# RKWin93/E2E-MAPPO-for-MT-FJSP

Measured on AMD Instinct MI355X. Metric: env-steps/sec (batched J6M6E2), higher is better.
Workload: dtype f64 (environment) / f32 (encoder: f32 storage and accumulation; 128x128 products on the 16-bit matrix cores from split f32 operands, f32-accurate: DESIGN.md §4)

## Files before the change

### __graft_entry__.py

```python
#!/usr/bin/env python3
import os
import sys

ROOT = os.path.dirname(os.path.abspath(__file__))
if ROOT not in sys.path:
    sys.path.insert(0, ROOT)


def build() -> None:
    from importlib import import_module
    import mtfjsp_amd
    _build = import_module("e2e-mappo-for-mt-fjsp_amd._build")
    lib = _build.build(force=True, verbose=True)
    capi = import_module("e2e-mappo-for-mt-fjsp_amd.capi")
    capi.lib()
    print("variant:", _build.build_variant("funcs", ["-DMTFJSP_BODY_FUNCS=3"]))
    from oracle import env_oracle
    print("oracle:", env_oracle.build(force=True))
    print("built", lib)


def smoke() -> None:
    import numpy as np
    import torch
    from importlib import import_module
    import mtfjsp_amd
    assert torch.cuda.is_available(), "smoke() needs cuda:0"
    batch_env = import_module("e2e-mappo-for-mt-fjsp_amd.batch_env")
    inst = import_module("e2e-mappo-for-mt-fjsp_amd.instances")
    from oracle.env_oracle import OracleBatch
    J, M, E, B = 6, 6, 2, 8
    T = J * M
    t, p, tt, edge = inst.generate_instances(B, J, M, E, seed=0)
    import random
    random.seed(0)
    w3 = inst.random_weights(B)
    env = batch_env.DeviceBatchEnv(J, M, E, B, obs_dtype="f64")
    env.load_instances(t, p, tt, edge=edge)
    env.scaler_init()
    env.reset(w3)
    orc = OracleBatch(t, p, tt, edge)
    orc.scaler_init()
    orc.reset(w3)
    a = torch.zeros(B, dtype=torch.int32, device=env.device); m = torch.zeros_like(a); j = torch.zeros_like(a)
    for s in range(T):
        env.random_actions(7, s, a, m, j)
        env.step(a, m)
        info, raw, _ = orc.step(a.cpu().numpy(), m.cpu().numpy())
        cand, mask = orc.job_mask_update(j.cpu().numpy())
        o = orc.observe()
        assert np.array_equal(env.info.cpu().numpy(), info), f"step {s}: rewards differ"
        assert np.array_equal(env.tasks_fea.cpu().numpy(), o["tfea"]), f"step {s}: tasks_fea differ"
        assert np.array_equal(env.dense_adj().cpu().numpy(), o["adj"]), f"step {s}: adj differ"
        assert np.array_equal(env.m_fea2.cpu().numpy(), o["mfea2"])
        assert np.array_equal(env.candidate.cpu().numpy(), cand) and np.array_equal(env.job_mask.cpu().numpy(), mask)
    assert bool(env.info[:, 1].all())
    _smoke_encoder()
    print("smoke OK: HIP env == oracle on", B, "instances x", T, "steps")


def _smoke_encoder() -> None:
    try:
        from importlib import import_module
        enc = import_module("e2e-mappo-for-mt-fjsp_amd.encoder")
    except ImportError:
        return
    if hasattr(enc, "smoke"):
        enc.smoke()


if __name__ == "__main__":
    cmd = sys.argv[1] if len(sys.argv) > 1 else "build"
    {"build": build, "smoke": smoke}[cmd]()
```

### e2e-mappo-for-mt-fjsp_amd/capi.py

```python
import ctypes as C
import os

from . import _build

_LIB = None

OBS_F64, OBS_F32 = 0, 1
OK, ERR_ARG, ERR_STATE, ERR_HIP, ERR_ACTION, ERR_RETRY = 0, -1, -2, -3, -4, -5
PATH_MASK, ST_INVALID, ST_INFEASIBLE = 0x7, 0x100, 0x200
FORK_INSTANCE, FORK_STATE, FORK_OBS = 1, 2, 4
STATE_MACHINE, STATE_START, STATE_FINISH, STATE_ROUTES, STATE_PREV_COSTS, STATE_SCALER, STATE_W3 = range(7)


class Config(C.Structure):
    _fields_ = [("n_job", C.c_int32), ("n_machine", C.c_int32), ("n_edge", C.c_int32), ("batch", C.c_int32),
                ("left_shift", C.c_int32), ("obs_dtype", C.c_int32), ("device_id", C.c_int32), ("reserved", C.c_int32),
                ("gamma", C.c_double), ("w_mk", C.c_double), ("w_ec", C.c_double), ("w_tt", C.c_double),
                ("scaling_divisor", C.c_double)]


class Obs(C.Structure):
    _fields_ = [("tasks_fea", C.c_void_p), ("ell_col", C.c_void_p), ("ell_val", C.c_void_p), ("m_fea2", C.c_void_p),
                ("info", C.c_void_p), ("raw", C.c_void_p), ("candidate", C.c_void_p), ("job_mask", C.c_void_p),
                ("status", C.c_void_p)]


class Mfea1Ctx(C.Structure):
    _fields_ = [("t", C.c_void_p), ("p", C.c_void_p), ("tt", C.c_void_p), ("mean3", C.c_void_p), ("shop", C.c_void_p),
                ("link", C.c_void_p), ("m_fea1_out", C.c_void_p), ("mmask_out", C.c_void_p),
                ("T", C.c_int32), ("M", C.c_int32), ("obs_f32", C.c_int32), ("m_fea2", C.c_void_p)]


class EncoderConfig(C.Structure):
    _fields_ = [("n_job", C.c_int32), ("n_machine", C.c_int32), ("batch", C.c_int32), ("hidden", C.c_int32),
                ("obs_dtype", C.c_int32), ("device_id", C.c_int32)]


_VP, _I, _U64, _SZ = C.c_void_p, C.c_int, C.c_uint64, C.c_size_t
PROTOTYPES = {
    "mtfjsp_create": (_I, [C.POINTER(Config), C.POINTER(_VP)]),
    "mtfjsp_destroy": (_I, [_VP]),
    "mtfjsp_last_error": (C.c_char_p, [_VP]),
    "mtfjsp_set_stream": (_I, [_VP, _VP]),
    "mtfjsp_synchronize": (_I, [_VP]),
    "mtfjsp_alloc_obs": (_I, [_VP, C.POINTER(Obs)]),
    "mtfjsp_bind_obs": (_I, [_VP, C.POINTER(Obs)]),
    "mtfjsp_snapshot_obs": (_I, [_VP, C.POINTER(Obs)]),
    "mtfjsp_snapshot_obs2": (_I, [_VP, C.POINTER(Obs), C.POINTER(Obs), _VP]),
    "mtfjsp_generate_instances": (_I, [_VP, _U64, _U64, _VP]),
    "mtfjsp_read_instances_host": (_I, [_VP, _VP, _VP, _VP, _VP]),
    "mtfjsp_load_instances": (_I, [_VP, _VP, _VP, _VP, _VP]),
    "mtfjsp_load_instances_host": (_I, [_VP, _VP, _VP, _VP, _VP]),
    "mtfjsp_scaler_init": (_I, [_VP]),
    "mtfjsp_scaler_reset_returns": (_I, [_VP]),
    "mtfjsp_scaler_reset_returns_masked_host": (_I, [_VP, _VP]),
    "mtfjsp_reset": (_I, [_VP, _VP]),
    "mtfjsp_draw_reward_weights": (_I, [_VP, _U64, _U64, _VP]),
    "mtfjsp_reset_episode": (_I, [_VP, _U64, _U64, _VP, C.c_int32]),
    "mtfjsp_reset_host": (_I, [_VP, _VP]),
    "mtfjsp_step": (_I, [_VP, _VP, _VP]),
    "mtfjsp_step_host": (_I, [_VP, _VP, _VP]),
    "mtfjsp_step_record": (_I, [_VP, _VP, _VP, _VP, _VP]),
    "mtfjsp_step_params_bytes": (C.c_int32, []),
    "mtfjsp_step_params": (_I, [_VP, _VP, _VP, _VP, _VP, _VP, C.c_int32]),
    "mtfjsp_step_kernel_name": (C.c_char_p, [_VP]),
    "mtfjsp_step_kernel_name_for": (C.c_char_p, [C.c_int32, C.c_int32, C.c_int32, C.c_int32, C.c_int64, C.POINTER(C.c_int32), C.POINTER(C.c_int64), C.POINTER(C.c_int32)]),
    "mtfjsp_gae": (_I, [_VP, C.c_int32, _VP, C.c_int64, C.c_int64, _VP, C.c_int64, C.c_int64, _VP, C.c_int64, C.c_int64, _VP, C.c_float, C.c_float, _VP]),
    "mtfjsp_normalize_advantages": (_I, [_VP, C.c_int32, C.c_int32, C.c_int32, C.c_int32, C.c_int32, _VP, C.c_float, _VP, _VP, _VP, _VP, _VP, _VP]),
    "mtfjsp_pack_views": (_I, [_VP, C.c_int32, C.c_int32, _VP, _VP, _VP, _VP]),
    "mtfjsp_observe_mfea1": (_I, [_VP, _VP, _VP, _VP, _VP]),
    "mtfjsp_random_actions": (_I, [_VP, _U64, _U64, _VP, _VP, _VP]),
    "mtfjsp_pdr_plan": (_I, [_VP, _VP, _VP, _VP, _U64, _VP, _VP]),
    "mtfjsp_fork": (_I, [_VP, _VP, _VP, C.c_int32]),
    "mtfjsp_lookahead_expand": (_I, [_VP, _VP, _VP, _VP]),
    "mtfjsp_lookahead_select": (_I, [_VP, _VP, C.c_int32, _VP, _VP, _VP, _VP]),
    "mtfjsp_export_dense_adj": (_I, [_VP, _VP]),
    "mtfjsp_export_dense_adj_host": (_I, [_VP, _VP]),
    "mtfjsp_valid_action_mask": (_I, [_VP, _VP]),
    "mtfjsp_read_state_host": (_I, [_VP, _I, _VP]),
    "mtfjsp_set_scaler_state_host": (_I, [_VP, _I, _I, _VP]),
    "mtfjsp_copy_to_host": (_I, [_VP, _VP, _VP, _SZ]),
    "mtfjsp_footprint_copy": (_I, [_VP, _SZ, _SZ, C.c_int32, C.c_int32, C.c_int32, C.POINTER(C.c_double), C.POINTER(C.c_double)]),
    "mtfjsp_timing_begin": (_I, [_VP]),
    "mtfjsp_timing_end": (_I, [_VP, C.POINTER(C.c_double), C.POINTER(C.c_int64)]),
    "mtfjsp_encoder_create": (_I, [C.POINTER(EncoderConfig), C.POINTER(_VP)]),
    "mtfjsp_encoder_destroy": (_I, [_VP]),
    "mtfjsp_encoder_last_error": (C.c_char_p, [_VP]),
    "mtfjsp_encoder_set_stream": (_I, [_VP, _VP]),
    "mtfjsp_encoder_load_weight_host": (_I, [_VP, C.c_char_p, _VP, C.c_int64]),
    "mtfjsp_encoder_weights_ready": (_I, [_VP]),
    "mtfjsp_job_actor_forward": (_I, [_VP] * 11),
    "mtfjsp_machine_actor_forward": (_I, [_VP] * 8),
    "mtfjsp_global_critic_forward": (_I, [_VP] * 7),
    "mtfjsp_sample_categorical": (_I, [_VP, _VP, C.c_int32, C.c_int32, _U64, _U64, _VP, _VP, _VP, _VP]),
    "mtfjsp_encoder_set_bn_mode": (_I, [_VP, C.c_int32]),
    "mtfjsp_encoder_set_product_mode": (_I, [_VP, C.c_int32]),
    "mtfjsp_encoder_set_stats_reduce": (_I, [_VP, C.c_void_p, _VP, C.c_int64]),
    "mtfjsp_encoder_set_deferred_poll": (_I, [_VP, C.c_int32]),
    "mtfjsp_get_mfea1_context": (_I, [_VP, _VP, _VP, C.POINTER(Mfea1Ctx)]),
    "mtfjsp_encoder_arm_mfea1": (_I, [_VP, C.POINTER(Mfea1Ctx)]),
    "mtfjsp_encoder_arm_machine_heads": (_I, [_VP, _VP, _VP, _VP]),
    "mtfjsp_encoder_fused_launches": (_I, [_VP, C.POINTER(C.c_int64)]),
    "mtfjsp_encoder_arm_env_step": (_I, [_VP, _VP, C.c_int32]),
    "mtfjsp_encoder_arm_values_only": (_I, [_VP]),
    "mtfjsp_encoder_env_step_fused": (_I, [_VP]),
    "mtfjsp_encoder_arm_selection": (_I, [_VP, C.c_int32, C.c_int32, _U64, _U64, _VP, _VP, _VP, _VP]),
    "mtfjsp_hostgen_infeasible": (_I, [_VP, C.POINTER(C.c_int32), C.c_int64, _I, _I, C.c_int64, C.c_int64, _VP]),
    "mtfjsp_hostgen_transport": (_I, [_VP, C.POINTER(C.c_int32), C.c_int64, _I, _VP, C.c_double, C.c_double, C.c_double, C.c_int64, C.c_int64, _VP]),
    "mtfjsp_encoder_check": (_I, [_VP, C.POINTER(C.c_int32)]),
    "mtfjsp_encoder_resident_failures": (_I, [_VP, C.POINTER(C.c_int64)]),
    "mtfjsp_encoder_range_fallbacks": (_I, [_VP, C.POINTER(C.c_int64), C.POINTER(C.c_int32)]),
    "mtfjsp_encoder_peek_nodes_host": (_I, [_VP, _VP, C.c_int64]),
    "mtfjsp_encoder_timing_begin": (_I, [_VP]),
    "mtfjsp_encoder_timing_end": (_I, [_VP, C.POINTER(C.c_double), C.POINTER(C.c_int64)]),
    "mtfjsp_encoder_timing_query": (_I, [_VP, C.c_char_p, C.POINTER(C.c_double), C.POINTER(C.c_int64)]),
}


def lib_path():
    return os.environ.get("MTFJSP_LIB") or _build.LIB


def lib():
    global _LIB
    if _LIB is None:
        path = lib_path()
        if not os.path.exists(path):
            raise RuntimeError(
                f"{path} is missing: build the HIP extension first (python __graft_entry__.py build, "
                "or python e2e-mappo-for-mt-fjsp_amd/_build.py). There is no CPU fallback.")
        L = C.CDLL(path)
        for name, (res, args) in PROTOTYPES.items():
            fn = getattr(L, name)
            fn.restype, fn.argtypes = res, args
        _LIB = L
    return _LIB


class MtfjspError(RuntimeError):
    def __init__(self, code, msg):
        super().__init__(f"libmtfjsp error {code}: {msg}")
        self.code = code


def check(rc, handle=None, enc=False):
    if rc != 0:
        L = lib()
        msg = (L.mtfjsp_encoder_last_error(handle) if enc else L.mtfjsp_last_error(handle)) or b""
        raise MtfjspError(rc, msg.decode())
```

### e2e-mappo-for-mt-fjsp_amd/csrc/mtfjsp_encoder.hip

```cpp
#include <hip/hip_runtime.h>
#include <math.h>
#include <stdint.h>
#include <stdio.h>
#include <stdlib.h>
#include <string.h>
#include <algorithm>
#include <map>
#include <stdexcept>
#include <string>
#include <vector>

#include "../../include/mtfjsp.h"


#include "mtfjsp_enc_shared.h"

enum { PRO_PLAIN = 0, PRO_BNRELU = 1, PRO_AGG = 2, PRO_GIN0 = 3, PRO_GIN0BN = 4 };
enum { EPI_PLAIN = 0, EPI_STATS = 1, EPI_TANH = 2 };

struct GemmArgs {
    const float *in;
    int N;
    const float *Wt;
    const void *Wx6;
// ... 2379 lines not shown
    float *my_a = s_a + wave * 16 * LDA16;
    float *my_f = s_feat + wave * 128;
    const float *ap = my_a + m * LDA16 + q;
    const float *bp = s_w + q * HD + m;
    int bo[8];
    for (int c = 0; c < 8; c++) bo[c] = (c ^ qo) * 16;
    float asrc[8], adst[8];
    for (int c = 0; c < 8; c++) { asrc[c] = A.gat_a[c * 16 + m]; adst[c] = A.gat_a[HD + c * 16 + m]; }
    const int t = wave;
    const bool active = t * 16 < N;
    float mv[8][2];
    for (int c = 0; c < 8; c++) { mv[c][0] = 0.f; mv[c][1] = 0.f; }
    if (active) {
        {
            const int r = t * 16 + (lane >> 1), k0 = (lane & 1) * 4;
            float x[4] = {0.f, 0.f, 0.f, 0.f};
            if (lane < 32 && r < N) {
                const int u = r >> 1, node = r & 1, width = node ? 8 : 6;
                for (int k = 0; k < 4; k++)
                    if (k0 + k < width) {
                        const size_t idx = ((size_t)b * M + u) * width + k0 + k;
                        x[k] = A.feat_f64 ? (float)reinterpret_cast<const double *>(node ? A.f2 : A.f1)[idx]
                                          : reinterpret_cast<const float *>(node ? A.f2 : A.f1)[idx];
                    }
            }
            if (lane < 32) *reinterpret_cast<float4 *>(my_f + lane * 4) = make_float4(x[0], x[1], x[2], x[3]);
            asm volatile("s_waitcnt lgkmcnt(0)" ::: "memory");
        }
#pragma unroll
        for (int p = 0; p < 8; p++) {
            const int r = 2 * p + h;
            const float4 fa = *reinterpret_cast<const float4 *>(my_f + r * 8), fb = *reinterpret_cast<const float4 *>(my_f + r * 8 + 4);
            const float ff[8] = {fa.x, fa.y, fa.z, fa.w, fb.x, fb.y, fb.z, fb.w};
            float o[4];
            for (int x = 0; x < 4; x++) {
                float a = 0.f;
                for (int k = 0; k < 8; k++) {
                    const float w = h == 0 ? (k < 6 ? A.W1[(c4 + x) * 6 + k] : 0.f) : A.W2[(c4 + x) * 8 + k];
                    a = fmaf(ff[k], w, a);
                }
                o[x] = a;
            }
            float *d = my_a + r * LDA16 + c4;
            *reinterpret_cast<float2 *>(d) = make_float2(o[0], o[1]);
            *reinterpret_cast<float2 *>(d + 2) = make_float2(o[2], o[3]);
        }
        asm volatile("s_waitcnt lgkmcnt(0)" ::: "memory");
#pragma unroll 1
        for (int pass = 0; pass < 3; pass++) {
            f32x4 acc[8];
            for (int c = 0; c < 8; c++) for (int i = 0; i < 4; i++) acc[c][i] = 0.f;
            mfma_tile16(ap, bp, bo, acc);
            asm volatile("" ::: "memory");
#pragma unroll
            for (int u = 0; u < 2; u++) {
                const int i = 2 * u;
                float s0 = 0.f, d0 = 0.f, d1 = 0.f;
                for (int c = 0; c < 8; c++) { const float z0 = acc[c][i], z1 = acc[c][i + 1]; s0 += asrc[c] * z0; d0 += adst[c] * z0; d1 += adst[c] * z1; }
                s0 = row_sum16(s0); d0 = row_sum16(d0); d1 = row_sum16(d1);
                float e00 = s0 + d0, e01 = s0 + d1;
                e00 = e00 > 0.f ? e00 : 0.2f * e00;
                e01 = e01 > 0.f ? e01 : 0.2f * e01;
                const float mx = fmaxf(e00, e01);
                const float x0 = __expf(e00 - mx), x1 = __expf(e01 - mx);
                const float inv = 1.0f / (x0 + x1);
                const float al0 = x0 * inv, al1 = x1 * inv;
                const int r = 4 * q + i;
                for (int c = 0; c < 8; c++) {
                    const float z0 = acc[c][i], z1 = acc[c][i + 1];
                    float n0 = al0 * z0 + al1 * z1, n1 = z1;
                    if (pass < 2) {
                        n0 = n0 > 0.f ? n0 : __expf(n0) - 1.0f;
                        n1 = n1 > 0.f ? n1 : __expf(n1) - 1.0f;
                        my_a[r * LDA16 + c * 16 + m] = n0;
                        my_a[(r + 1) * LDA16 + c * 16 + m] = n1;
                    } else mv[c][u] = (n0 + n1) * 0.5f;
                }
            }
            asm volatile("s_waitcnt lgkmcnt(0)" ::: "memory");
        }
        for (int c = 0; c < 8; c++) {
            double a = 0, bq = 0;
            for (int u = 0; u < 2; u++)
                if (t * 16 + 4 * q + 2 * u < N) { a += (double)mv[c][u]; bq += (double)mv[c][u] * (double)mv[c][u]; }
            a += __shfl_xor(a, 16); a += __shfl_xor(a, 32);
            bq += __shfl_xor(bq, 16); bq += __shfl_xor(bq, 32);
            if (q == 0) { atomicAdd(&s_st[c * 16 + m], a); atomicAdd(&s_st[HD + c * 16 + m], bq); }
        }
    }
    __syncthreads();
    stage_bn_local(s_bn, s_st, 1.0 / (double)M, A.gamma, A.beta, tid);
    __syncthreads();
    if (active) {
        for (int c = 0; c < 8; c++) {
            const int col = c * 16 + m;
            float pl = 0.f;
            for (int u = 0; u < 2; u++) {
                const int r = t * 16 + 4 * q + 2 * u;
                if (r < N) {
                    const float y = fmaf(mv[c][u], s_bn[col], s_bn[HD + col]);
                    A.node[((size_t)b * M + (r >> 1)) * HD + col] = y;
                    pl += y;
                }
            }
            pl += __shfl_xor(pl, 16); pl += __shfl_xor(pl, 32);
            if (q == 0) atomicAdd(&s_pool[col], pl);
        }
    }
    __syncthreads();
    if (tid < HD) A.h_pooled[(size_t)b * HD + tid] = s_pool[tid] / (float)M;
}
static size_t inst_lds_bytes() { return (size_t)(HD * HD + 8 * 16 * LDA16 + 2 * HD) * 4 + 512 * 8 + (HD + 8 * 128) * 4 + 64; }

struct mtfjsp_encoder {
    mtfjsp_encoder_config_t cfg;
    int T = 0;
    hipStream_t stream = nullptr;
    std::string err;
    std::map<std::string, float *> w;
    std::map<std::string, float *> wt;
    std::map<std::string, std::vector<float>> hostw;
    std::map<std::string, float *> wfused;
    std::map<std::string, size_t> wx6_bytes;
    std::map<std::string, size_t> wx32_bytes;
    std::map<std::string, void *> wx6;
    std::map<std::string, void *> wx32;
    std::map<std::string, float> wx32_sinv;
    std::map<std::string, float> wx6_sinv;
    std::map<std::string, float *> wimg;
    std::vector<void *> owned;
    int num_cu = 256;
    float *zA = nullptr, *zB = nullptr;
    float *cand_feat = nullptr;
    float *u = nullptr, *c1 = nullptr, *c2 = nullptr, *hm_b = nullptr, *pooled_int = nullptr;
    bool hm_b_valid = false;
    float *node = nullptr;
    double *stats = nullptr;
    bool gin_slot5_dirty = false;
    bool gin_stats_clean = false;
    bool gat_stats_clean[2] = {false, false};
    int bn_mode = 0;
    bool defer_poll = false;
    mtfjsp_stats_reduce_fn reduce_fn = nullptr; void *reduce_user = nullptr;
    double reduce_scale = 1.0;
    int f32_products = (getenv("MTFJSP_GEMM_F32MFMA") ? 1 : 0) | (getenv("MTFJSP_GAT_F32MFMA") ? 2 : 0) |
                       (getenv("MTFJSP_HEADS_F32MFMA") ? 4 : 0) | (getenv("MTFJSP_GIN0_VALU") ? 8 : 0);
    bool res_ok = false; int res_ipc = 0, res_grid = 0;
    double *res_stats = nullptr;
    unsigned long long *res_bar = nullptr;
    unsigned *res_fail = nullptr;
    volatile unsigned *res_fail_host = nullptr;
    unsigned *range_flag = nullptr;
    long long range_fallbacks = 0;
    bool res_eligible = false;
    long long res_failures = 0, res_launches = 0;
    long long res_fail_at = getenv("MTFJSP_GIN_RES_FAIL_AT") ? atoll(getenv("MTFJSP_GIN_RES_FAIL_AT")) : 0;
    long long range_fail_at = getenv("MTFJSP_RANGE_FAIL_AT") ? atoll(getenv("MTFJSP_RANGE_FAIL_AT")) : 0, job_forwards = 0;
    float *res_zspill = nullptr;
    unsigned long long res_epoch = 0;
    int gat_slot = 0;
    struct { bool valid = false; const void *f1 = nullptr, *f2 = nullptr; int slot = 0;
             bool heads = false; const float *h_pooled_o = nullptr; const uint8_t *mmask = nullptr; float *prob = nullptr, *h_pooled = nullptr, *machine_v = nullptr;
           } prefused;
    bool fuse_gat = !getenv("MTFJSP_NO_FUSED_GAT");
    bool fuse_mheads = !getenv("MTFJSP_NO_FUSED_MHEADS");
    struct { bool armed = false; float *prob = nullptr, *h_pooled = nullptr, *machine_v = nullptr; } mh;
    unsigned long long *xw = nullptr;
    unsigned long long xw_epoch = 0;
    long long fused3_launches = 0;
    double xchg_fine_limit = getenv("MTFJSP_XCHG_FINE_LIMIT") ? atof(getenv("MTFJSP_XCHG_FINE_LIMIT")) : 2147483648.0;
    long long fused3_fail_at = getenv("MTFJSP_FUSED3_FAIL_AT") ? atoll(getenv("MTFJSP_FUSED3_FAIL_AT")) : 0;
    bool heads_hg8 = !getenv("MTFJSP_NO_HEADS_HG8");
    bool heads10 = !getenv("MTFJSP_NO_HEADS10");
    bool fuse_env = getenv("MTFJSP_FUSED_ENV") != nullptr;
    bool fuse_env3 = getenv("MTFJSP_FUSED_ENV3") != nullptr;
    bool nodes_lds = !getenv("MTFJSP_FUSED3_NODES_HBM");
    bool warm_heads = !getenv("MTFJSP_NO_WARM_HEADS");
    struct { bool armed = false, done = false; EnvParams P; } env_step;
    int fuse_pair = getenv("MTFJSP_FUSE_PAIR") ? atoi(getenv("MTFJSP_FUSE_PAIR")) : 0;
    int stream_order = getenv("MTFJSP_NO_STREAM_ORDER") ? 0 : 1;
    int fuse_pool = getenv("MTFJSP_FUSE_POOL") ? atoi(getenv("MTFJSP_FUSE_POOL")) : 1;
    int fuse_gin0 = getenv("MTFJSP_FUSE_GIN0") ? atoi(getenv("MTFJSP_FUSE_GIN0")) : 1;
    int pool_s = getenv("MTFJSP_POOL_S") ? atoi(getenv("MTFJSP_POOL_S")) : 4;
    int stream_nt = getenv("MTFJSP_STREAM_NT") ? atoi(getenv("MTFJSP_STREAM_NT")) : 5;
    mtfjsp_mfea1_ctx_t mf_ctx{}; bool mf_armed = false;
    struct FusedSample { bool armed = false; int greedy = 0; uint64_t seed = 0, counter = 0; int32_t *idx = nullptr; float *logp = nullptr;
                         const int32_t *gather_from = nullptr; int32_t *gathered = nullptr; } fs[2];
    int values_only = 0;
    bool vo_now = false;
    FusedSample fs1_consumed;
    bool timing = false;
    std::map<std::string, std::vector<std::pair<hipEvent_t, hipEvent_t>>> ev;
    std::vector<std::pair<hipEvent_t, hipEvent_t>> ev_free;
};
static thread_local std::string g_enc_err;

#define HIPCHK(e, call)                                                                         \
    do {                                                                                        \
        hipError_t e_ = (call);                                                                 \
        if (e_ != hipSuccess) {                                                                 \
            (e)->err = std::string(#call) + ": " + hipGetErrorString(e_);                       \
            return MTFJSP_ERR_HIP;                                                              \
        }                                                                                       \
    } while (0)

template <typename Tp>
static int dalloc(mtfjsp_encoder *e, Tp **ptr, size_t n)
{
    HIPCHK(e, hipMalloc((void **)ptr, n * sizeof(Tp)));
    e->owned.push_back(*ptr);
    return 0;
}

static const char *REQUIRED[] = {
    "job_actor._input",
    "job_actor.encoder.feature_extract.mlps.0.linears.0.weight", "job_actor.encoder.feature_extract.mlps.0.linears.0.bias",
    "job_actor.encoder.feature_extract.mlps.0.linears.1.weight", "job_actor.encoder.feature_extract.mlps.0.linears.1.bias",
    "job_actor.encoder.feature_extract.mlps.0.linears.2.weight", "job_actor.encoder.feature_extract.mlps.0.linears.2.bias",
    "job_actor.encoder.feature_extract.mlps.0.batch_norms.0.weight", "job_actor.encoder.feature_extract.mlps.0.batch_norms.0.bias",
    "job_actor.encoder.feature_extract.mlps.0.batch_norms.1.weight", "job_actor.encoder.feature_extract.mlps.0.batch_norms.1.bias",
    "job_actor.encoder.feature_extract.mlps.1.linears.0.weight", "job_actor.encoder.feature_extract.mlps.1.linears.0.bias",
    "job_actor.encoder.feature_extract.mlps.1.linears.1.weight", "job_actor.encoder.feature_extract.mlps.1.linears.1.bias",
    "job_actor.encoder.feature_extract.mlps.1.linears.2.weight", "job_actor.encoder.feature_extract.mlps.1.linears.2.bias",
    "job_actor.encoder.feature_extract.mlps.1.batch_norms.0.weight", "job_actor.encoder.feature_extract.mlps.1.batch_norms.0.bias",
    "job_actor.encoder.feature_extract.mlps.1.batch_norms.1.weight", "job_actor.encoder.feature_extract.mlps.1.batch_norms.1.bias",
    "job_actor.encoder.feature_extract.batch_norms.0.weight", "job_actor.encoder.feature_extract.batch_norms.0.bias",
    "job_actor.encoder.feature_extract.batch_norms.1.weight", "job_actor.encoder.feature_extract.batch_norms.1.bias",
    "job_actor.o_policy.linears.0.weight", "job_actor.o_policy.linears.0.bias",
    "job_actor.o_policy.linears.1.weight", "job_actor.o_policy.linears.1.bias",
    "job_actor.o_policy.linears.2.weight", "job_actor.o_policy.linears.2.bias",
    "job_actor.job_critic.linears.0.weight", "job_actor.job_critic.linears.0.bias",
    "job_actor.job_critic.linears.1.weight", "job_actor.job_critic.linears.1.bias",
    "job_actor.job_critic.linears.2.weight", "job_actor.job_critic.linears.2.bias",
    "machine_actor.bn.weight", "machine_actor.bn.bias", "machine_actor.m_fea_1_fcl.weight", "machine_actor.m_fea_2_fcl.weight",
    "machine_actor.gat_layer.W", "machine_actor.gat_layer.a",
    "machine_actor.m_policy.linears.0.weight", "machine_actor.m_policy.linears.0.bias",
    "machine_actor.m_policy.linears.1.weight", "machine_actor.m_policy.linears.1.bias",
    "machine_actor.m_policy.linears.2.weight", "machine_actor.m_policy.linears.2.bias",
    "machine_actor.machine_critic.linears.0.weight", "machine_actor.machine_critic.linears.0.bias",
    "machine_actor.machine_critic.linears.1.weight", "machine_actor.machine_critic.linears.1.bias",
    "machine_actor.machine_critic.linears.2.weight", "machine_actor.machine_critic.linears.2.bias",
};

static int res_alloc_fail_word(mtfjsp_encoder *e)
{
    void *h = nullptr, *d = nullptr;
    if (hipHostMalloc(&h, 64, hipHostMallocMapped) != hipSuccess) return 1;
    if (hipHostGetDevicePointer(&d, h, 0) != hipSuccess) { (void)hipHostFree(h); return 1; }
    e->res_fail_host = (volatile unsigned *)h; e->res_fail = (unsigned *)d; e->range_flag = (unsigned *)d + 1;
    e->res_fail_host[0] = 0u; e->res_fail_host[1] = 0u;
    return 0;
}
static bool res_census(mtfjsp_encoder *e)
{
    if (hipDeviceSynchronize() != hipSuccess) return false;
    if (hipMemset(e->res_bar, 0, (size_t)17 * 16 * 8) != hipSuccess) return false;
    e->res_epoch = 0;
    *e->res_fail_host = 0u;
    GinResArgs a{};
    a.bar = e->res_bar; a.epoch = e->res_epoch++; a.fail = e->res_fail; a.barrier_only = 1;
    hipLaunchKernelGGL(k_gin_res, dim3(e->res_grid), dim3(256), gin_res_lds_bytes(), nullptr, a);
    if (hipDeviceSynchronize() != hipSuccess || *e->res_fail_host) {
        (void)hipMemset(e->res_bar, 0, (size_t)17 * 16 * 8); e->res_epoch = 0; *e->res_fail_host = 0u;
        return false;
    }
    return true;
}
static bool split_products_in_use(const mtfjsp_encoder *e) { return (e->f32_products & 15) != 15; }
static int res_poll_failure(mtfjsp_encoder *e)
{
    if (!e->res_fail_host) return MTFJSP_OK;
    if (e->res_fail_host[0]) {
        (void)hipStreamSynchronize(e->stream);
        e->res_ok = false; e->res_failures++;
        e->res_fail_host[0] = 0u; e->res_fail_host[1] = 0u;
        (void)hipMemset(e->res_bar, 0, (size_t)17 * 16 * 8); e->res_epoch = 0;
        if (e->res_stats) (void)hipMemset(e->res_stats, 0, (size_t)2 * GR_STATS_SET * 8);
        if (e->xw) (void)hipMemset(e->xw, 0, (size_t)2 * XW_SET * 8);
        e->xw_epoch = 0; e->prefused.valid = false; e->prefused.heads = false;
        e->gin_stats_clean = false; e->gat_stats_clean[0] = e->gat_stats_clean[1] = false;
        e->err = "single-launch GIN kernel / fused heads launch: a grid-wide statistics exchange timed out (the workgroups were not co-resident); every output "
                 "enqueued since that launch is invalid and must be recomputed; the handle now uses the streaming launches";
        return MTFJSP_ERR_RETRY;
    }
    if (e->res_fail_host[1]) {
        (void)hipStreamSynchronize(e->stream);
        e->res_fail_host[1] = 0u;
        if (split_products_in_use(e)) {
            e->f32_products |= 15; e->range_fallbacks++;
            e->gin_stats_clean = false; e->gat_stats_clean[0] = e->gat_stats_clean[1] = false;
            e->err = "an activation left the f16 range of the split products (outputs were not numbers): the handle now uses the "
                     "f32-instruction kernels; repeat the forward(s) enqueued since";
            return MTFJSP_ERR_RETRY;
        }
    }
    return MTFJSP_OK;
}

extern "C" const char *mtfjsp_encoder_last_error(mtfjsp_encoder_t e) { return e ? e->err.c_str() : g_enc_err.c_str(); }

extern "C" int mtfjsp_encoder_create(const mtfjsp_encoder_config_t *cfg, mtfjsp_encoder_t *out)
{
    if (!cfg || !out) { g_enc_err = "null argument"; return MTFJSP_ERR_ARG; }
    if (cfg->hidden != HD || cfg->n_job < 1 || cfg->n_job > 64 || cfg->n_machine < 2 || cfg->n_machine > 64 || cfg->batch < 1) {
        g_enc_err = "bad encoder configuration (hidden must be 128, n_job<=64, 2<=n_machine<=64)"; return MTFJSP_ERR_ARG;
    }
    int ndev = 0;
    if (hipGetDeviceCount(&ndev) != hipSuccess || ndev == 0) { g_enc_err = "no HIP device available"; return MTFJSP_ERR_HIP; }
    if (cfg->device_id < 0 || cfg->device_id >= ndev) { g_enc_err = "device_id out of range"; return MTFJSP_ERR_ARG; }
    if (hipSetDevice(cfg->device_id) != hipSuccess) { g_enc_err = "hipSetDevice failed"; return MTFJSP_ERR_HIP; }
    mtfjsp_encoder *e = new mtfjsp_encoder();
    e->cfg = *cfg;
    e->T = cfg->n_job * cfg->n_machine;
    hipDeviceProp_t prop;
    if (hipGetDeviceProperties(&prop, cfg->device_id) == hipSuccess) e->num_cu = prop.multiProcessorCount;
    const size_t B = cfg->batch, T = e->T, M = cfg->n_machine, J = cfg->n_job, R = J > M ? J : M;
    int rc = 0;
    auto rows_padded = [](size_t rows) { return ((rows + 31) / 32 + 1) * 32; };
    auto dalloc_rows = [&](float **ptr, size_t rows) {
        const size_t n = rows_padded(rows) * HD;
        if (dalloc(e, ptr, n)) return 1;
        return hipMemset(*ptr, 0, n * sizeof(float)) == hipSuccess ? 0 : 1;
    };
    rc |= dalloc_rows(&e->zA, B * T); rc |= dalloc_rows(&e->zB, B * T);
    rc |= dalloc_rows(&e->cand_feat, B * R);
    rc |= dalloc_rows(&e->u, B); rc |= dalloc_rows(&e->c1, B); rc |= dalloc_rows(&e->c2, B); rc |= dalloc_rows(&e->hm_b, B);
    rc |= dalloc_rows(&e->pooled_int, B);
    rc |= dalloc_rows(&e->node, B * M);
    rc |= dalloc(e, &e->stats, 8 * STAT_REP * 256);
    rc |= res_alloc_fail_word(e);
    rc |= dalloc(e, &e->xw, (size_t)2 * XW_SET);
    if (!rc && hipMemset(e->xw, 0, (size_t)2 * XW_SET * 8) != hipSuccess) rc = 1;
    if (!rc && hipMemset(e->stats, 0, 8 * STAT_REP * 256 * sizeof(double)) == hipSuccess) { e->gin_stats_clean = true; e->gat_stats_clean[0] = e->gat_stats_clean[1] = true; }
    if (rc) { g_enc_err = e->err; mtfjsp_encoder_destroy(e); return MTFJSP_ERR_HIP; }
    const int lds16 = (int)gemm16_lds_bytes();
    (void)hipFuncSetAttribute((const void *)k_gemm16<EPI_PLAIN, false>, hipFuncAttributeMaxDynamicSharedMemorySize, lds16);
    (void)hipFuncSetAttribute((const void *)k_gemm16<EPI_TANH, false>, hipFuncAttributeMaxDynamicSharedMemorySize, lds16);
    (void)hipFuncSetAttribute((const void *)k_gemm16<EPI_TANH, true>, hipFuncAttributeMaxDynamicSharedMemorySize, lds16);
    (void)hipFuncSetAttribute((const void *)k_gemm16p<PRO_BNRELU>, hipFuncAttributeMaxDynamicSharedMemorySize, lds16);
    (void)hipFuncSetAttribute((const void *)k_gemm16p<PRO_AGG>, hipFuncAttributeMaxDynamicSharedMemorySize, lds16);
    (void)hipFuncSetAttribute((const void *)k_gat3, hipFuncAttributeMaxDynamicSharedMemorySize, lds16);
    (void)hipFuncSetAttribute((const void *)k_gat3x, hipFuncAttributeMaxDynamicSharedMemorySize, (int)gat3x_lds_bytes());
    (void)hipFuncSetAttribute((const void *)k_gemm_x6<PRO_BNRELU>, hipFuncAttributeMaxDynamicSharedMemorySize, (int)gemm_x6_lds_bytes());
    (void)hipFuncSetAttribute((const void *)k_gemm_x6<PRO_AGG>, hipFuncAttributeMaxDynamicSharedMemorySize, (int)gemm_x6_lds_bytes());
    (void)hipFuncSetAttribute((const void *)k_gemm_x6<PRO_GIN0>, hipFuncAttributeMaxDynamicSharedMemorySize, (int)gemm_x6_lds_bytes());
    (void)hipFuncSetAttribute((const void *)k_gemm_x6<PRO_GIN0BN>, hipFuncAttributeMaxDynamicSharedMemorySize, (int)gemm_x6_lds_bytes());
    if (hipFuncSetAttribute((const void *)k_gemm_x6f, hipFuncAttributeMaxDynamicSharedMemorySize, (int)gemm_x6f_lds_bytes()) != hipSuccess) e->fuse_pair = 0;
    (void)hipFuncSetAttribute((const void *)k_gin_inst<float>, hipFuncAttributeMaxDynamicSharedMemorySize, (int)inst_lds_bytes());
    (void)hipFuncSetAttribute((const void *)k_gin_inst<double>, hipFuncAttributeMaxDynamicSharedMemorySize, (int)inst_lds_bytes());
    (void)hipFuncSetAttribute((const void *)k_gat_inst, hipFuncAttributeMaxDynamicSharedMemorySize, (int)inst_lds_bytes());
    (void)hipFuncSetAttribute((const void *)k_heads, hipFuncAttributeMaxDynamicSharedMemorySize, (int)heads_lds_bytes());
    (void)hipFuncSetAttribute((const void *)k_headsx, hipFuncAttributeMaxDynamicSharedMemorySize, (int)headsx_lds_bytes());
    if (hipFuncSetAttribute((const void *)k_headsx10, hipFuncAttributeMaxDynamicSharedMemorySize, (int)headsx10_lds_bytes()) != hipSuccess) e->heads10 = false;
    (void)hipFuncSetAttribute((const void *)k_headsx_envstep<float>, hipFuncAttributeMaxDynamicSharedMemorySize, (int)(headsx_lds_bytes() > EnvGrpDynLds<1>::bytes ? headsx_lds_bytes() : EnvGrpDynLds<1>::bytes));
    (void)hipFuncSetAttribute((const void *)k_headsx_envstep<double>, hipFuncAttributeMaxDynamicSharedMemorySize, (int)(headsx_lds_bytes() > EnvGrpDynLds<1>::bytes ? headsx_lds_bytes() : EnvGrpDynLds<1>::bytes));
    (void)hipFuncSetAttribute((const void *)k_headsx_gat3x, hipFuncAttributeMaxDynamicSharedMemorySize,
                              (int)(headsx_lds_bytes() > gat3x_lds_bytes() ? headsx_lds_bytes() : gat3x_lds_bytes()));
#if !MTFJSP_BODY_FUNCS
    (void)hipFuncSetAttribute((const void *)k_headsx_values, hipFuncAttributeMaxDynamicSharedMemorySize, (int)headsx_lds_bytes());
    (void)hipFuncSetAttribute((const void *)k_headsx_gat3x_headsx<1, false>, hipFuncAttributeMaxDynamicSharedMemorySize, (int)fused3_lds_bytes());
    (void)hipFuncSetAttribute((const void *)k_headsx_gat3x_headsx<2, false>, hipFuncAttributeMaxDynamicSharedMemorySize, (int)fused3_lds_bytes());
    (void)hipFuncSetAttribute((const void *)k_headsx_gat3x_headsx<0, true>, hipFuncAttributeMaxDynamicSharedMemorySize, (int)fused3_lds_bytes());
    (void)hipFuncSetAttribute((const void *)k_headsx_gat3x_headsx<1, true>, hipFuncAttributeMaxDynamicSharedMemorySize, (int)fused3_lds_bytes());
    (void)hipFuncSetAttribute((const void *)k_headsx_gat3x_headsx<2, true>, hipFuncAttributeMaxDynamicSharedMemorySize, (int)fused3_lds_bytes());
    if (hipFuncSetAttribute((const void *)k_headsx_gat3x_headsx<0, false>, hipFuncAttributeMaxDynamicSharedMemorySize,
                            (int)fused3_lds_bytes()) != hipSuccess) e->fuse_mheads = false;
#else
    e->fuse_mheads = false;
#endif
    {
        const int T = e->T, B = cfg->batch;
        if (!getenv("MTFJSP_NO_RESIDENT_GIN") && T >= GR_MINT && T <= GR_MAXT) {
            const int ipc = (B + e->num_cu - 1) / e->num_cu;
            const int grid = (B + ipc - 1) / ipc;
            if (ipc * T <= GR_ROWS && ipc <= GR_MAXIPC && grid <= e->num_cu && (grid + 7) / 8 <= 63 && ipc * cfg->n_job <= GR_MAXCAND &&
                hipFuncSetAttribute((const void *)k_gin_res, hipFuncAttributeMaxDynamicSharedMemorySize, (int)gin_res_lds_bytes()) == hipSuccess) {
                int rc = dalloc(e, &e->res_stats, (size_t)2 * GR_STATS_SET) | dalloc(e, &e->res_bar, (size_t)17 * 16) |
                         dalloc(e, &e->res_zspill, (size_t)grid * 4 * (GR_NT - GR_NRES) * 1024);
                if (!rc && hipMemset(e->res_stats, 0, (size_t)2 * GR_STATS_SET * 8) == hipSuccess &&
                    hipMemset(e->res_bar, 0, (size_t)17 * 16 * 8) == hipSuccess) {
                    e->res_ipc = ipc; e->res_grid = grid; e->res_eligible = true;
                    e->res_ok = res_census(e);
                }
            }
        }
    }
    *out = e;
    return MTFJSP_OK;
}

extern "C" int mtfjsp_encoder_destroy(mtfjsp_encoder_t e)
{
    if (!e) return MTFJSP_OK;
    (void)hipSetDevice(e->cfg.device_id);
    (void)hipDeviceSynchronize();
    for (void *p : e->owned) (void)hipFree(p);
    if (e->res_fail_host) (void)hipHostFree((void *)e->res_fail_host);
    for (auto &kv : e->ev) for (auto &p : kv.second) { (void)hipEventDestroy(p.first); (void)hipEventDestroy(p.second); }
    for (auto &p : e->ev_free) { (void)hipEventDestroy(p.first); (void)hipEventDestroy(p.second); }
    delete e;
    return MTFJSP_OK;
}
extern "C" int mtfjsp_encoder_set_stream(mtfjsp_encoder_t e, void *s) { if (!e) return MTFJSP_ERR_ARG; e->stream = (hipStream_t)s; return MTFJSP_OK; }

static uint16_t f32_to_f16_bits(float x)
{
    uint32_t u; memcpy(&u, &x, 4);
    const uint32_t sign = (u >> 16) & 0x8000u; u &= 0x7fffffffu;
    uint32_t o;
    if (u >= ((127u + 16u) << 23)) o = u > (255u << 23) ? 0x7e00u : 0x7c00u;
    else if (u < (113u << 23)) { float f, magic; const uint32_t mb = ((127u - 15u) + (23u - 10u) + 1u) << 23; memcpy(&f, &u, 4); memcpy(&magic, &mb, 4);
                                 f += magic; uint32_t fu; memcpy(&fu, &f, 4); o = fu - mb; }
    else { const uint32_t odd = (u >> 13) & 1u; u += ((15u - 127u) << 23) + 0xfffu; u += odd; o = u >> 13; }
    return (uint16_t)(o | sign);
}
static float f16_bits_to_f32(uint16_t hbits)
{
    const uint32_t sgn = (uint32_t)(hbits & 0x8000u) << 16, ex = (hbits >> 10) & 31u, m = hbits & 0x3ffu;
    float x;
    if (ex == 0) { x = ldexpf((float)m, -24); return sgn ? -x : x; }
    const uint32_t u = sgn | ((ex == 31 ? 255u : ex + 112u) << 23) | (m << 13);
    memcpy(&x, &u, 4); return x;
}
static float f16_image_scale(const float *data, int64_t numel, bool *finite)
{
    float mx = 0.f;
    for (int64_t i = 0; i < numel; i++) mx = fmaxf(mx, fabsf(data[i]));
    *finite = mx < INFINITY;
    int ex = 0;
    if (mx > 0.f && *finite) (void)frexpf(mx, &ex);
    int k = 14 - ex; k = k > 60 ? 60 : k < -60 ? -60 : k;
    return ldexpf(1.0f, k);
}

static int64_t expected_numel(const std::string &key)
{
    const size_t dot = key.find('.');
    if (dot == std::string::npos) return -1;
    const std::string pre = key.substr(0, dot), k = key.substr(dot + 1);
    if (pre != "job_actor" && pre != "machine_actor" && pre != "global_critic") return -1;
    auto ends = [&](const char *suf) { const size_t n = strlen(suf); return k.size() >= n && k.compare(k.size() - n, n, suf) == 0; };
    auto has = [&](const char *sub) { return k.find(sub) != std::string::npos; };
    if (k == "_input") return HD;
    if (has("batch_norms") || k == "bn.weight" || k == "bn.bias" || k == "encoder.feature_extract.bn.weight" || k == "encoder.feature_extract.bn.bias")
        return has("feature_extract.bn.") ? 12 : HD;
    if (has("feature_extract.mlps.")) {
        if (ends(".bias")) return HD;
        return has("mlps.0.linears.0.weight") ? (int64_t)HD * 12 : (int64_t)HD * HD;
    }
    if (has("feature_extract.eps")) return 2;
    if (k == "m_fea_1_fcl.weight") return (int64_t)HD * 6;
    if (k == "m_fea_2_fcl.weight") return (int64_t)HD * 8;
    if (k == "gat_layer.W") return (int64_t)HD * HD;
    if (k == "gat_layer.a") return 2 * HD;
    if (has("fcl_pooling")) return ends(".bias") ? HD : (int64_t)HD * HD;
    for (const char *head : {"o_policy", "m_policy", "job_critic", "machine_critic", "critic"}) {
        const std::string h = std::string(head) + ".linears.";
        if (k.compare(0, h.size(), h) != 0) continue;
        const int layer = k[h.size()] - '0';
        const bool policy = strstr(head, "policy") != nullptr;
        const int first_in = policy ? 3 * HD : (strcmp(head, "critic") == 0 ? 2 * HD : HD);
        const int out_last = policy ? 1 : (strcmp(head, "critic") == 0 ? 4 : 2);
        const int in = layer == 0 ? first_in : HD, out = layer == 2 ? out_last : HD;
        if (layer < 0 || layer > 2) return -1;
        return ends(".bias") ? out : (int64_t)out * in;
    }
    return -1;
}

extern "C" int mtfjsp_encoder_load_weight_host(mtfjsp_encoder_t e, const char *name, const float *data, int64_t numel)
{
    if (!e || !name || !data || numel <= 0) return MTFJSP_ERR_ARG;
    std::string key(name);
    {
        const int64_t want = expected_numel(key);
        if (want < 0) { e->err = "unknown weight name: " + key; return MTFJSP_ERR_ARG; }
        if (want != numel) {
            e->err = "weight " + key + ": expected " + std::to_string(want) + " elements, got " + std::to_string(numel);
            return MTFJSP_ERR_ARG;
        }
    }
    HIPCHK(e, hipSetDevice(e->cfg.device_id));
    float *d = nullptr;
    auto it = e->w.find(key);
    if (it != e->w.end()) d = it->second;
    else { if (dalloc(e, &d, (size_t)numel)) return MTFJSP_ERR_HIP; e->w[key] = d; }
    HIPCHK(e, hipMemcpy(d, data, (size_t)numel * 4, hipMemcpyHostToDevice));
    if (key == "job_actor._input") e->hm_b_valid = false;
    if ((key.size() >= 11 && key.compare(key.size() - 11, 11, "gat_layer.W") == 0) || key.find("m_fea_1_fcl.weight") != std::string::npos ||
        key.find("m_fea_2_fcl.weight") != std::string::npos) {
        e->hostw[key].assign(data, data + numel);
        const std::string prefix = key.substr(0, key.find('.') + 1);
        e->wfused.erase(prefix + "1"); e->wfused.erase(prefix + "2"); e->wfused.erase(prefix + "q");
    }
    if (numel == (int64_t)HD * 12 && key.find("mlps.0.linears.0.weight") != std::string::npos) {
        auto to_bf16 = [](float x) { uint32_t u; memcpy(&u, &x, 4); u += 0x7fffu + ((u >> 16) & 1u); return (uint16_t)(u >> 16); };
        auto from_bf16 = [](uint16_t b) { uint32_t u = (uint32_t)b << 16; float x; memcpy(&x, &u, 4); return x; };
        std::vector<uint16_t> im((size_t)4 * 2 * 3 * 64 * 8, 0);
        for (int cgi = 0; cgi < 4; cgi++)
            for (int c = 0; c < 2; c++)
                for (int lane = 0; lane < 64; lane++)
                    for (int i = 0; i < 8; i++) {
                        const int n = 32 * cgi + 16 * c + (lane & 15), k = 8 * (lane >> 4) + i;
                        if (k >= 12) continue;
                        const float w = data[(size_t)n * 12 + k];
                        const uint16_t p0 = to_bf16(w); const float r1 = w - from_bf16(p0);
                        const uint16_t p1 = to_bf16(r1); const float r2 = r1 - from_bf16(p1);
                        const uint16_t pl[3] = {p0, p1, to_bf16(r2)};
                        for (int p = 0; p < 3; p++) im[(((((size_t)cgi * 2 + c) * 3 + p) * 64 + lane) * 8) + i] = pl[p];
                    }
        void *dx = nullptr;
        auto kt = e->wx6.find(key);
        if (kt != e->wx6.end()) dx = kt->second;
        else { float *tmp = nullptr; if (dalloc(e, &tmp, im.size() / 2)) return MTFJSP_ERR_HIP; dx = tmp; e->wx6[key] = dx; }
        HIPCHK(e, hipMemcpy(dx, im.data(), im.size() * 2, hipMemcpyHostToDevice));
            e->wx6_bytes[key] = im.size() * 2;
    }
    if (key.find("feature_extract.mlps.") != std::string::npos && key.size() > 7 && key.compare(key.size() - 7, 7, ".weight") == 0 &&
        key.find("linears") != std::string::npos) {
        const int in = (int)(numel / HD), KS = in == 12 ? 1 : in / 16, P = in == 12 ? 3 : 2;
        auto to_bf16 = [](float x) { uint32_t u; memcpy(&u, &x, 4); u += 0x7fffu + ((u >> 16) & 1u); return (uint16_t)(u >> 16); };
        auto from_bf16 = [](uint16_t b) { uint32_t u = (uint32_t)b << 16; float x; memcpy(&x, &u, 4); return x; };
        float scale = 1.0f;
        if (P == 2) {
            bool finite = true;
            scale = f16_image_scale(data, numel, &finite);
            if (!finite) { e->err = "load_weight: non-finite value in " + key; return MTFJSP_ERR_ARG; }
        }
        std::vector<uint16_t> im((size_t)4 * P * KS * 64 * 8, 0);
        for (int w = 0; w < 4; w++)
            for (int ks = 0; ks < KS; ks++)
                for (int lane = 0; lane < 64; lane++)
                    for (int j = 0; j < 8; j++) {
                        const int n = 32 * w + (lane & 31), k = 16 * ks + 8 * (lane >> 5) + j;
// ... 211 lines not shown
            hipLaunchKernelGGL((k_gin0<float>), dim3(pgrid), dim3(256), 0, e->stream, N, T, (const float *)tasks_fea, ell_col, ell_val,
                               W(P + "mlps.0.linears.0.weight"), W(P + "mlps.0.linears.0.bias"), e->zA, st + 0 * STAT_REP * 256);
        else
            hipLaunchKernelGGL((k_gin0<double>), dim3(pgrid), dim3(256), 0, e->stream, N, T, (const double *)tasks_fea, ell_col, ell_val,
                               W(P + "mlps.0.linears.0.weight"), W(P + "mlps.0.linears.0.bias"), e->zA, st + 0 * STAT_REP * 256);
        if ((rrc = reduce_stats(e, st + 0 * STAT_REP * 256))) return rrc;
    }
    const int so = e->stream_order;
    auto bn_gemm = [&](const float *in, float *out, int sin, const std::string &bn, const std::string &lin, int sout, int rev) {
        GemmArgs a = gemm_args(in, N, WT(P + lin + ".weight"), W(P + lin + ".bias"), out);
        a.rev = so ? rev : 0; a.nt = so && (e->stream_nt & 1);
        a.pro_stats = st + sin * STAT_REP * 256; a.pro_gamma = W(P + bn + ".weight"); a.pro_beta = W(P + bn + ".bias"); a.pro_inv_rows = invN;
        a.epi_stats = st + sout * STAT_REP * 256;
        a.Wx6 = e->wx6.at(P + lin + ".weight"); a.w_sinv = e->wx6_sinv.at(P + lin + ".weight");
        launch_gemm<PRO_BNRELU, EPI_STATS>(e, a, "gin_gemm_bn_relu");
        if (!rrc) rrc = reduce_stats(e, st + sout * STAT_REP * 256);
    };
    auto bn_gemm_pair = [&](const float *in, float *out, int sin, const std::string &bn1, const std::string &lin1, int smid,
                            const std::string &bn2, const std::string &lin2, int sout, int rev) {
        {
            GemmArgs a = gemm_args(in, N, WT(P + lin1 + ".weight"), W(P + lin1 + ".bias"), nullptr);
            a.rev = so ? rev : 0; a.nt = so && (e->stream_nt & 1);
            a.pro_stats = st + sin * STAT_REP * 256; a.pro_gamma = W(P + bn1 + ".weight"); a.pro_beta = W(P + bn1 + ".bias"); a.pro_inv_rows = invN;
            a.epi_stats = st + smid * STAT_REP * 256;
            a.Wx6 = e->wx6.at(P + lin1 + ".weight"); a.w_sinv = e->wx6_sinv.at(P + lin1 + ".weight");
            launch_gemm<PRO_BNRELU, EPI_STATS>(e, a, "gin_gemm_stats_only");
            if (!rrc) rrc = reduce_stats(e, st + smid * STAT_REP * 256);
        }
        {
            Timed t(e, "gin_gemm_pair");
            Gemm2Args g{};
            g.a = gemm_args(in, N, WT(P + lin1 + ".weight"), W(P + lin1 + ".bias"), out);
            g.a.rev = so ? rev ^ 1 : 0; g.a.nt = so && (e->stream_nt & 1);
            g.a.pro_stats = st + sin * STAT_REP * 256; g.a.pro_gamma = W(P + bn1 + ".weight"); g.a.pro_beta = W(P + bn1 + ".bias"); g.a.pro_inv_rows = invN;
            g.a.epi_stats = st + sout * STAT_REP * 256;
            g.a.Wx6 = e->wx6.at(P + lin1 + ".weight"); g.a.w_sinv = e->wx6_sinv.at(P + lin1 + ".weight");
            g.a.range_flag = e->range_flag;
            g.Wx6b = e->wx6.at(P + lin2 + ".weight"); g.w_sinvb = e->wx6_sinv.at(P + lin2 + ".weight"); g.biasb = W(P + lin2 + ".bias");
            g.mid_stats = st + smid * STAT_REP * 256; g.mid_gamma = W(P + bn2 + ".weight"); g.mid_beta = W(P + bn2 + ".bias"); g.mid_inv_rows = invN;
            const int ntiles = (N + 15) / 16;
            int grid = (ntiles + 7) / 8;
            if (grid > e->num_cu) grid = e->num_cu;
            hipLaunchKernelGGL(k_gemm_x6f, dim3(grid), dim3(512), gemm_x6f_lds_bytes(), e->stream, g);
        }
        if (!rrc) rrc = reduce_stats(e, st + sout * STAT_REP * 256);
    };
    if (pair) bn_gemm_pair(e->zA, e->zB, 0, "mlps.0.batch_norms.0", "mlps.0.linears.1", 1, "mlps.0.batch_norms.1", "mlps.0.linears.2", 2, 0);
    else {
    if (fuse0) {
        const std::string lin = "mlps.0.linears.1", bn = "mlps.0.batch_norms.0";
        GemmArgs a = gemm_args(nullptr, N, WT(P + lin + ".weight"), W(P + lin + ".bias"), e->zB);
        a.rev = 0; a.nt = 0;
        a.tfea = tasks_fea; a.feat_f64 = 0; a.ell_col = ell_col; a.ell_val = ell_val; a.T = T;
        a.Wx6_0 = e->wx6.at(P + "mlps.0.linears.0.weight"); a.bias0 = W(P + "mlps.0.linears.0.bias");
        a.W0 = mom0 ? W(P + "mlps.0.linears.0.weight") : nullptr;
        a.pro_stats = st + 0 * STAT_REP * 256; a.pro_gamma = W(P + bn + ".weight"); a.pro_beta = W(P + bn + ".bias"); a.pro_inv_rows = invN;
        a.epi_stats = st + 1 * STAT_REP * 256;
        a.Wx6 = e->wx6.at(P + lin + ".weight"); a.w_sinv = e->wx6_sinv.at(P + lin + ".weight");
        launch_gemm<PRO_GIN0BN, EPI_STATS>(e, a, "gin0_bn_gemm");
        if (!rrc) rrc = reduce_stats(e, st + 1 * STAT_REP * 256);
    } else
    bn_gemm(e->zA, e->zB, 0, "mlps.0.batch_norms.0", "mlps.0.linears.1", 1, 0);
    bn_gemm(e->zB, e->zA, 1, "mlps.0.batch_norms.1", "mlps.0.linears.2", 2, 1);
    }
    const float *z2 = pair ? e->zB : e->zA;
    float *z3 = pair ? e->zA : e->zB;
    {
        GemmArgs a = gemm_args(z2, N, WT(P + "mlps.1.linears.0.weight"), W(P + "mlps.1.linears.0.bias"), z3);
        a.pro_stats = st + 2 * STAT_REP * 256; a.pro_gamma = W(P + "batch_norms.0.weight"); a.pro_beta = W(P + "batch_norms.0.bias"); a.pro_inv_rows = invN;
        a.ell_col = ell_col; a.ell_val = ell_val; a.T = T;
        a.rev = 0; a.nt = so && (e->stream_nt & 2);
        a.epi_stats = st + 3 * STAT_REP * 256;
        a.Wx6 = e->wx6.at(P + "mlps.1.linears.0.weight"); a.w_sinv = e->wx6_sinv.at(P + "mlps.1.linears.0.weight");
        launch_gemm<PRO_AGG, EPI_STATS>(e, a, "gin_gemm_agg");
        if (!rrc) rrc = reduce_stats(e, st + 3 * STAT_REP * 256);
    }
    if (pair) bn_gemm_pair(z3, e->zB, 3, "mlps.1.batch_norms.0", "mlps.1.linears.1", 4, "mlps.1.batch_norms.1", "mlps.1.linears.2", 5, 1);
    else {
    bn_gemm(e->zB, e->zA, 3, "mlps.1.batch_norms.0", "mlps.1.linears.1", 4, 1);
    const bool fuse_pool = e->fuse_pool && h_pooled && !h_nodes && T >= 16 && T < 65536 && (!candidate || (J > 0 && T % J == 0)) && (size_t)N < ((size_t)1 << 24) &&
                           e->wx6.count(P + "mlps.1.linears.2.weight") && !(e->f32_products & 1);
    if (fuse_pool) {
        const std::string lin = "mlps.1.linears.2", bn = "mlps.1.batch_norms.1";
        GemmArgs a = gemm_args(e->zA, N, WT(P + lin + ".weight"), W(P + lin + ".bias"), nullptr);
        a.rev = 0; a.nt = 0;
        a.pro_stats = st + 4 * STAT_REP * 256; a.pro_gamma = W(P + bn + ".weight"); a.pro_beta = W(P + bn + ".bias"); a.pro_inv_rows = invN;
        a.epi_stats = st + 5 * STAT_REP * 256;
        a.Wx6 = e->wx6.at(P + lin + ".weight"); a.w_sinv = e->wx6_sinv.at(P + lin + ".weight");
        a.zero_f32 = h_pooled; a.zero_count = B * HD;
        launch_gemm<PRO_BNRELU, EPI_STATS>(e, a, "gin_gemm_stats_only");
        a.zero_f32 = nullptr; a.zero_count = 0;
        if (!rrc) rrc = reduce_stats(e, st + 5 * STAT_REP * 256);
        if (rrc) return rrc;
        a.rev = so ? 1 : 0; a.nt = so && (e->stream_nt & 1);
        a.epi_stats = nullptr;
        a.T = T; a.pooled = h_pooled; a.cand_feat = candidate ? cand_feat : nullptr; a.cand = candidate; a.pool_J = candidate ? J : 0;
        a.pool_stats = st + 5 * STAT_REP * 256; a.pool_gamma = W(P + "batch_norms.1.weight"); a.pool_beta = W(P + "batch_norms.1.bias"); a.pool_inv_rows = invN;
        launch_gemm<PRO_BNRELU, EPI_STATS>(e, a, "gin_gemm_pool");
        if (candidate) {
            Timed t(e, "cand_fixup");
            hipLaunchKernelGGL(k_cand_fixup, dim3((B * J + 127) / 128), dim3(128), 0, e->stream, B, T, J, candidate, e->zA, st + 4 * STAT_REP * 256, W(P + bn + ".weight"), W(P + bn + ".bias"),
                               WT(P + lin + ".weight"), W(P + lin + ".bias"), st + 5 * STAT_REP * 256, W(P + "batch_norms.1.weight"), W(P + "batch_norms.1.bias"), invN, cand_feat);
        }
        HIPCHK(e, hipGetLastError());
        return MTFJSP_OK;
    }
    bn_gemm(e->zA, e->zB, 4, "mlps.1.batch_norms.1", "mlps.1.linears.2", 5, 0);
    }
    if (rrc) return rrc;
    if (h_pooled) {
        Timed t(e, "job_pool_gather");
        const int ntiles = (N + 15) / 16, ggrid = std::min((ntiles + 7) / 8, e->num_cu), rpr = so && e->pool_s > 0 ? ((ntiles + ggrid - 1) / ggrid) * 16 : 0;
        const int pool_grid = rpr ? ggrid * e->pool_s : (B < e->num_cu * 8 ? B : e->num_cu * 8);
        if (so && (e->stream_nt & 4))
            hipLaunchKernelGGL(k_job_pool_gather<1>, dim3(pool_grid), dim3(256), 0, e->stream, split_products_in_use(e) ? e->range_flag : nullptr, rpr, e->pool_s, B, T, candidate ? J : 0, e->zB, st + 5 * STAT_REP * 256, invN,
                               W(P + "batch_norms.1.weight"), W(P + "batch_norms.1.bias"), candidate, h_pooled, cand_feat, h_nodes);
        else
            hipLaunchKernelGGL(k_job_pool_gather<0>, dim3(pool_grid), dim3(256), 0, e->stream, split_products_in_use(e) ? e->range_flag : nullptr, rpr, e->pool_s, B, T, candidate ? J : 0, e->zB, st + 5 * STAT_REP * 256, invN,
                               W(P + "batch_norms.1.weight"), W(P + "batch_norms.1.bias"), candidate, h_pooled, cand_feat, h_nodes);
    }
    HIPCHK(e, hipGetLastError());
    return MTFJSP_OK;
}

static int run_gin_resident(mtfjsp_encoder *e, const std::string &pre, const void *tasks_fea, const int32_t *ell_col, const float *ell_val,
                            const int32_t *candidate, int J, float *h_pooled, float *cand_feat, float *h_nodes)
{
    const int B = e->cfg.batch, T = e->T;
    const std::string P = pre + "encoder.feature_extract.";
    auto W = [&](const std::string &k) { return e->w.at(k); };
    GinResArgs a{};
    a.B = B; a.T = T; a.J = candidate ? J : 0; a.ipc = e->res_ipc;
    a.tfea = tasks_fea; a.feat_f64 = e->cfg.obs_dtype == MTFJSP_OBS_F64; a.ell_col = ell_col; a.ell_val = ell_val;
    const char *lin[6] = {"mlps.0.linears.0", "mlps.0.linears.1", "mlps.0.linears.2", "mlps.1.linears.0", "mlps.1.linears.1", "mlps.1.linears.2"};
    const char *bn[6] = {"mlps.0.batch_norms.0", "mlps.0.batch_norms.1", "batch_norms.0", "mlps.1.batch_norms.0", "mlps.1.batch_norms.1", "batch_norms.1"};
    for (int i = 0; i < 6; i++) {
        a.Wx32[i] = e->wx32.at(P + lin[i] + ".weight");
        a.wsinv[i] = e->wx32_sinv.at(P + lin[i] + ".weight");
        a.gamma[i] = W(P + bn[i] + ".weight"); a.beta[i] = W(P + bn[i] + ".bias");
    }
    for (int i = 0; i < 6; i++) {
        int ex = 0;
        const float mant = frexpf(a.wsinv[i], &ex);
        if (mant != 0.5f) { e->err = "resident GIN: a weight image scale is not a power of two"; return MTFJSP_ERR_STATE; }
        a.wexp[i] = 1 - ex;
        a.ffrac[i] = i == 0 ? GR_FIX_FRAC_FIRST : GR_FIX_FRAC_DEFAULT;
    }
    const int set = (int)(e->res_epoch & 1);
    a.stats = reinterpret_cast<unsigned long long *>(e->res_stats) + (size_t)set * GR_STATS_SET;
    a.stats_next = reinterpret_cast<unsigned long long *>(e->res_stats) + (size_t)(set ^ 1) * GR_STATS_SET;
    a.bar = e->res_bar; a.epoch = e->res_epoch++; a.fail = e->res_fail; a.range_flag = e->range_flag;
    a.candidate = candidate; a.pooled = h_pooled; a.cand_feat = cand_feat; a.h_nodes = h_nodes; a.zspill = e->res_zspill;
    a.inv_rows = 1.0 / ((double)B * (double)T);
    if (pre == "job_actor." && e->warm_heads) {
        const char *keys[9] = {"job_actor.o_policy.linears.0.weight", "job_actor.job_critic.linears.0.weight", "job_actor.o_policy.linears.1.weight",
                               "job_actor.job_critic.linears.1.weight", "machine_actor.gat_layer.W", "machine_actor.m_policy.linears.0.weight",
                               "machine_actor.machine_critic.linears.0.weight", "machine_actor.m_policy.linears.1.weight", "machine_actor.machine_critic.linears.1.weight"};
        for (const char *k : keys) {
            auto it = e->wx6.find(k);
            auto bt = e->wx6_bytes.find(k);
            if (it == e->wx6.end() || bt == e->wx6_bytes.end() || a.nwarm >= GR_MAXWARM) continue;
            a.warm[a.nwarm] = it->second; a.warm_lines[a.nwarm] = (unsigned)(bt->second / 128); a.nwarm++;
        }
        auto q = e->wfused.find("machine_actor.q");
        if (q != e->wfused.end() && a.nwarm < GR_MAXWARM) { a.warm[a.nwarm] = q->second; a.warm_lines[a.nwarm] = 64; a.nwarm++; }
    }
    if (++e->res_launches == e->res_fail_at) a.expect_extra = 1u;
#ifdef GR_STAMP
    static unsigned long long *d_st = nullptr;
    if (!d_st) (void)hipMalloc((void **)&d_st, 256 * 64 * 8);
    a.stamps = d_st;
#endif
    {
        Timed t(e, "gin_resident");
        hipLaunchKernelGGL(k_gin_res, dim3(e->res_grid), dim3(256), gin_res_lds_bytes(), e->stream, a);
    }
#ifdef GR_STAMP
    static int printed = 0;
    if (printed++ % 50 == 20 && getenv("MTFJSP_STAMP_PRINT")) {
        (void)hipStreamSynchronize(e->stream);
        std::vector<unsigned long long> h((size_t)e->res_grid * 64);
        (void)hipMemcpy(h.data(), d_st, h.size() * 8, hipMemcpyDeviceToHost);
        unsigned long long t0 = ~0ull;
        for (int b = 0; b < e->res_grid; b++) t0 = h[(size_t)b * 64 + 32] < t0 ? h[(size_t)b * 64 + 32] : t0;
        printf("GR_STAMP (us since first block start; mean / max over %d blocks):", e->res_grid);
        for (int i = 0; i < 33; i++) {
            double m = 0, mx = 0;
            for (int b = 0; b < e->res_grid; b++) { const double v = (double)(h[(size_t)b * 64 + i] - t0) / 100.0; m += v; mx = v > mx ? v : mx; }
            printf(" [%d] %.1f/%.1f", i, m / e->res_grid, mx);
        }
        printf("\n");
        {
            auto clk = [&](int a, int b) {
                std::vector<double> v;
                for (int blk = 0; blk < e->res_grid; blk++) {
                    const double dr = (double)(h[(size_t)blk * 64 + b] - h[(size_t)blk * 64 + a]), dc = (double)(h[(size_t)blk * 64 + 33 + b] - h[(size_t)blk * 64 + 33 + a]);
                    if (dr > 0) v.push_back(dc / dr * 0.1);
                }
                std::sort(v.begin(), v.end());
                return v.empty() ? 0.0 : v[v.size() / 2];
            };
            printf("GR_CLOCK launch %d (GHz, median over %d workgroups): five layers [7 -> 24] %.3f | layer 1 [7 -> 8] %.3f  layer 2 [11 -> 12] %.3f  layer 3 [15 -> 16] %.3f  "
                   "layer 4 [19 -> 20] %.3f  layer 5 [23 -> 24] %.3f | whole kernel [0 -> 30] %.3f\n", printed, e->res_grid, clk(7, 24), clk(7, 8), clk(11, 12), clk(15, 16), clk(19, 20), clk(23, 24), clk(0, 30));
        }
    }
#endif
    HIPCHK(e, hipGetLastError());
    return MTFJSP_OK;
}

static std::vector<float> fused_projection_host(mtfjsp_encoder *e, const std::string &pre, int which)
{
    const int K = which == 1 ? 6 : 8;
    const std::vector<float> &P = e->hostw.at(pre + (which == 1 ? "m_fea_1_fcl.weight" : "m_fea_2_fcl.weight"));
    const std::vector<float> &W = e->hostw.at(pre + "gat_layer.W");
    std::vector<float> f((size_t)HD * K);
    for (int n = 0; n < HD; n++)
        for (int k = 0; k < K; k++) {
            double a = 0.0;
            for (int i = 0; i < HD; i++) a += (double)P[(size_t)i * K + k] * (double)W[(size_t)i * HD + n];
            f[(size_t)n * K + k] = (float)a;
        }
    return f;
}
static int fused_projection(mtfjsp_encoder *e, const std::string &pre, int which, const float **out)
{
    const std::string key = pre + (which == 1 ? "1" : "2");
    auto it = e->wfused.find(key);
    if (it != e->wfused.end()) { *out = it->second; return MTFJSP_OK; }
    const std::vector<float> f = fused_projection_host(e, pre, which);
    float *d = nullptr;
    if (dalloc(e, &d, f.size())) return MTFJSP_ERR_HIP;
    HIPCHK(e, hipMemcpy(d, f.data(), f.size() * 4, hipMemcpyHostToDevice));
    e->wfused[key] = d;
    *out = d;
    return MTFJSP_OK;
}
static int fused_projection_image(mtfjsp_encoder *e, const std::string &pre, const float **out)
{
    const std::string key = pre + "q";
    auto it = e->wfused.find(key);
    if (it != e->wfused.end()) { *out = it->second; return MTFJSP_OK; }
    const std::vector<float> f1 = fused_projection_host(e, pre, 1), f2 = fused_projection_host(e, pre, 2);
    std::vector<float> img((size_t)8 * 64 * 4);
    for (int c = 0; c < 8; c++)
        for (int lane = 0; lane < 64; lane++)
            for (int ks = 0; ks < 4; ks++) {
                const int kk = 4 * ks + (lane >> 4), col = 16 * c + (lane & 15);
                img[((size_t)c * 64 + lane) * 4 + ks] = kk < 6 ? f1[(size_t)col * 6 + kk] : kk < 8 ? 0.f : f2[(size_t)col * 8 + (kk - 8)];
            }
    float *d = nullptr;
    if (dalloc(e, &d, img.size())) return MTFJSP_ERR_HIP;
    HIPCHK(e, hipMemcpy(d, img.data(), img.size() * 4, hipMemcpyHostToDevice));
    e->wfused[key] = d;
    *out = d;
    return MTFJSP_OK;
}
static int gat3x_args(mtfjsp_encoder *e, const std::string &pre, const void *m_fea1, const void *m_fea2, int slot, GatArgs *out)
{
    const int R = e->cfg.batch * e->cfg.n_machine;
    double *st = nullptr;
    if (slot >= 0) {
        st = e->stats + (6 + slot) * STAT_REP * 256;
        if (!e->gat_stats_clean[slot]) HIPCHK(e, hipMemsetAsync(st, 0, STAT_REP * 256 * sizeof(double), e->stream));
        e->gat_stats_clean[slot] = false;
    }
    GatArgs a{};
    a.R = R; a.f1 = m_fea1; a.f2 = m_fea2; a.feat_f64 = e->cfg.obs_dtype == MTFJSP_OBS_F64;
    int frc = fused_projection(e, pre, 1, &a.W1);
    if (!frc) frc = fused_projection(e, pre, 2, &a.W2);
    if (!frc) frc = fused_projection_image(e, pre, &a.Wq);
    if (frc) return frc;
    a.Wt = e->wt.at(pre + "gat_layer.W"); a.gat_a = e->w.at(pre + "gat_layer.a"); a.node = e->node; a.epi_stats = st;
    a.Wx6 = e->wx6.at(pre + "gat_layer.W"); a.w_sinv = e->wx6_sinv.at(pre + "gat_layer.W");
    *out = a;
    return MTFJSP_OK;
}
static bool gat_fusable(const mtfjsp_encoder *e)
{
    const int hgrid = e->cfg.batch / HG, gtiles = (2 * e->cfg.batch * e->cfg.n_machine + 15) / 16, ggrid = (gtiles + 7) / 8 < e->num_cu ? (gtiles + 7) / 8 : e->num_cu;
    return e->fuse_gat && !e->bn_mode && !e->reduce_fn && !(e->f32_products & (2 | 4)) && e->cfg.batch % HG == 0 && hgrid <= e->num_cu && hgrid >= ggrid &&
           e->w.count("machine_actor.gat_layer.W") && e->wx6.count("machine_actor.gat_layer.W");
}
static bool mheads_fusable(const mtfjsp_encoder *e)
{
    const int hgrid = e->cfg.batch / HG;
    return e->fuse_mheads && e->res_ok && gat_fusable(e) && hgrid <= e->num_cu && (hgrid + 7) / 8 <= 63 && e->xw && e->cfg.n_machine <= 8 &&
           e->wx6.count("machine_actor.m_policy.linears.0.weight") && e->wx6.count("machine_actor.machine_critic.linears.0.weight");
}
static int run_gat(mtfjsp_encoder *e, const std::string &pre, const void *m_fea1, const void *m_fea2, float *h_pooled, int *slot_out = nullptr)
{
    const int B = e->cfg.batch, M = e->cfg.n_machine, R = B * M;
    auto W = [&](const std::string &k) { return e->w.at(k); };
    auto WT = [&](const std::string &k) { return e->wt.at(k); };
    const int slot = e->gat_slot;
    e->gat_slot ^= 1;
    if (slot_out) *slot_out = slot;
    double *st = e->stats + (6 + slot) * STAT_REP * 256;
    if (!e->gat_stats_clean[slot]) HIPCHK(e, hipMemsetAsync(st, 0, STAT_REP * 256 * sizeof(double), e->stream));
    e->gat_stats_clean[slot] = false;
    {
        Timed t(e, "gat3");
        GatArgs a{};
        a.R = R; a.f1 = m_fea1; a.f2 = m_fea2; a.feat_f64 = e->cfg.obs_dtype == MTFJSP_OBS_F64;
        int frc = fused_projection(e, pre, 1, &a.W1);
        if (!frc) frc = fused_projection(e, pre, 2, &a.W2);
// ... 455 lines not shown
    int slot = 0;
    if (e->prefused.heads && !e->bn_mode && m_fea1 == e->prefused.f1 && m_fea2 == e->prefused.f2 && h_pooled_o == e->prefused.h_pooled_o &&
        mmask == e->prefused.mmask && prob == e->prefused.prob && h_pooled == e->prefused.h_pooled && machine_v == e->prefused.machine_v) {
        if (!e->defer_poll && (rc = res_poll_failure(e))) { e->prefused.heads = false; e->prefused.valid = false; return rc; }
        e->prefused.heads = false; e->prefused.valid = false;
        e->fs1_consumed = mtfjsp_encoder::FusedSample{};
        e->env_step.armed = false;
        e->fs[1].armed = false;
        return MTFJSP_OK;
    }
    if (e->prefused.heads && e->fs1_consumed.idx && !e->fs[1].armed) e->fs[1] = e->fs1_consumed;
    e->fs1_consumed = mtfjsp_encoder::FusedSample{};
    e->prefused.heads = false;
    if (e->prefused.valid && !e->bn_mode && m_fea1 == e->prefused.f1 && m_fea2 == e->prefused.f2) slot = e->prefused.slot;
    else rc = e->bn_mode ? run_gat_inst(e, "machine_actor.", m_fea1, m_fea2, h_pooled) : run_gat(e, "machine_actor.", m_fea1, m_fea2, nullptr, &slot);
    e->prefused.valid = false;
    if (rc) return rc;
    {
        Timed t(e, "heads");
        HeadArgs ha = machine_head_args(e, h_pooled_o, mmask, prob, machine_v);
        if (e->bn_mode) ha.pooled = h_pooled;
        else {
            ha.pooled = nullptr;
            ha.xbn_stats = e->stats + (6 + slot) * STAT_REP * 256; ha.xbn_gamma = W("machine_actor.bn.weight"); ha.xbn_beta = W("machine_actor.bn.bias");
            ha.xbn_inv_rows = 1.0 / ((double)R * e->reduce_scale); ha.pooled_out = h_pooled;
            ha.zero_stats = e->stats + (6 + (slot ^ 1)) * STAT_REP * 256; ha.zero_count = STAT_REP * 256;
            e->gat_stats_clean[slot ^ 1] = true;
            if (e->gin_slot5_dirty) {
                ha.zero_stats2 = e->stats + 5 * STAT_REP * 256; ha.zero_count2 = STAT_REP * 256;
                e->gin_slot5_dirty = false; e->gin_stats_clean = true;
            }
        }
        arm_sampling(e, 1, ha);
        e->vo_now = e->values_only > 0 && !ha.sample_mode && !(e->f32_products & 4) && !e->bn_mode;
        if (e->values_only > 0) e->values_only--;
        const EnvParams &EP = e->env_step.P;
        const bool env_tail = e->env_step.armed && e->fuse_env && !e->timing && !e->bn_mode && !(e->f32_products & 4) && ha.sample_mode &&
                              (const void *)ha.idx_out == (const void *)EP.mach_idx && EP.B == B && EP.M == M && env_one_slot(EP.J, EP.M, EP.T);
        e->env_step.armed = false; e->env_step.done = env_tail;
        launch_heads(e, ha, "machine_actor.m_policy", "machine_actor.machine_critic", nullptr, (env_tail && !e->vo_now) ? &EP : nullptr);
        e->vo_now = false;
    }
    HIPCHK(e, hipGetLastError());
    return MTFJSP_OK;
}

__global__ void k_linear_small(int B, int O, const float *x, const float *W, const float *bias, float *out, unsigned *range_flag)
{
    const int i = blockIdx.x * blockDim.x + threadIdx.x;
    if (i >= B * O) return;
    const int b = i / O, o = i % O;
    float p = 0.f;
    for (int k = 0; k < HD; k++) p = fmaf(x[(size_t)b * HD + k], W[o * HD + k], p);
    p += bias[o];
    out[i] = p;
    if (range_flag && p != p) __hip_atomic_store(range_flag, 1u, __ATOMIC_RELAXED, __HIP_MEMORY_SCOPE_SYSTEM);
}

static int global_critic_forward_impl(mtfjsp_encoder_t e, const void *tasks_fea, const int32_t *ell_col, const float *ell_val,
                                      const void *m_fea1, const void *m_fea2, float *value4)
{
    if (!e || !tasks_fea || !ell_col || !ell_val || !m_fea1 || !m_fea2 || !value4) return MTFJSP_ERR_ARG;
    static const char *need[] = {"global_critic.critic.linears.0.weight", "global_critic.critic.linears.2.bias", "global_critic.gat_layer.W",
                                 "global_critic.encoder.feature_extract.mlps.1.linears.2.weight", "global_critic.bn.weight"};
    for (const char *k : need)
        if (!e->w.count(k)) { e->err = std::string("missing weight: ") + k; return MTFJSP_ERR_STATE; }
    HIPCHK(e, hipSetDevice(e->cfg.device_id));
    e->prefused.valid = false; e->prefused.heads = false;
    if (!e->defer_poll) { const int prc = res_poll_failure(e); if (prc) return prc; }
    const int B = e->cfg.batch;
    auto W = [&](const std::string &k) { return e->w.at(k); };
    auto WT = [&](const std::string &k) { return e->wt.at(k); };
    const bool resident = e->res_ok && !e->reduce_fn && !(e->f32_products & (1 | 8 | 16));
    int rc = resident ? run_gin_resident(e, "global_critic.", tasks_fea, ell_col, ell_val, nullptr, 0, e->pooled_int, e->cand_feat, nullptr)
                      : run_gin(e, "global_critic.", tasks_fea, ell_col, ell_val, nullptr, 0, e->pooled_int, e->cand_feat, nullptr);
    if (rc) return rc;
    rc = run_gat(e, "global_critic.", m_fea1, m_fea2, e->u);
    if (rc) return rc;
    const float *W0t = WT("global_critic.critic.linears.0.weight");
    GemmArgs a = gemm_args(e->u, B, W0t, W("global_critic.critic.linears.0.bias"), e->c1);
    launch_gemm<PRO_PLAIN, EPI_PLAIN>(e, a, "head_gemm");
    GemmArgs b = gemm_args(e->pooled_int, B, W0t + HD * HD, nullptr, e->c1);
    launch_gemm<PRO_PLAIN, EPI_TANH, true>(e, b, "head_gemm");
    GemmArgs c = gemm_args(e->c1, B, WT("global_critic.critic.linears.1.weight"), W("global_critic.critic.linears.1.bias"), e->c2);
    launch_gemm<PRO_PLAIN, EPI_TANH>(e, c, "head_gemm");
    {
        Timed t(e, "small");
        hipLaunchKernelGGL(k_linear_small, dim3((B * 4 + 255) / 256), dim3(256), 0, e->stream, B, 4, e->c2, W("global_critic.critic.linears.2.weight"),
                           W("global_critic.critic.linears.2.bias"), value4, split_products_in_use(e) ? e->range_flag : nullptr);
    }
    HIPCHK(e, hipGetLastError());
    return MTFJSP_OK;
}

#define GUARDED(e, call)                                                                               \
    try { return call; }                                                                               \
    catch (const std::exception &ex) { if (e) (e)->err = std::string("missing weight or internal error: ") + ex.what(); return MTFJSP_ERR_STATE; }
extern "C" int mtfjsp_job_actor_forward(mtfjsp_encoder_t e, const void *tasks_fea, const int32_t *ell_col, const float *ell_val,
                                        const int32_t *candidate, const uint8_t *job_mask, const float *h_m_prev,
                                        float *prob, float *h_pooled, float *job_v, float *h_nodes)
{
    GUARDED(e, job_actor_forward_impl(e, tasks_fea, ell_col, ell_val, candidate, job_mask, h_m_prev, prob, h_pooled, job_v, h_nodes))
}
extern "C" int mtfjsp_machine_actor_forward(mtfjsp_encoder_t e, const void *m_fea1, const void *m_fea2, const float *h_pooled_o,
                                            const uint8_t *mmask, float *prob, float *h_pooled, float *machine_v)
{
    GUARDED(e, machine_actor_forward_impl(e, m_fea1, m_fea2, h_pooled_o, mmask, prob, h_pooled, machine_v))
}
extern "C" int mtfjsp_global_critic_forward(mtfjsp_encoder_t e, const void *tasks_fea, const int32_t *ell_col, const float *ell_val,
                                            const void *m_fea1, const void *m_fea2, float *value4)
{
    GUARDED(e, global_critic_forward_impl(e, tasks_fea, ell_col, ell_val, m_fea1, m_fea2, value4))
}

extern "C" int mtfjsp_sample_categorical(mtfjsp_encoder_t e, const float *prob, int32_t n, int32_t greedy, uint64_t seed, uint64_t counter,
                                         int32_t *idx_out, float *logp_out, const int32_t *gather_from, int32_t *gathered_out)
{
    if (!e || !prob || !idx_out || n < 1) return MTFJSP_ERR_ARG;
    HIPCHK(e, hipSetDevice(e->cfg.device_id));
    Timed t(e, "sample");
    const int B = e->cfg.batch;
    hipLaunchKernelGGL(k_sample, dim3((B + 127) / 128), dim3(128), 0, e->stream, B, n, prob, greedy, seed, counter, idx_out, logp_out, gather_from, gathered_out);
    HIPCHK(e, hipGetLastError());
    return MTFJSP_OK;
}

extern "C" int mtfjsp_encoder_check(mtfjsp_encoder_t e, int32_t *gin_resident_out)
{
    if (!e) return MTFJSP_ERR_ARG;
    HIPCHK(e, hipSetDevice(e->cfg.device_id));
    HIPCHK(e, hipStreamSynchronize(e->stream));
    int rc = res_poll_failure(e);
    if (!rc && e->res_eligible && !e->res_ok && e->res_failures > 0 && !getenv("MTFJSP_NO_RESIDENT_GIN")) {
        e->res_ok = res_census(e);
    }
    if (gin_resident_out) *gin_resident_out = (e->res_ok && !e->reduce_fn && !(e->f32_products & (1 | 8 | 16))) ? 1 : 0;
    return rc;
}
extern "C" int mtfjsp_encoder_resident_failures(mtfjsp_encoder_t e, int64_t *count_out)
{
    if (!e || !count_out) return MTFJSP_ERR_ARG;
    *count_out = e->res_failures;
    return MTFJSP_OK;
}

extern "C" int mtfjsp_encoder_peek_nodes_host(mtfjsp_encoder_t e, float *out_host, int64_t count)
{
    if (!e || !out_host || count < 0 || count > (int64_t)e->cfg.batch * e->cfg.n_machine * HD) return MTFJSP_ERR_ARG;
    HIPCHK(e, hipSetDevice(e->cfg.device_id));
    HIPCHK(e, hipStreamSynchronize(e->stream));
    HIPCHK(e, hipMemcpy(out_host, e->node, (size_t)count * sizeof(float), hipMemcpyDeviceToHost));
    return MTFJSP_OK;
}
extern "C" int mtfjsp_encoder_range_fallbacks(mtfjsp_encoder_t e, int64_t *count_out, int32_t *product_mode_out)
{
    if (!e || !count_out) return MTFJSP_ERR_ARG;
    *count_out = e->range_fallbacks;
    if (product_mode_out) *product_mode_out = e->f32_products;
    return MTFJSP_OK;
}

extern "C" int mtfjsp_encoder_timing_begin(mtfjsp_encoder_t e)
{
    if (!e) return MTFJSP_ERR_ARG;
    for (auto &kv : e->ev) { for (auto &p : kv.second) e->ev_free.push_back(p); kv.second.clear(); }
    e->timing = true;
    return MTFJSP_OK;
}
extern "C" int mtfjsp_encoder_timing_end(mtfjsp_encoder_t e, double *ms_total, int64_t *launches)
{
    if (!e) return MTFJSP_ERR_ARG;
    HIPCHK(e, hipSetDevice(e->cfg.device_id));
    HIPCHK(e, hipStreamSynchronize(e->stream));
    double tot = 0; int64_t n = 0;
    for (auto &kv : e->ev)
        for (auto &p : kv.second) { float ms = 0; HIPCHK(e, hipEventElapsedTime(&ms, p.first, p.second)); tot += ms; n++; }
    if (ms_total) *ms_total = tot;
    if (launches) *launches = n;
    e->timing = false;
    return MTFJSP_OK;
}
extern "C" int mtfjsp_encoder_timing_query(mtfjsp_encoder_t e, const char *family, double *ms_total, int64_t *launches)
{
    if (!e || !family) return MTFJSP_ERR_ARG;
    HIPCHK(e, hipSetDevice(e->cfg.device_id));
    HIPCHK(e, hipStreamSynchronize(e->stream));
    double tot = 0; int64_t n = 0;
    auto it = e->ev.find(family);
    if (it != e->ev.end())
        for (auto &p : it->second) { float ms = 0; HIPCHK(e, hipEventElapsedTime(&ms, p.first, p.second)); tot += ms; n++; }
    if (ms_total) *ms_total = tot;
    if (launches) *launches = n;
    return MTFJSP_OK;
}
```

### e2e-mappo-for-mt-fjsp_amd/csrc/mtfjsp_gin_resident.h

```cpp
#pragma once
#include <type_traits>
#include <utility>

#ifndef GR_ABL
#define GR_ABL 0
#endif
#define GR_NT 18
#ifndef GR_NRES
#define GR_NRES 16
#endif
#ifndef GR_VRES
#define GR_VRES 1
#endif
#define GR_ROWS (32 * GR_NT)
#define GR_RING 6
#define GR_NBAR 6
#ifndef GR_GRP
#define GR_GRP 2
#endif
#ifndef GR_LOOK
#define GR_LOOK 2
#endif
#define GR_ROWB 272
#define GR_PLANE (32 * GR_ROWB)
#define GR_TILE (2 * GR_PLANE)
#define GR_MAXCAND 384
#define GR_MAXWARM 10
#define GR_MAXT 65
#define GR_MINT 16
#define GR_MAXIPC 64

#ifndef GR_MIX
#define GR_MIX 2
#endif
#ifndef GR_SETTLE
#define GR_SETTLE 1
#endif
#ifndef GR_FOLD_DPP
#define GR_FOLD_DPP 1
#endif
#ifndef GR_STAT_ASM
#define GR_STAT_ASM 0
#endif
#ifndef GR_PK
#define GR_PK 1
#endif
typedef float f32x16 __attribute__((ext_vector_type(16)));
typedef _Float16 gr_h8 __attribute__((ext_vector_type(8)));
typedef _Float16 gr_h2 __attribute__((ext_vector_type(2)));

struct GinResArgs {
    int B, T, J, ipc;
    const void *tfea; int feat_f64;
    const int *ell_col; const float *ell_val;
    const void *Wx32[6];
    float wsinv[6];
    const float *gamma[6], *beta[6];
    unsigned long long *stats;
    unsigned long long *stats_next;
    int wexp[6];
    int ffrac[6];
    unsigned long long *bar;
    unsigned long long epoch;
    unsigned *fail;
    unsigned *range_flag;
    const int *candidate;
    float *pooled;
    float *cand_feat;
    float *h_nodes;
    float *zspill;
    double inv_rows;
    int barrier_only;
    unsigned expect_extra;
    unsigned long long *stamps;
    const void *warm[GR_MAXWARM];
    unsigned warm_lines[GR_MAXWARM];
    int nwarm;
};
#define GR_STATS_PART (6 * 8 * HD * 2)
#define GR_STATS_SET GR_STATS_PART
#ifdef GR_STAMP
#define GR_STAMP_AT(i) do { if (tid == 0 && A.stamps) { A.stamps[(size_t)blockIdx.x * 64 + (i)] = __builtin_amdgcn_s_memrealtime(); \
                                                         if ((i) <= 30) A.stamps[(size_t)blockIdx.x * 64 + 33 + (i)] = __builtin_amdgcn_s_memtime(); } } while (0)
#else
#define GR_STAMP_AT(i) do { } while (0)
#endif

#define GR_OFF_PLANES 0
#define GR_OFF_RING (2 * GR_TILE)
#define GR_RING_BYTES ((2 * GR_LOOK - 2) * GR_TILE > GR_RING * 32 * HD * 4 ? (2 * GR_LOOK - 2) * GR_TILE : GR_RING * 32 * HD * 4)
#define GR_OFF_ELLC (GR_OFF_RING + GR_RING_BYTES)
#define GR_OFF_ELLV0 (GR_OFF_ELLC + GR_ROWS * 4)
#define GR_OFF_ELLV1 (GR_OFF_ELLV0 + GR_ROWS * 4)
#define GR_OFF_BN (GR_OFF_ELLV1 + GR_ROWS * 4)
#define GR_OFF_CAND (GR_OFF_BN + 2 * HD * 4)
#define GR_OFF_ZERO (GR_OFF_CAND + GR_ROWS * 4)
#define GR_OFF_FLAG (GR_OFF_ZERO + 2 * HD * 4)
#define GR_OFF_CNT (GR_OFF_FLAG + 64)
#define GR_LDS_BYTES (GR_OFF_CNT + 5 * (GR_NT / GR_GRP) * 4 + 12)
static size_t gin_res_lds_bytes() { return (size_t)GR_LDS_BYTES; }
static_assert(GR_LDS_BYTES <= 160 * 1024, "resident GIN kernel: LDS budget");

#if GR_PK == 1
__device__ __forceinline__ f32x2 gr_fma2(f32x2 a, f32x2 b, f32x2 c) { return __builtin_elementwise_fma(a, b, c); }
__device__ __forceinline__ f32x2 gr_add2(f32x2 a, f32x2 b) { return a + b; }
__device__ __forceinline__ f32x2 gr_sub2(f32x2 a, f32x2 b) { return a - b; }
__device__ __forceinline__ f32x2 gr_mul2(f32x2 a, f32x2 b) { return a * b; }
#else
#if GR_PK == 2
__device__ __forceinline__ float gr_pin(float x) { return x; }
#else
__device__ __forceinline__ float gr_pin(float x) { asm("" : "+v"(x)); return x; }
#endif
__device__ __forceinline__ f32x2 gr_fma2(f32x2 a, f32x2 b, f32x2 c) { return f32x2{gr_pin(__builtin_fmaf(a[0], b[0], c[0])), gr_pin(__builtin_fmaf(a[1], b[1], c[1]))}; }
__device__ __forceinline__ f32x2 gr_add2(f32x2 a, f32x2 b) { return f32x2{gr_pin(a[0] + b[0]), gr_pin(a[1] + b[1])}; }
__device__ __forceinline__ f32x2 gr_sub2(f32x2 a, f32x2 b) { return f32x2{gr_pin(a[0] - b[0]), gr_pin(a[1] - b[1])}; }
__device__ __forceinline__ f32x2 gr_mul2(f32x2 a, f32x2 b) { return f32x2{gr_pin(a[0] * b[0]), gr_pin(a[1] * b[1])}; }
#endif
__device__ __forceinline__ f32x2 gr_rem2(f32x2 v, gr_h2 p)
{
#if GR_MIX
    float r0, r1;
    const unsigned pp = __builtin_bit_cast(unsigned, p);
    asm("v_fma_mix_f32 %0, %1, -1.0, %2 op_sel_hi:[1,0,0]" : "=v"(r0) : "v"(pp), "v"(v[0]));
    asm("v_fma_mix_f32 %0, %1, -1.0, %2 op_sel:[1,0,0] op_sel_hi:[1,0,0]" : "=v"(r1) : "v"(pp), "v"(v[1]));
    return f32x2{r0, r1};
#else
    return gr_sub2(v, __builtin_convertvector(p, f32x2));
#endif
}
__device__ __forceinline__ gr_h2 gr_rem16(f32x2 v, gr_h2 p)
{
    unsigned r;
    const unsigned pp = __builtin_bit_cast(unsigned, p);
    asm("v_fma_mixlo_f16 %0, %1, -1.0, %2 op_sel_hi:[1,0,0]" : "=v"(r) : "v"(pp), "v"(v[0]));
    asm("v_fma_mixhi_f16 %0, %1, -1.0, %2 op_sel:[1,0,0] op_sel_hi:[1,0,0]" : "+v"(r) : "v"(pp), "v"(v[1]));
    return __builtin_bit_cast(gr_h2, r);
}
template <typename F, int... I>
__device__ __forceinline__ void gr_static_for_impl(F &&f, std::integer_sequence<int, I...>) { (f(std::integral_constant<int, I>{}), ...); }
template <int N, typename F>
__device__ __forceinline__ void gr_static_for(F &&f) { gr_static_for_impl(f, std::make_integer_sequence<int, N>{}); }

__device__ __forceinline__ float gr_sum32(float x)
{
    x = row_sum16(x);
    return x + __shfl_xor(x, 16);
}

#define GR_FIX_FRAC_DEFAULT 20
#define GR_FIX_FRAC_FIRST 12
#define GR_FIX_BIAS (1ull << 51)
#define GR_FIX_ONE (1ull << 58)
#define GR_FIX_PAYLOAD (GR_FIX_ONE - 1ull)
__device__ __forceinline__ unsigned long long gr_fix_encode(float x, int exp2, int frac)
{
    const unsigned u = __builtin_bit_cast(unsigned, x);
    const int e = (int)((u >> 23) & 255u);
    const unsigned long long mant = (unsigned long long)((u & 0x7fffffu) | (e ? 0x800000u : 0u));
    const int sh = (e ? e : 1) - 150 + frac - exp2;
    long long v = sh >= 0 ? (long long)(mant << (sh > 39 ? 39 : sh)) : (sh > -25 ? (long long)((mant + (1ull << (-sh - 1))) >> (-sh)) : 0ll);
    if (u >> 31) v = -v;
    return GR_FIX_ONE | (unsigned long long)(v + (long long)GR_FIX_BIAS);
}
__device__ __forceinline__ double gr_fix_decode(unsigned long long sum, unsigned n, int frac)
{
    const long long v = (long long)sum - (long long)n * (long long)GR_FIX_BIAS;
    return __builtin_ldexp((double)v, -frac);
}

__device__ __forceinline__ void gr_grid_barrier(unsigned long long *bar, unsigned long long gen, unsigned nblk, unsigned *fail, unsigned *s_flag)
{
    const int tid = threadIdx.x;
    const unsigned g = blockIdx.x & 7u;
    const unsigned ngroups = nblk < 8u ? nblk : 8u;
    (void)s_flag;
    __syncthreads();
    if (tid == 0) {
        const unsigned long long gsize = (nblk >> 3) + (g < (nblk & 7u) ? 1u : 0u);
        const unsigned long long old = __hip_atomic_fetch_add(&bar[16 * g], 1ull, __ATOMIC_RELAXED, __HIP_MEMORY_SCOPE_AGENT);
        if (old + 1 == gen * gsize) {
            const unsigned long long old2 = __hip_atomic_fetch_add(&bar[16 * 8], 1ull, __ATOMIC_RELAXED, __HIP_MEMORY_SCOPE_AGENT);
            if (old2 + 1 == gen * ngroups)
                for (unsigned j = 0; j < ngroups; j++) __hip_atomic_store(&bar[16 * (9 + j)], gen, __ATOMIC_RELAXED, __HIP_MEMORY_SCOPE_AGENT);
        }
        const unsigned long long t0 = __builtin_amdgcn_s_memrealtime();
        while (__hip_atomic_load(&bar[16 * (9 + g)], __ATOMIC_RELAXED, __HIP_MEMORY_SCOPE_AGENT) < gen) {
            __builtin_amdgcn_s_sleep(1);
            if (__builtin_amdgcn_s_memrealtime() - t0 > 400000ull) {
                __hip_atomic_store(fail, 1u, __ATOMIC_RELAXED, __HIP_MEMORY_SCOPE_SYSTEM);
                break;
            }
        }
    }
    __syncthreads();
}

#ifdef MTFJSP_GIN_RES_DECL_ONLY
__global__ __launch_bounds__(256) void k_gin_res(GinResArgs A);
#else
__global__ __launch_bounds__(256) void k_gin_res(GinResArgs A)
{
    extern __shared__ __align__(16) unsigned char smem[];
    unsigned char *s_planes = smem + GR_OFF_PLANES;
    float *s_ring = reinterpret_cast<float *>(smem + GR_OFF_RING);
    unsigned *s_ellc = reinterpret_cast<unsigned *>(smem + GR_OFF_ELLC);
    float *s_ellv0 = reinterpret_cast<float *>(smem + GR_OFF_ELLV0);
    float *s_ellv1 = reinterpret_cast<float *>(smem + GR_OFF_ELLV1);
    float *s_bn = reinterpret_cast<float *>(smem + GR_OFF_BN);
    int *s_rowcand = reinterpret_cast<int *>(smem + GR_OFF_CAND);
    float *s_zero = reinterpret_cast<float *>(smem + GR_OFF_ZERO);
    unsigned *s_flag = reinterpret_cast<unsigned *>(smem + GR_OFF_FLAG);
    unsigned *s_cnt = reinterpret_cast<unsigned *>(smem + GR_OFF_CNT);
    const int tid = threadIdx.x, wave = __builtin_amdgcn_readfirstlane(tid >> 6), lane = tid & 63;
    const int n = lane & 31, h = lane >> 5;
    const unsigned nblk = gridDim.x + A.expect_extra;
    const unsigned long long gen0 = A.epoch * GR_NBAR;
    if (A.barrier_only) {
        for (int k = 0; k < GR_NBAR; k++) gr_grid_barrier(A.bar, gen0 + k + 1, nblk, A.fail, s_flag);
        return;
    }
    const int T = A.T;
    const int inst0 = blockIdx.x * A.ipc;
    const int ninst = A.B - inst0 < A.ipc ? A.B - inst0 : A.ipc;
    const int nrows = ninst * T;
    const size_t grow0 = (size_t)inst0 * T;

    GR_STAMP_AT(32);
    f32x4 w0pre[3];
    for (int i = blockIdx.x * 256 + tid; i < GR_STATS_SET; i += (int)gridDim.x * 256) A.stats_next[i] = 0ull;
    {
        int cand_pre[(GR_MAXCAND + 255) / 256];
#pragma unroll
        for (int k = 0; k < (GR_MAXCAND + 255) / 256; k++) {
            const int i = tid + 256 * k;
            cand_pre[k] = (A.candidate && i < ninst * A.J) ? A.candidate[(size_t)inst0 * A.J + i] : -1;
        }
        float *s_feat = s_ring;
        constexpr int NF4 = (GR_ROWS * 3 + 255) / 256, NER = (GR_ROWS + 255) / 256;
        f32x4 fpre[NF4];
        {
            const f32x4 *src = reinterpret_cast<const f32x4 *>(reinterpret_cast<const float *>(A.tfea) + grow0 * 12);
            const int last = nrows * 3 - 1;
#pragma unroll
            for (int k = 0; k < NF4; k++) { const int i = tid + 256 * k; fpre[k] = src[i < last ? i : last]; }
        }
        int2 ecc[NER]; float2 evv[NER];
#pragma unroll
        for (int k = 0; k < NER; k++) {
            const int r = tid + 256 * k, rc = r < nrows ? r : nrows - 1;
            ecc[k] = *reinterpret_cast<const int2 *>(A.ell_col + (grow0 + rc) * 2);
            evv[k] = *reinterpret_cast<const float2 *>(A.ell_val + (grow0 + rc) * 2);
        }
#pragma unroll
        for (int k = 0; k < NF4; k++) reinterpret_cast<f32x4 *>(s_feat)[tid + 256 * k] = fpre[k];
        if (A.feat_f64) {
            const double *src = reinterpret_cast<const double *>(A.tfea) + grow0 * 12;
            const int n12 = nrows * 12;
            __syncthreads();
#pragma unroll 1
            for (int i0 = 0; i0 < n12; i0 += 256 * 9) {
                double d[9];
#pragma unroll
                for (int k = 0; k < 9; k++) { const int i = i0 + tid + 256 * k; d[k] = src[i < n12 ? i : n12 - 1]; }
#pragma unroll
                for (int k = 0; k < 9; k++) { const int i = i0 + tid + 256 * k; if (i < n12) s_feat[i] = (float)d[k]; }
            }
        }
#pragma unroll
        for (int k = 0; k < NER; k++) {
            const int r = tid + 256 * k;
            if (r < GR_ROWS) {
                unsigned cp = 0xffffffffu; float v0 = 0.f, v1 = 0.f;
                if (r < nrows) {
                    const int2 cc = ecc[k];
                    const float2 vv = evv[k];
                    const int base = (r / T) * T;
                    const unsigned r0 = cc.x >= 0 ? (unsigned)(base + cc.x) : 0xffffu, r1 = cc.y >= 0 ? (unsigned)(base + cc.y) : 0xffffu;
                    cp = r0 | (r1 << 16); v0 = cc.x >= 0 ? vv.x : 0.f; v1 = cc.y >= 0 ? vv.y : 0.f;
                }
                s_ellc[r] = cp; s_ellv0[r] = v0; s_ellv1[r] = v1; s_rowcand[r] = -1;
            }
        }
        {
            const f32x4 *wi = reinterpret_cast<const f32x4 *>(A.Wx32[0]) + (size_t)wave * (3 * 64) + lane;
            __builtin_amdgcn_sched_barrier(0);
#pragma unroll
            for (int p = 0; p < 3; p++) w0pre[p] = wi[p * 64];
            __builtin_amdgcn_sched_barrier(0);
        }
        if (tid == 0) s_flag[1] = 0u;
        if (tid < 5 * (GR_NT / GR_GRP)) s_cnt[tid] = 0u;
        for (int i = tid; i < 2 * GR_TILE / 16; i += 256) reinterpret_cast<float4 *>(s_planes)[i] = make_float4(0.f, 0.f, 0.f, 0.f);
        if (A.candidate) {
            LDS_BARRIER();
#pragma unroll
            for (int k = 0; k < (GR_MAXCAND + 255) / 256; k++) {
                const int i = tid + 256 * k, c = cand_pre[k];
                if (i < ninst * A.J && c >= 0 && c < T && atomicExch(&s_rowcand[(i / A.J) * T + c], i) != -1) s_flag[1] = 1u;
            }
        }
        s_zero[tid] = 0.f;
    }
    f32x16 acc[GR_NRES];
    f32x16 zs[2];
    float *zsp = A.zspill + ((size_t)(blockIdx.x * 4 + wave) * (GR_NT - GR_NRES)) * 1024 + lane * 4;
    auto zload = [&](auto Jc) __attribute__((always_inline)) {
        constexpr int j = decltype(Jc)::value;
        if constexpr (GR_VRES) return;
#pragma unroll
        for (int g = 0; g < 4; g++) {
            const float4 v = *reinterpret_cast<const float4 *>(zsp + j * 1024 + g * 256);
            zs[j & 1][4 * g] = v.x; zs[j & 1][4 * g + 1] = v.y; zs[j & 1][4 * g + 2] = v.z; zs[j & 1][4 * g + 3] = v.w;
        }
    };
    auto zstore = [&](auto Jc, const f32x16 &a) __attribute__((always_inline)) {
        constexpr int j = decltype(Jc)::value;
        if constexpr (GR_VRES) return;
#pragma unroll
        for (int g = 0; g < 4; g++) *reinterpret_cast<float4 *>(zsp + j * 1024 + g * 256) = make_float4(a[4 * g], a[4 * g + 1], a[4 * g + 2], a[4 * g + 3]);
    };
#define GR_TILEVAL(rt) ((rt) < GR_NRES ? acc[(rt) < GR_NRES ? (rt) : 0] : zs[(rt) >= GR_NRES ? ((rt) - GR_NRES) & 1 : 0])
    auto mfma_v = [&](f32x16 &c, const gr_h8 &a, const gr_h8 &b, bool zero) __attribute__((always_inline)) {
        if (zero) asm volatile("v_mfma_f32_32x32x16_f16 %0, %1, %2, 0" : "=v"(c) : "v"(a), "v"(b));
        else asm volatile("v_mfma_f32_32x32x16_f16 %0, %1, %2, %0" : "+v"(c) : "v"(a), "v"(b));
    };
    int nrows_l = nrows, n_l = n;
    bool timed_out = false;
    gr_h8 wf[2][8];
    bf16x8 w0f[3];
    f32x2 ts[8], tq[8];
#pragma unroll
    for (int i = 0; i < 8; i++) { ts[i] = f32x2{0.f, 0.f}; tq[i] = f32x2{0.f, 0.f}; }

    auto load_weights = [&](int layer) __attribute__((always_inline)) {
        const float4 *wi = reinterpret_cast<const float4 *>(A.Wx32[layer]) + (size_t)wave * (2 * 8 * 64) + lane;
#pragma unroll
        for (int p = 0; p < 2; p++)
#pragma unroll
            for (int ks = 0; ks < 8; ks++) wf[p][ks] = __builtin_bit_cast(gr_h8, wi[(p * 8 + ks) * 64]);
    };
    auto stat2 = [&](int i, float x, float y) __attribute__((always_inline)) {
        const f32x2 v = {x, y};
#if GR_STAT_ASM == 1
        asm volatile("v_pk_add_f32 %0, %2, %0\n\tv_pk_fma_f32 %1, %2, %2, %1" : "+v"(ts[i]), "+v"(tq[i]) : "v"(v));
#elif GR_STAT_ASM == 2
        float s0 = ts[i][0], s1 = ts[i][1], q0 = tq[i][0], q1 = tq[i][1];
        asm volatile("v_add_f32 %0, %4, %0\n\tv_add_f32 %1, %5, %1\n\tv_fma_f32 %2, %4, %4, %2\n\tv_fma_f32 %3, %5, %5, %3" : "+v"(s0), "+v"(s1), "+v"(q0), "+v"(q1) : "v"(x), "v"(y));
        ts[i] = f32x2{s0, s1}; tq[i] = f32x2{q0, q1};
#else
        ts[i] = gr_add2(ts[i], v); tq[i] = gr_fma2(v, v, tq[i]);
        asm volatile("" : "+v"(ts[i]), "+v"(tq[i]));
#endif
    };
    auto stats_all = [&](const f32x16 &a) __attribute__((always_inline)) {
        if (GR_ABL & 4) return;
#pragma unroll
        for (int i = 0; i < 8; i++) stat2(i, a[2 * i], a[2 * i + 1]);
    };
    auto split2x4 = [&](f32x2 v01, f32x2 v23, uint2 &p0, uint2 &p1) __attribute__((always_inline)) {
        const gr_h2 a = __builtin_convertvector(v01, gr_h2), b = __builtin_convertvector(v23, gr_h2);
#if GR_MIX == 2
        const gr_h2 c = gr_rem16(v01, a), d = gr_rem16(v23, b);
#else
        const f32x2 r01 = gr_rem2(v01, a), r23 = gr_rem2(v23, b);
        const gr_h2 c = __builtin_convertvector(r01, gr_h2), d = __builtin_convertvector(r23, gr_h2);
#endif
        p0 = make_uint2(__builtin_bit_cast(unsigned, a), __builtin_bit_cast(unsigned, b));
        p1 = make_uint2(__builtin_bit_cast(unsigned, c), __builtin_bit_cast(unsigned, d));
    };
    auto stats_tile = [&](auto Tc) __attribute__((always_inline)) {
        constexpr int RT = decltype(Tc)::value;
        stats_all(GR_TILEVAL(RT));
    };
    auto fold_stats = [&]() __attribute__((always_inline)) {
        float *red = s_ring;
        float *mine = red + (wave * 64 + lane) * 36;
#pragma unroll
        for (int j = 0; j < 4; j++) {
            *reinterpret_cast<float4 *>(mine + 4 * j) = make_float4(ts[2 * j][0], ts[2 * j][1], ts[2 * j + 1][0], ts[2 * j + 1][1]);
            *reinterpret_cast<float4 *>(mine + 16 + 4 * j) = make_float4(tq[2 * j][0], tq[2 * j][1], tq[2 * j + 1][0], tq[2 * j + 1][1]);
        }
#pragma unroll
        for (int i = 0; i < 8; i++) { ts[i] = f32x2{0.f, 0.f}; tq[i] = f32x2{0.f, 0.f}; }
        LDS_BARRIER();
        const int col = tid >> 1, kind = tid & 1, cw = col & 31;
        const float *src = red + ((col >> 5) * 64 + 32 * ((cw >> 2) & 1)) * 36 + 4 * (cw >> 3) + (cw & 3) + 16 * kind;
        float s0 = 0.f, s1 = 0.f, s2 = 0.f, s3 = 0.f;
#pragma unroll
        for (int i = 0; i < 32; i += 4) { s0 += src[i * 36]; s1 += src[(i + 1) * 36]; s2 += src[(i + 2) * 36]; s3 += src[(i + 3) * 36]; }
        return (s0 + s1) + (s2 + s3);
    };
    auto fold_stats_dpp = [&]() __attribute__((always_inline)) {
        const bool b4 = (lane & 16) != 0, b3 = (lane & 8) != 0, b2 = (lane & 4) != 0, b1 = (lane & 2) != 0, b0 = (lane & 1) != 0;
        auto dpp = [&](float x, auto Ctrl) __attribute__((always_inline)) {
            return __builtin_bit_cast(float, __builtin_amdgcn_update_dpp(0, __builtin_bit_cast(int, x), decltype(Ctrl)::value, 0xF, 0xF, true));
        };
        float v16[16];
#pragma unroll
        for (int c = 0; c < 16; c++) {
            const float a = ts[c >> 1][c & 1], q_ = tq[c >> 1][c & 1];
            v16[c] = (b4 ? q_ : a) + __shfl_xor(b4 ? a : q_, 16);
        }
#pragma unroll
        for (int i = 0; i < 8; i++) { ts[i] = f32x2{0.f, 0.f}; tq[i] = f32x2{0.f, 0.f}; }
        float v8[8];
#pragma unroll
        for (int c = 0; c < 8; c++) v8[c] = (b3 ? v16[c + 8] : v16[c]) + dpp(b3 ? v16[c] : v16[c + 8], std::integral_constant<int, 0x140>{});
        float v4[4];
#pragma unroll
        for (int c = 0; c < 4; c++) v4[c] = (b2 ? v8[c + 4] : v8[c]) + dpp(b2 ? v8[c] : v8[c + 4], std::integral_constant<int, 0x141>{});
        float v2[2];
#pragma unroll
        for (int c = 0; c < 2; c++) v2[c] = (b1 ? v4[c + 2] : v4[c]) + dpp(b1 ? v4[c] : v4[c + 2], std::integral_constant<int, 0x4E>{});
        return (b0 ? v2[1] : v2[0]) + dpp(b0 ? v2[0] : v2[1], std::integral_constant<int, 0xB1>{});
    };
    unsigned char *const pl0 = s_planes, *const pl1 = s_planes + GR_TILE, *const plr = reinterpret_cast<unsigned char *>(s_ring);
    auto plane_buf = [&](int i) __attribute__((always_inline)) { return i == 0 ? pl0 : i == 1 ? pl1 : plr + (i - 2) * GR_TILE; };
    auto produce_quarter = [&](auto Tc, auto Gc, unsigned char *pbuf) __attribute__((always_inline)) {
        constexpr int rt = decltype(Tc)::value, g = decltype(Gc)::value;
        unsigned char *dst = pbuf + n * GR_ROWB + (32 * wave + 8 * g + 4 * h) * 2;
        const float *bn = rt * 32 + n_l < nrows_l ? s_bn : s_zero;
        const float4 s4 = *reinterpret_cast<const float4 *>(bn + 32 * wave + 8 * g + 4 * h);
        const float4 h4 = *reinterpret_cast<const float4 *>(bn + HD + 32 * wave + 8 * g + 4 * h);
        const f32x16 &a = GR_TILEVAL(rt);
        uint2 p0, p1;
        split2x4(f32x2{bn_relu_ss(a[4 * g], s4.x, h4.x), bn_relu_ss(a[4 * g + 1], s4.y, h4.y)},
                 f32x2{bn_relu_ss(a[4 * g + 2], s4.z, h4.z), bn_relu_ss(a[4 * g + 3], s4.w, h4.w)}, p0, p1);
        *reinterpret_cast<uint2 *>(dst) = p0;
        *reinterpret_cast<uint2 *>(dst + GR_PLANE) = p1;
    };
    auto produce_tile = [&](auto Tc, unsigned char *pbuf) __attribute__((always_inline)) {
        gr_static_for<4>([&](auto Gc) __attribute__((always_inline)) { produce_quarter(Tc, Gc, pbuf); });
        __builtin_amdgcn_sched_barrier(0);
    };
    const unsigned char *xa0 = s_planes + n * GR_ROWB + 16 * h;
#define GR_FENCE() __builtin_amdgcn_sched_barrier(0)
#define GR_PIN_V() do { } while (0)
    auto consume_tile = [&](auto Tc) __attribute__((always_inline)) {
        constexpr int RT = decltype(Tc)::value;
        constexpr int PT = RT + GR_LOOK;
        constexpr bool NEXT = (PT < GR_NT) && !(GR_ABL & 1);
        constexpr bool STATS = RT > 0 && (GR_VRES || RT - 1 < GR_NRES) && !(GR_ABL & 4);
        const unsigned char *xa = plane_buf(RT % (2 * GR_LOOK)) + n * GR_ROWB + 16 * h;
        unsigned char *pnext = plane_buf(PT % (2 * GR_LOOK));
        const float *bn = PT * 32 + n_l < nrows_l ? s_bn : s_zero;
        gr_h8 xf[2][2];
#pragma unroll
        for (int p = 0; p < 2; p++) xf[0][p] = *reinterpret_cast<const gr_h8 *>(xa + p * GR_PLANE);
        float4 s4 = make_float4(0.f, 0.f, 0.f, 0.f), h4 = s4;
        if constexpr (NEXT) {
            s4 = *reinterpret_cast<const float4 *>(bn + 32 * wave + 4 * h);
            h4 = *reinterpret_cast<const float4 *>(bn + HD + 32 * wave + 4 * h);
        }
        constexpr bool VT = GR_VRES && RT >= GR_NRES;
        f32x16 atmp;
        f32x16 &a = RT < GR_NRES ? acc[RT < GR_NRES ? RT : 0] : VT ? zs[RT >= GR_NRES ? (RT - GR_NRES) & 1 : 0] : atmp;
        if constexpr (RT + GR_LOOK + 1 >= GR_NRES && RT + GR_LOOK + 1 < GR_NT) zload(std::integral_constant<int, RT + GR_LOOK + 1 - GR_NRES>{});
        gr_static_for<4>([&](auto Pc) __attribute__((always_inline)) {
            constexpr int g = decltype(Pc)::value;
            const gr_h8 *x0 = xf[0], *x1 = xf[1];
            f32x2 v01 = {0.f, 0.f}, v23 = {0.f, 0.f}, e01 = v01, e23 = v01;
            gr_h2 p01 = {0, 0}, p23 = p01, q01 = p01, q23 = p01;
            unsigned char *dst = pnext + n * GR_ROWB + (32 * wave + 8 * g + 4 * h) * 2;
            const f32x16 &nx = GR_TILEVAL(PT < GR_NT ? PT : RT);
            const f32x16 &pv = GR_TILEVAL(RT > 0 ? RT - 1 : 0);
            auto M = [&](int ks, int wp, int xp) __attribute__((always_inline)) {
                if (GR_ABL & 2) return;
                if constexpr (VT) mfma_v(a, wf[wp][ks], (ks & 1) ? x1[xp] : x0[xp], ks == 0 && wp == 0 && xp == 1);
                else if (ks == 0 && wp == 0 && xp == 1)
                    a = __builtin_amdgcn_mfma_f32_32x32x16_f16(wf[wp][ks], x0[xp], f32x16{0.f, 0.f, 0.f, 0.f, 0.f, 0.f, 0.f, 0.f, 0.f, 0.f, 0.f, 0.f, 0.f, 0.f, 0.f, 0.f}, 0, 0, 0);
                else a = __builtin_amdgcn_mfma_f32_32x32x16_f16(wf[wp][ks], (ks & 1) ? x1[xp] : x0[xp], a, 0, 0, 0);
            };
            M(2 * g, 0, 1);
            xf[1][0] = *reinterpret_cast<const gr_h8 *>(xa + 32 * (2 * g + 1));
            if constexpr (NEXT) { v01 = gr_fma2(f32x2{nx[4 * g], nx[4 * g + 1]}, f32x2{s4.x, s4.y}, f32x2{h4.x, h4.y});
                                  v23 = gr_fma2(f32x2{nx[4 * g + 2], nx[4 * g + 3]}, f32x2{s4.z, s4.w}, f32x2{h4.z, h4.w}); }
            GR_FENCE();
            M(2 * g, 1, 0);
            xf[1][1] = *reinterpret_cast<const gr_h8 *>(xa + GR_PLANE + 32 * (2 * g + 1));
            if constexpr (NEXT) { v01 = __builtin_elementwise_max(v01, f32x2{0.f, 0.f}); v23 = __builtin_elementwise_max(v23, f32x2{0.f, 0.f}); }
            GR_FENCE();
            M(2 * g, 0, 0);
            if constexpr (NEXT) { p01 = __builtin_convertvector(v01, gr_h2); p23 = __builtin_convertvector(v23, gr_h2); }
            if constexpr (NEXT && g < 3) s4 = *reinterpret_cast<const float4 *>(bn + 32 * wave + 8 * (g + 1) + 4 * h);
            GR_FENCE();
            M(2 * g + 1, 0, 1);
            if constexpr (g < 3) xf[0][0] = *reinterpret_cast<const gr_h8 *>(xa + 32 * (2 * g + 2));
            if constexpr (NEXT && !GR_MIX) { e01 = __builtin_convertvector(p01, f32x2); e23 = __builtin_convertvector(p23, f32x2); }
            if constexpr (NEXT && g < 3) h4 = *reinterpret_cast<const float4 *>(bn + HD + 32 * wave + 8 * (g + 1) + 4 * h);
            GR_FENCE();
            M(2 * g + 1, 1, 0);
            if constexpr (g < 3) xf[0][1] = *reinterpret_cast<const gr_h8 *>(xa + GR_PLANE + 32 * (2 * g + 2));
            if constexpr (NEXT) { if constexpr (GR_MIX == 2) { q01 = gr_rem16(v01, p01); q23 = gr_rem16(v23, p23); }
                                  else if constexpr (GR_MIX == 1) { v01 = gr_rem2(v01, p01); v23 = gr_rem2(v23, p23); } else { v01 = gr_sub2(v01, e01); v23 = gr_sub2(v23, e23); }
                                  if (!(GR_ABL & 8)) *reinterpret_cast<uint2 *>(dst) = make_uint2(__builtin_bit_cast(unsigned, p01), __builtin_bit_cast(unsigned, p23));
                                  if constexpr (GR_MIX != 2) { q01 = __builtin_convertvector(v01, gr_h2); q23 = __builtin_convertvector(v23, gr_h2); } }
            GR_FENCE();
            M(2 * g + 1, 0, 0);
            if constexpr (NEXT) { if (!(GR_ABL & 8)) *reinterpret_cast<uint2 *>(dst + GR_PLANE) = make_uint2(__builtin_bit_cast(unsigned, q01), __builtin_bit_cast(unsigned, q23));
                                  else asm volatile("" :: "v"(p01), "v"(p23), "v"(q01), "v"(q23)); }
            if constexpr (STATS) { stat2(2 * g, pv[4 * g], pv[4 * g + 1]); stat2(2 * g + 1, pv[4 * g + 2], pv[4 * g + 3]); }
            GR_FENCE();
        });
        if constexpr (RT >= GR_NRES && !GR_VRES) {
            stats_all(a);
            zstore(std::integral_constant<int, RT - GR_NRES>{}, a);
            GR_FENCE();
        }
        if constexpr (!VT && GR_SETTLE) { asm volatile("s_nop 1"); GR_FENCE(); }
    };
    auto consume_tile0 = [&](auto Tc) __attribute__((always_inline)) {
        constexpr int RT = decltype(Tc)::value;
        const unsigned char *xa = xa0 + 32 * (RT & 7);
        bf16x8 x[3];
#pragma unroll
        for (int p = 0; p < 3; p++) x[p] = *reinterpret_cast<const bf16x8 *>(xa + p * GR_PLANE);
        f32x16 a = {0.f, 0.f, 0.f, 0.f, 0.f, 0.f, 0.f, 0.f, 0.f, 0.f, 0.f, 0.f, 0.f, 0.f, 0.f, 0.f};
        a = __builtin_amdgcn_mfma_f32_32x32x16_bf16(w0f[0], x[2], a, 0, 0, 0);
        a = __builtin_amdgcn_mfma_f32_32x32x16_bf16(w0f[2], x[0], a, 0, 0, 0);
        a = __builtin_amdgcn_mfma_f32_32x32x16_bf16(w0f[1], x[1], a, 0, 0, 0);
        a = __builtin_amdgcn_mfma_f32_32x32x16_bf16(w0f[0], x[1], a, 0, 0, 0);
        a = __builtin_amdgcn_mfma_f32_32x32x16_bf16(w0f[1], x[0], a, 0, 0, 0);
        a = __builtin_amdgcn_mfma_f32_32x32x16_bf16(w0f[0], x[0], a, 0, 0, 0);
        if constexpr (RT < GR_NRES) acc[RT] = a;
        else if constexpr (GR_VRES) zs[(RT - GR_NRES) & 1] = a;
        else {
            stats_all(a);
            zstore(std::integral_constant<int, RT - GR_NRES>{}, a);
        }
        if constexpr (RT > 0 && (GR_VRES || RT - 1 < GR_NRES)) stats_tile(std::integral_constant<int, RT - 1>{});
        __builtin_amdgcn_sched_barrier(0);
    };
    auto layer_boundary = [&](auto Kc) __attribute__((always_inline)) {
        constexpr int k = decltype(Kc)::value;
        GR_STAMP_AT(4 + 4 * k);
        if constexpr (GR_VRES && GR_NT > GR_NRES) {
            asm volatile("s_nop 15\n\ts_nop 15" ::: "memory");
            stats_all(zs[(GR_NT - 1 - GR_NRES) & 1]);
        }
#if GR_FOLD_DPP
        (void)fold_stats;
        const float colsum = fold_stats_dpp();
        const int kind = n >> 4, scol = 32 * wave + 8 * ((n & 15) >> 2) + 4 * h + (n & 3);
        constexpr int PAIR = 16;
#else
        const float colsum = fold_stats();
        const int kind = tid & 1, scol = tid >> 1;
        constexpr int PAIR = 1;
#endif
        const int sidx = 2 * scol + kind;
        if (k == 1) GR_STAMP_AT(2);
        const unsigned grp = blockIdx.x & 7u;
        {
            float x = colsum;
            if (!(__builtin_fabsf(x) * (kind ? A.wsinv[k] * A.wsinv[k] : A.wsinv[k]) < __builtin_ldexpf(1.0f, 51 - A.ffrac[k]))) {
                if (A.range_flag && !timed_out) __hip_atomic_store(A.range_flag, 1u, __ATOMIC_RELAXED, __HIP_MEMORY_SCOPE_SYSTEM);
                x = 0.f;
            }
            (void)__hip_atomic_fetch_add(A.stats + ((size_t)k * 8 + grp) * 256 + sidx, gr_fix_encode(x, kind ? 2 * A.wexp[k] : A.wexp[k], A.ffrac[k]),
                                         __ATOMIC_RELAXED, __HIP_MEMORY_SCOPE_AGENT);
        }
        if (k == 1) GR_STAMP_AT(3);
        const float ga = A.gamma[k][scol], be = A.beta[k][scol];
        if constexpr (k < 5) load_weights(k + 1);
        GR_STAMP_AT(5 + 4 * k);
        const unsigned long long *w0 = A.stats + (size_t)k * 8 * 256 + sidx;
        unsigned long long vw[8], want[8], ssum = 0;
#pragma unroll
        for (int j = 0; j < 8; j++) want[j] = (unsigned long long)((nblk >> 3) + ((unsigned)j < (nblk & 7u) ? 1u : 0u));
        {
            const unsigned long long t0 = __builtin_amdgcn_s_memrealtime();
            for (;;) {
#pragma unroll
                for (int j = 0; j < 8; j++) vw[j] = __hip_atomic_load(w0 + (size_t)j * 256, __ATOMIC_RELAXED, __HIP_MEMORY_SCOPE_AGENT);
                bool done = true;
                ssum = 0;
#pragma unroll
                for (int j = 0; j < 8; j++) { done = done && (vw[j] >> 58) == want[j]; ssum += vw[j] & GR_FIX_PAYLOAD; }
                if (__builtin_amdgcn_ballot_w64(!done) == 0ull) break;
                if (__builtin_amdgcn_s_memrealtime() - t0 > 400000ull) {
                    __hip_atomic_store(A.fail, 1u, __ATOMIC_RELAXED, __HIP_MEMORY_SCOPE_SYSTEM);
                    timed_out = true;
                    break;
                }
                __builtin_amdgcn_s_sleep(2);
            }
            GR_STAMP_AT(6 + 4 * k);
            const double tot = gr_fix_decode(ssum, nblk, A.ffrac[k]);
            const double oth = __shfl_xor(tot, PAIR);
            if (!kind) {
                const double mean = tot * A.inv_rows;
                double var = oth * A.inv_rows - mean * mean;
                if (var < 0) var = 0;
                const float rstd = 1.0f / sqrtf((float)(var + BN_EPS));
                const float s = rstd * ga;
                s_bn[scol] = s * A.wsinv[k];
                s_bn[HD + scol] = be - (float)mean * s;
            }
        }
        LDS_BARRIER();
        GR_STAMP_AT(7 + 4 * k);
    };

    GR_STAMP_AT(0);
#pragma unroll
    for (int p = 0; p < 3; p++) w0f[p] = __builtin_bit_cast(bf16x8, w0pre[p]);
    LDS_BARRIER();
    GR_STAMP_AT(1);
    {
        const float *s_feat = s_ring;
        auto produce0 = [&](int rt) __attribute__((always_inline)) {
            const int r = 8 * wave + (lane >> 3), fk = lane & 7, row = rt * 32 + r;
            const int fo = fk < 6 ? 2 * fk : 0;
            const unsigned cp = s_ellc[row];
            const unsigned r0 = cp & 0xffffu, r1 = cp >> 16;
            const int deg = 1 + (r0 != 0xffffu) + (r1 != 0xffffu);
            const float inv = deg == 1 ? 1.0f : deg == 2 ? 0.5f : (1.0f / 3.0f);
            const float w0 = s_ellv0[row], w1 = s_ellv1[row];
            const int n0 = r0 != 0xffffu ? (int)r0 : row, n1 = r1 != 0xffffu ? (int)r1 : row;
            const float2 o = *reinterpret_cast<const float2 *>(s_feat + row * 12 + fo);
            const float2 x = *reinterpret_cast<const float2 *>(s_feat + n0 * 12 + fo);
            const float2 y = *reinterpret_cast<const float2 *>(s_feat + n1 * 12 + fo);
            float v[4] = {__builtin_fmaf(w1, y.x, __builtin_fmaf(w0, x.x, o.x)) * inv, __builtin_fmaf(w1, y.y, __builtin_fmaf(w0, x.y, o.y)) * inv, 0.f, 0.f};
            if (row >= nrows) { v[0] = 0.f; v[1] = 0.f; }
            uint2 p0, p1, p2;
            split3x4(v, p0, p1, p2);
            unsigned char *d = s_planes + r * GR_ROWB + 32 * (rt & 7) + 4 * fk;
            if (fk < 6) {
                *reinterpret_cast<unsigned *>(d) = p0.x;
                *reinterpret_cast<unsigned *>(d + GR_PLANE) = p1.x;
                *reinterpret_cast<unsigned *>(d + 2 * GR_PLANE) = p2.x;
            }
        };
        gr_static_for<(GR_NT + 7) / 8>([&](auto Cc) __attribute__((always_inline)) {
            constexpr int C = decltype(Cc)::value;
            constexpr int NTC = GR_NT - 8 * C < 8 ? GR_NT - 8 * C : 8;
#pragma unroll
            for (int i = 0; i < NTC; i++) produce0(8 * C + i);
            LDS_BARRIER();
            __builtin_amdgcn_sched_barrier(0);
            gr_static_for<NTC>([&](auto Ic) __attribute__((always_inline)) {
                constexpr int RT = 8 * C + decltype(Ic)::value;
                consume_tile0(std::integral_constant<int, RT>{});
            });
            LDS_BARRIER();
            __builtin_amdgcn_sched_barrier(0);
        });
    }
    layer_boundary(std::integral_constant<int, 0>{});

    gr_static_for<5>([&](auto Lc) __attribute__((always_inline)) {
        constexpr int layer = decltype(Lc)::value + 1;
#ifndef GR_KEEP_MASKS
        asm volatile("" : "+s"(nrows_l), "+v"(n_l));
#endif
        if constexpr (layer != 3) {
            gr_static_for<GR_LOOK>([&](auto Ic) __attribute__((always_inline)) { produce_tile(Ic, plane_buf(decltype(Ic)::value)); });
            LDS_BARRIER();
            unsigned *cnt = s_cnt + (layer - 1) * (GR_NT / GR_GRP);
            gr_static_for<GR_NT>([&](auto Tc) __attribute__((always_inline)) {
                constexpr int RT = decltype(Tc)::value;
                constexpr int step = RT / GR_GRP, back = GR_LOOK / GR_GRP;
                if constexpr (GR_LOOK > GR_GRP && RT % GR_GRP == 0 && step >= back) {
                    while (__builtin_amdgcn_readfirstlane(__hip_atomic_load(&cnt[step - back], __ATOMIC_RELAXED, __HIP_MEMORY_SCOPE_WORKGROUP)) < 4u)
                        __builtin_amdgcn_s_sleep(1);
                    asm volatile("" ::: "memory");
                    __builtin_amdgcn_sched_barrier(0);
                }
                consume_tile(Tc);
                GR_PIN_V();
                if constexpr (RT % GR_GRP == GR_GRP - 1) {
                    if constexpr (GR_LOOK > GR_GRP) {
                        asm volatile("" ::: "memory");
                        if (lane == 0) __hip_atomic_fetch_add(&cnt[step], 1u, __ATOMIC_RELAXED, __HIP_MEMORY_SCOPE_WORKGROUP);
                    } else LDS_BARRIER();
                }
                __builtin_amdgcn_sched_barrier(0);
            });
            if constexpr (GR_LOOK > GR_GRP) LDS_BARRIER();
            static_assert(GR_NT % GR_GRP == 0 && GR_GRP >= 1 && (GR_LOOK == GR_GRP || GR_LOOK == 2 * GR_GRP) && GR_LOOK <= GR_NRES, "tile groups");
        } else {
            auto write_h = [&](auto Tc) __attribute__((always_inline)) {
                constexpr int rt = decltype(Tc)::value;
                float *base = s_ring + ((rt % GR_RING) * 32 + n) * HD;
                gr_static_for<4>([&](auto Gc) __attribute__((always_inline)) {
                    constexpr int g = decltype(Gc)::value;
                    const float *bn = rt * 32 + n_l < nrows_l ? s_bn : s_zero;
                    const float4 s4 = *reinterpret_cast<const float4 *>(bn + 32 * wave + 8 * g + 4 * h);
                    const float4 h4 = *reinterpret_cast<const float4 *>(bn + HD + 32 * wave + 8 * g + 4 * h);
                    const f32x16 &a = GR_TILEVAL(rt);
                    const int ch = (8 * wave + 2 * g + h) ^ (n & 7);
                    *reinterpret_cast<float4 *>(base + 4 * ch) = make_float4(bn_relu_ss(a[4 * g], s4.x, h4.x), bn_relu_ss(a[4 * g + 1], s4.y, h4.y),
                                                                             bn_relu_ss(a[4 * g + 2], s4.z, h4.z), bn_relu_ss(a[4 * g + 3], s4.w, h4.w));
                });
                __builtin_amdgcn_sched_barrier(0);
            };
            auto ring_row = [&](int R) __attribute__((always_inline)) {
                const int t = R >> 5;
                return ((t - GR_RING * ((t * 43) >> 8)) * 32 + (R & 31)) * HD;
            };
            struct AggRow { const float *po, *px, *py; float w0, w1, inv; int s0, s1, s2; };
            auto agg_row = [&](int RT) __attribute__((always_inline)) {
                AggRow r;
                const int row = RT * 32 + n_l;
                const unsigned cp = s_ellc[row];
                const unsigned r0 = cp & 0xffffu, r1 = cp >> 16;
                r.w0 = s_ellv0[row]; r.w1 = s_ellv1[row];
                const int deg = 1 + (r0 != 0xffffu) + (r1 != 0xffffu);
                r.inv = deg == 1 ? 1.0f : deg == 2 ? 0.5f : (1.0f / 3.0f);
                const int n0 = r0 != 0xffffu ? (int)r0 : row, n1 = r1 != 0xffffu ? (int)r1 : row;
                r.po = s_ring + ((RT % GR_RING) * 32 + n) * HD; r.px = s_ring + ring_row(n0); r.py = s_ring + ring_row(n1);
                r.s0 = n & 7; r.s1 = n0 & 7; r.s2 = n1 & 7;
                return r;
            };
            auto agg_quarter_standalone = [&](const AggRow &r, int g, unsigned char *dst) __attribute__((always_inline)) {
                const int chl = 8 * wave + 2 * g + h;
                const float4 o = *reinterpret_cast<const float4 *>(r.po + 4 * (chl ^ r.s0));
                const float4 x = *reinterpret_cast<const float4 *>(r.px + 4 * (chl ^ r.s1));
                const float4 y = *reinterpret_cast<const float4 *>(r.py + 4 * (chl ^ r.s2));
                const f32x2 W0 = {r.w0, r.w0}, W1 = {r.w1, r.w1}, IV = {r.inv, r.inv};
                const f32x2 v01 = gr_mul2(gr_fma2(W1, f32x2{y.x, y.y}, gr_fma2(W0, f32x2{x.x, x.y}, f32x2{o.x, o.y})), IV);
                const f32x2 v23 = gr_mul2(gr_fma2(W1, f32x2{y.z, y.w}, gr_fma2(W0, f32x2{x.z, x.w}, f32x2{o.z, o.w})), IV);
                uint2 p0, p1;
                split2x4(v01, v23, p0, p1);
                *reinterpret_cast<uint2 *>(dst + 16 * g) = p0;
                *reinterpret_cast<uint2 *>(dst + 16 * g + GR_PLANE) = p1;
            };
            auto consume_agg = [&](auto Tc) __attribute__((always_inline)) {
                constexpr int RT = decltype(Tc)::value;
                constexpr bool NEXT = RT + 1 < GR_NT && !(GR_ABL & 1);
                constexpr bool WH = RT + 4 < GR_NT && !(GR_ABL & 1);
                constexpr int WT = WH ? RT + 4 : RT;
                constexpr bool STATS = RT > 0 && (GR_VRES || RT - 1 < GR_NRES) && !(GR_ABL & 4);
                constexpr bool VT = GR_VRES && RT >= GR_NRES;
                const unsigned char *xa = xa0 + (RT & 1) * GR_TILE;
                gr_h8 xf[2][2];
#pragma unroll
                for (int p = 0; p < 2; p++) xf[0][p] = *reinterpret_cast<const gr_h8 *>(xa + p * GR_PLANE);
                AggRow r = agg_row(NEXT ? RT + 1 : RT);
                unsigned char *dst = s_planes + ((RT + 1) & 1) * GR_TILE + n * GR_ROWB + (32 * wave + 4 * h) * 2;
                const float *bnw = WT * 32 + n_l < nrows_l ? s_bn : s_zero;
                float *hbase = s_ring + ((WT % GR_RING) * 32 + n) * HD;
                float4 s4 = make_float4(0.f, 0.f, 0.f, 0.f), h4 = s4;
                if constexpr (WH) {
                    s4 = *reinterpret_cast<const float4 *>(bnw + 32 * wave + 4 * h);
                    h4 = *reinterpret_cast<const float4 *>(bnw + HD + 32 * wave + 4 * h);
                }
                f32x16 atmp;
                f32x16 &a = RT < GR_NRES ? acc[RT < GR_NRES ? RT : 0] : VT ? zs[RT >= GR_NRES ? (RT - GR_NRES) & 1 : 0] : atmp;
                if constexpr (RT + 6 >= GR_NRES && RT + 6 < GR_NT) zload(std::integral_constant<int, RT + 6 - GR_NRES>{});
                gr_static_for<4>([&](auto Pc) __attribute__((always_inline)) {
                    constexpr int g = decltype(Pc)::value;
                    const gr_h8 *x0 = xf[0], *x1 = xf[1];
                    const f32x16 &wv = GR_TILEVAL(WT);
                    const f32x16 &pv = GR_TILEVAL(RT > 0 ? RT - 1 : 0);
                    const int chl = 8 * wave + 2 * g + h;
                    float4 o = make_float4(0.f, 0.f, 0.f, 0.f), x = o, y = o;
                    f32x2 v01 = {0.f, 0.f}, v23 = v01, e01 = v01, e23 = v01, u01 = v01, u23 = v01;
                    gr_h2 p01 = {0, 0}, p23 = p01, q01 = p01, q23 = p01;
                    const f32x2 W0 = {r.w0, r.w0}, W1 = {r.w1, r.w1}, IV = {r.inv, r.inv};
                    auto M = [&](int ks, int wp, int xp) __attribute__((always_inline)) {
                        if (!(GR_ABL & 2)) {
                            if constexpr (VT) mfma_v(a, wf[wp][ks], (ks & 1) ? x1[xp] : x0[xp], g == 0 && ks == 0 && wp == 0 && xp == 1);
                            else if (g == 0 && ks == 0 && wp == 0 && xp == 1)
                                a = __builtin_amdgcn_mfma_f32_32x32x16_f16(wf[wp][ks], x0[xp], f32x16{0.f, 0.f, 0.f, 0.f, 0.f, 0.f, 0.f, 0.f, 0.f, 0.f, 0.f, 0.f, 0.f, 0.f, 0.f, 0.f}, 0, 0, 0);
                            else a = __builtin_amdgcn_mfma_f32_32x32x16_f16(wf[wp][ks], (ks & 1) ? x1[xp] : x0[xp], a, 0, 0, 0);
                        }
                    };
                    M(2 * g, 0, 1);
                    xf[1][0] = *reinterpret_cast<const gr_h8 *>(xa + 32 * (2 * g + 1));
                    if constexpr (NEXT) { o = *reinterpret_cast<const float4 *>(r.po + 4 * (chl ^ r.s0)); x = *reinterpret_cast<const float4 *>(r.px + 4 * (chl ^ r.s1));
                                          y = *reinterpret_cast<const float4 *>(r.py + 4 * (chl ^ r.s2)); }
                    if constexpr (STATS) { stat2(2 * g, pv[4 * g], pv[4 * g + 1]); stat2(2 * g + 1, pv[4 * g + 2], pv[4 * g + 3]); }
                    GR_FENCE();
                    M(2 * g, 1, 0);
                    xf[1][1] = *reinterpret_cast<const gr_h8 *>(xa + GR_PLANE + 32 * (2 * g + 1));
                    if constexpr (WH) { u01 = __builtin_elementwise_max(gr_fma2(f32x2{wv[4 * g], wv[4 * g + 1]}, f32x2{s4.x, s4.y}, f32x2{h4.x, h4.y}), f32x2{0.f, 0.f});
                                        u23 = __builtin_elementwise_max(gr_fma2(f32x2{wv[4 * g + 2], wv[4 * g + 3]}, f32x2{s4.z, s4.w}, f32x2{h4.z, h4.w}), f32x2{0.f, 0.f}); }
                    GR_FENCE();
                    M(2 * g, 0, 0);
                    if constexpr (WH) *reinterpret_cast<float4 *>(hbase + 4 * (chl ^ (n & 7))) = make_float4(u01[0], u01[1], u23[0], u23[1]);
                    if constexpr (NEXT) { v01 = gr_fma2(W0, f32x2{x.x, x.y}, f32x2{o.x, o.y}); v23 = gr_fma2(W0, f32x2{x.z, x.w}, f32x2{o.z, o.w}); }
                    if constexpr (WH && g < 3) s4 = *reinterpret_cast<const float4 *>(bnw + 32 * wave + 8 * (g + 1) + 4 * h);
                    GR_FENCE();
                    M(2 * g + 1, 0, 1);
                    if constexpr (g < 3) xf[0][0] = *reinterpret_cast<const gr_h8 *>(xa + 32 * (2 * g + 2));
                    if constexpr (NEXT) { v01 = gr_fma2(W1, f32x2{y.x, y.y}, v01); v23 = gr_fma2(W1, f32x2{y.z, y.w}, v23); }
                    if constexpr (WH && g < 3) h4 = *reinterpret_cast<const float4 *>(bnw + HD + 32 * wave + 8 * (g + 1) + 4 * h);
                    GR_FENCE();
                    M(2 * g + 1, 1, 0);
                    if constexpr (g < 3) xf[0][1] = *reinterpret_cast<const gr_h8 *>(xa + GR_PLANE + 32 * (2 * g + 2));
                    if constexpr (NEXT) { v01 = gr_mul2(v01, IV); v23 = gr_mul2(v23, IV); p01 = __builtin_convertvector(v01, gr_h2); p23 = __builtin_convertvector(v23, gr_h2);
                                          if constexpr (!GR_MIX) { e01 = __builtin_convertvector(p01, f32x2); e23 = __builtin_convertvector(p23, f32x2); } }
                    GR_FENCE();
                    M(2 * g + 1, 0, 0);
                    if constexpr (NEXT) { if constexpr (GR_MIX == 2) { q01 = gr_rem16(v01, p01); q23 = gr_rem16(v23, p23); }
                                          else { if constexpr (GR_MIX) { v01 = gr_rem2(v01, p01); v23 = gr_rem2(v23, p23); } else { v01 = gr_sub2(v01, e01); v23 = gr_sub2(v23, e23); } q01 = __builtin_convertvector(v01, gr_h2); q23 = __builtin_convertvector(v23, gr_h2); }
                                          *reinterpret_cast<uint2 *>(dst + 16 * g) = make_uint2(__builtin_bit_cast(unsigned, p01), __builtin_bit_cast(unsigned, p23));
                                          *reinterpret_cast<uint2 *>(dst + 16 * g + GR_PLANE) = make_uint2(__builtin_bit_cast(unsigned, q01), __builtin_bit_cast(unsigned, q23)); }
                    GR_FENCE();
                });
                if constexpr (RT >= GR_NRES && !GR_VRES) {
                    stats_all(a);
                    zstore(std::integral_constant<int, RT - GR_NRES>{}, a);
                    GR_FENCE();
                }
                if constexpr (!VT && GR_SETTLE) { asm volatile("s_nop 1"); GR_FENCE(); }
            };
            write_h(std::integral_constant<int, 0>{}); write_h(std::integral_constant<int, 1>{}); write_h(std::integral_constant<int, 2>{});
            write_h(std::integral_constant<int, 3>{});
            LDS_BARRIER();
            {
                const AggRow r = agg_row(0);
                unsigned char *dst = s_planes + n * GR_ROWB + (32 * wave + 4 * h) * 2;
#pragma unroll
                for (int g = 0; g < 4; g++) agg_quarter_standalone(r, g, dst);
            }
            LDS_BARRIER();
            __builtin_amdgcn_sched_barrier(0);
            gr_static_for<GR_NT>([&](auto Tc) __attribute__((always_inline)) {
                consume_agg(Tc);
                LDS_BARRIER();
                __builtin_amdgcn_sched_barrier(0);
            });
        }
        layer_boundary(std::integral_constant<int, layer>{});
    });

    GR_STAMP_AT(30);
    {
        float *s_part = reinterpret_cast<float *>(s_planes);
        static_assert(2 * GR_NT * 2 * HD * 4 <= 2 * GR_TILE + 4096, "partial pool sums: plane buffers + 4 KB");
        float *tb = s_ring + 1024 + wave * (2 * 32 * 36);
        float *s_wtab = s_ring + 1024 + 4 * (2 * 32 * 36);
        for (int i = tid; i < 17 * 16; i += 256) s_wtab[i] = (i & 15) < (i >> 4) ? 1.0f : 0.0f;
        unsigned warm_word = 0;
        if (A.nwarm > 0) {
            unsigned l = (blockIdx.x >> 3) * 256u + (unsigned)tid;
            const unsigned char *wp = reinterpret_cast<const unsigned char *>(A.warm[0]);
            bool found = false;
            for (int w = 0; w < A.nwarm; w++) {
                const unsigned nl = A.warm_lines[w];
                if (!found && l < nl) { wp = reinterpret_cast<const unsigned char *>(A.warm[w]) + (size_t)l * 128; found = true; }
                if (!found) l -= nl;
            }
            warm_word = *reinterpret_cast<const unsigned *>(wp);
        }
        float4 S[4], Hs[4];
#pragma unroll
        for (int g = 0; g < 4; g++) {
            S[g] = *reinterpret_cast<const float4 *>(s_bn + 32 * wave + 8 * g + 4 * h);
            Hs[g] = *reinterpret_cast<const float4 *>(s_bn + HD + 32 * wave + 8 * g + 4 * h);
        }
        if constexpr (GR_NT - GR_NRES >= 1) zload(std::integral_constant<int, 0>{});
        if constexpr (GR_NT - GR_NRES >= 2) zload(std::integral_constant<int, 1>{});
        const int c = lane & 31;
        int left = ((16 * h) / T + 1) * T - 16 * h;
        int slot[GR_NT];
#ifndef GR_KEEP_MASKS
        asm volatile("" : "+v"(n_l));
#endif
#pragma unroll
        for (int rt = 0; rt < GR_NT; rt++) slot[rt] = (GR_ABL & 32) ? -1 : s_rowcand[rt * 32 + n_l];
        LDS_BARRIER();
        GR_STAMP_AT(28);
        float x[16];
        float4 w0, w1, w2, w3;
        auto pool_load = [&](int rt) __attribute__((always_inline)) {
            const float *rb = tb + (rt & 1) * (32 * 36) + (16 * h) * 36 + c;
#pragma unroll
            for (int i = 0; i < 16; i++) x[i] = rb[i * 36];
            const float4 *wt = reinterpret_cast<const float4 *>(s_wtab + (left < 16 ? left : 16) * 16);
            w0 = wt[0]; w1 = wt[1]; w2 = wt[2]; w3 = wt[3];
        };
        auto pool_math = [&](int rt) __attribute__((always_inline)) {
            f32x2 sa2 = gr_fma2(f32x2{x[0], x[1]}, f32x2{w0.x, w0.y}, f32x2{0.f, 0.f});
            sa2 = gr_fma2(f32x2{x[2], x[3]}, f32x2{w0.z, w0.w}, sa2);
            sa2 = gr_fma2(f32x2{x[4], x[5]}, f32x2{w1.x, w1.y}, sa2);
            sa2 = gr_fma2(f32x2{x[6], x[7]}, f32x2{w1.z, w1.w}, sa2);
            sa2 = gr_fma2(f32x2{x[8], x[9]}, f32x2{w2.x, w2.y}, sa2);
            sa2 = gr_fma2(f32x2{x[10], x[11]}, f32x2{w2.z, w2.w}, sa2);
            sa2 = gr_fma2(f32x2{x[12], x[13]}, f32x2{w3.x, w3.y}, sa2);
            sa2 = gr_fma2(f32x2{x[14], x[15]}, f32x2{w3.z, w3.w}, sa2);
            const f32x2 t2 = gr_add2(gr_add2(gr_add2(f32x2{x[0], x[1]}, f32x2{x[2], x[3]}), gr_add2(f32x2{x[4], x[5]}, f32x2{x[6], x[7]})),
                                     gr_add2(gr_add2(f32x2{x[8], x[9]}, f32x2{x[10], x[11]}), gr_add2(f32x2{x[12], x[13]}, f32x2{x[14], x[15]})));
            const float tot = t2[0] + t2[1];
            const float sa = sa2[0] + sa2[1];
            float *pp = s_part + ((2 * rt + h) * 2) * HD + 32 * wave + c;
            pp[0] = left >= 16 ? tot : sa; pp[HD] = left >= 16 ? 0.f : tot - sa;
            left -= 32;
            if (left <= 0) left += T;
            if (left <= 0) left += T;
        };
        gr_static_for<GR_NT>([&](auto Tc) __attribute__((always_inline)) {
            constexpr int rt = decltype(Tc)::value;
            const f32x16 &a = GR_TILEVAL(rt);
            if constexpr (rt > 0) { if (!(GR_ABL & 16)) pool_load(rt - 1); }
            float4 v[4];
#pragma unroll
            for (int g = 0; g < 4; g++) {
                const f32x2 lo = __builtin_elementwise_max(gr_fma2(f32x2{a[4 * g], a[4 * g + 1]}, f32x2{S[g].x, S[g].y}, f32x2{Hs[g].x, Hs[g].y}), f32x2{0.f, 0.f});
                const f32x2 hi = __builtin_elementwise_max(gr_fma2(f32x2{a[4 * g + 2], a[4 * g + 3]}, f32x2{S[g].z, S[g].w}, f32x2{Hs[g].z, Hs[g].w}), f32x2{0.f, 0.f});
                v[g] = make_float4(lo[0], lo[1], hi[0], hi[1]);
            }
            float *wb = tb + (rt & 1) * (32 * 36);
#pragma unroll
            for (int g = 0; g < 4; g++) *reinterpret_cast<float4 *>(wb + n * 36 + 8 * g + 4 * h) = v[g];
            if (slot[rt] >= 0) {
                float *d = A.cand_feat + ((size_t)inst0 * A.J + slot[rt]) * HD + 32 * wave + 4 * h;
#pragma unroll
                for (int g = 0; g < 4; g++) *reinterpret_cast<float4 *>(d + 8 * g) = v[g];
            }
            if (A.h_nodes && rt * 32 + n_l < nrows) {
                float *d = A.h_nodes + (grow0 + rt * 32 + n_l) * HD + 32 * wave + 4 * h;
#pragma unroll
                for (int g = 0; g < 4; g++) *reinterpret_cast<float4 *>(d + 8 * g) = v[g];
            }
            if constexpr (rt > 0) { if (!(GR_ABL & 16)) pool_math(rt - 1); }
            __builtin_amdgcn_sched_barrier(0);
        });
        if (!(GR_ABL & 16)) { pool_load(GR_NT - 1); pool_math(GR_NT - 1); }
        asm volatile("" :: "v"(warm_word));
        GR_STAMP_AT(29);
        LDS_BARRIER();
        const float invT = 1.0f / (float)T;
        static_assert(GR_MAXT <= 65, "an instance spans at most five 16-row chunks");
        for (int item = tid; item < ninst * HD; item += 256) {
            const int inst = item >> 7, col = item & (HD - 1);
            const int r0 = inst * T, k0 = r0 >> 4, k1 = (r0 + T - 1) >> 4;
            float pv[5];
#pragma unroll
            for (int kk = 0; kk < 5; kk++) {
                const int k = k0 + kk < k1 ? k0 + kk : k1;
                pv[kk] = s_part[(2 * k + (16 * k < r0 ? 1 : 0)) * HD + col];
            }
            float sum = 0.f;
#pragma unroll
            for (int kk = 0; kk < 5; kk++) sum = k0 + kk <= k1 ? sum + pv[kk] : sum;
            A.pooled[(size_t)inst0 * HD + item] = sum * invT;
        }
        if (A.candidate && s_flag[1]) {
            __threadfence();
            __syncthreads();
            for (int i = wave; i < ninst * A.J; i += 4) {
                const int cnd = A.candidate[(size_t)inst0 * A.J + i];
                if (cnd < 0 || cnd >= T) continue;
                const int win = s_rowcand[(i / A.J) * T + cnd];
                if (win != i) {
                    const float2 x = *reinterpret_cast<const float2 *>(A.cand_feat + ((size_t)inst0 * A.J + win) * HD + 2 * lane);
                    *reinterpret_cast<float2 *>(A.cand_feat + ((size_t)inst0 * A.J + i) * HD + 2 * lane) = x;
                }
            }
        }
    }
    GR_STAMP_AT(31);
}
#endif
```

### e2e-mappo-for-mt-fjsp_amd/encoder.py

```python
import ctypes as C
import math

import os

import numpy as np
import torch

from . import capi

H = 128
FAMILIES = ["gin0_agg_linear12", "gin0_stats_only", "gin0_moments", "gin0_bn_gemm", "gin_gemm_bn_relu", "gin_gemm_stats_only", "gin_gemm_pool", "cand_fixup", "gin_gemm_pair", "gin_gemm_agg", "job_pool_gather", "heads", "head_gemm", "gat3", "mach_bn_pool",
            "sample", "small", "gin_inst", "gat_inst", "gin_resident", "heads_gat3", "heads_gat3_heads"]


def available():
    try:
        capi.lib()
        return torch.cuda.is_available()
    except Exception:
        return False


def random_init_weights(seed=0, with_critic=False):
    g = torch.Generator().manual_seed(seed)
# ... 3 lines not shown
        w = (torch.rand(out, inp, generator=g) * 2 - 1) * b
        return (w, (torch.rand(out, generator=g) * 2 - 1) * b) if bias else (w, None)

    ja, ma = {}, {}
    pre = "encoder.feature_extract."
    for l, inp in ((0, 12), (1, H)):
        for i, (o, k) in enumerate(((H, inp), (H, H), (H, H))):
            w, b = lin(o, k)
            ja[f"{pre}mlps.{l}.linears.{i}.weight"], ja[f"{pre}mlps.{l}.linears.{i}.bias"] = w, b
        for i in range(2):
            ja[f"{pre}mlps.{l}.batch_norms.{i}.weight"] = torch.ones(H); ja[f"{pre}mlps.{l}.batch_norms.{i}.bias"] = torch.zeros(H)
        ja[f"{pre}batch_norms.{l}.weight"] = torch.ones(H); ja[f"{pre}batch_norms.{l}.bias"] = torch.zeros(H)
    ja["_input"] = torch.rand(H, generator=g) * 2 - 1
    for name, d, out_last in (("o_policy", ja, 1), ("job_critic", ja, 2), ("m_policy", ma, 1), ("machine_critic", ma, 2)):
        first_in = 3 * H if "policy" in name else H
        for i, (o, k) in enumerate(((H, first_in), (H, H), (out_last, H))):
            w, b = lin(o, k)
            d[f"{name}.linears.{i}.weight"], d[f"{name}.linears.{i}.bias"] = w, b
    ma["bn.weight"] = torch.ones(H); ma["bn.bias"] = torch.zeros(H)
    ma["m_fea_1_fcl.weight"] = lin(H, 6, False)[0]; ma["m_fea_2_fcl.weight"] = lin(H, 8, False)[0]
    ma["gat_layer.W"] = torch.randn(H, H, generator=g) * math.sqrt(2.0 / (H + H))
    ma["gat_layer.a"] = torch.randn(1, 2 * H, 1, generator=g) * math.sqrt(2.0 / (2 * H + 1 * 1))
    if not with_critic:
        return {k: v.numpy() for k, v in ja.items()}, {k: v.numpy() for k, v in ma.items()}
    gc = {}
    for l, inp in ((0, 12), (1, H)):
        for i, (o, k) in enumerate(((H, inp), (H, H), (H, H))):
            w, b = lin(o, k)
            gc[f"{pre}mlps.{l}.linears.{i}.weight"], gc[f"{pre}mlps.{l}.linears.{i}.bias"] = w, b
        for i in range(2):
            gc[f"{pre}mlps.{l}.batch_norms.{i}.weight"] = torch.ones(H); gc[f"{pre}mlps.{l}.batch_norms.{i}.bias"] = torch.zeros(H)
        gc[f"{pre}batch_norms.{l}.weight"] = torch.ones(H); gc[f"{pre}batch_norms.{l}.bias"] = torch.zeros(H)
    for i, (o, k) in enumerate(((H, 2 * H), (H, H), (4, H))):
        w, b = lin(o, k)
        gc[f"critic.linears.{i}.weight"], gc[f"critic.linears.{i}.bias"] = w, b
    gc["bn.weight"] = torch.ones(H); gc["bn.bias"] = torch.zeros(H)
    gc["m_fea_1_fcl.weight"] = lin(H, 6, False)[0]; gc["m_fea_2_fcl.weight"] = lin(H, 8, False)[0]
    gc["gat_layer.W"] = torch.randn(H, H, generator=g) * math.sqrt(2.0 / (H + H))
    gc["gat_layer.a"] = torch.randn(1, 2 * H, 1, generator=g) * math.sqrt(2.0 / (2 * H + 1 * 1))
    return tuple({k: v.numpy() for k, v in d.items()} for d in (ja, ma, gc))


class Encoder:
    def __init__(self, n_job, n_machine, batch, device=0, obs_dtype="f32"):
        if not torch.cuda.is_available():
            raise RuntimeError("the encoder needs a GPU (MI355X); there is no CPU fallback")
        self.L = capi.lib()
        self.J, self.M, self.B = n_job, n_machine, batch
        self.T = n_job * n_machine
        self.device = torch.device("cuda", device)
        self.obs_f32 = obs_dtype in ("f32", torch.float32, np.float32)
        cfg = capi.EncoderConfig(n_job, n_machine, batch, H, capi.OBS_F32 if self.obs_f32 else capi.OBS_F64, device)
        h = C.c_void_p()
        capi.check(self.L.mtfjsp_encoder_create(C.byref(cfg), C.byref(h)), None, enc=True)
        self.h = h
        B, J, M = batch, n_job, n_machine
        f32 = dict(dtype=torch.float32, device=self.device)
        self.job_prob = torch.zeros(B, J, **f32); self.h_pooled_o = torch.zeros(B, H, **f32); self.job_v = torch.zeros(B, 2, **f32)
        self.mch_prob = torch.zeros(B, M, **f32); self.h_pooled_m = torch.zeros(B, H, **f32); self.mach_v = torch.zeros(B, 2, **f32)
        self.use_current_stream()

    def use_current_stream(self):
        s = torch.cuda.current_stream(self.device).cuda_stream
        capi.check(self.L.mtfjsp_encoder_set_stream(self.h, C.c_void_p(s)), self.h, enc=True)

    def close(self):
        if getattr(self, "h", None):
            self.L.mtfjsp_encoder_destroy(self.h)
            self.h = None

    def __del__(self):
        try:
            self.close()
        except Exception:
            pass

    def load_weights(self, job_actor, machine_actor, global_critic=None):
        for prefix, d in (("job_actor.", job_actor), ("machine_actor.", machine_actor), ("global_critic.", global_critic or {})):
            for k, v in d.items():
                if "running_" in k or "num_batches_tracked" in k:
                    continue
                a = v.detach().cpu().numpy() if torch.is_tensor(v) else np.asarray(v)
                a = np.ascontiguousarray(a, np.float32)
                capi.check(self.L.mtfjsp_encoder_load_weight_host(self.h, (prefix + k).encode(), a.ctypes.data, a.size), self.h, enc=True)
        capi.check(self.L.mtfjsp_encoder_weights_ready(self.h), self.h, enc=True)

    def job_actor_forward(self, tasks_fea, ell_col, ell_val, candidate, job_mask, h_m_prev=None, h_nodes=None, v_out=None):
        capi.check(self.L.mtfjsp_job_actor_forward(
            self.h, tasks_fea.data_ptr(), ell_col.data_ptr(), ell_val.data_ptr(), candidate.data_ptr(), job_mask.data_ptr(),
            h_m_prev.data_ptr() if h_m_prev is not None else 0, self.job_prob.data_ptr(), self.h_pooled_o.data_ptr(),
            (v_out if v_out is not None else self.job_v).data_ptr(), h_nodes.data_ptr() if h_nodes is not None else 0), self.h, enc=True)
        return self.job_prob, self.h_pooled_o, (v_out if v_out is not None else self.job_v)

    def machine_actor_forward(self, m_fea1, m_fea2, h_pooled_o, mmask, v_out=None):
        capi.check(self.L.mtfjsp_machine_actor_forward(
            self.h, m_fea1.data_ptr(), m_fea2.data_ptr(), h_pooled_o.data_ptr(), mmask.data_ptr(), self.mch_prob.data_ptr(),
            self.h_pooled_m.data_ptr(), (v_out if v_out is not None else self.mach_v).data_ptr()), self.h, enc=True)
        return self.mch_prob, self.h_pooled_m, (v_out if v_out is not None else self.mach_v)

    def global_critic_forward(self, tasks_fea, ell_col, ell_val, m_fea1, m_fea2, out=None):
        if out is None:
            out = torch.empty(self.B, 4, dtype=torch.float32, device=self.device)
        capi.check(self.L.mtfjsp_global_critic_forward(self.h, tasks_fea.data_ptr(), ell_col.data_ptr(), ell_val.data_ptr(),
                                                       m_fea1.data_ptr(), m_fea2.data_ptr(), out.data_ptr()), self.h, enc=True)
        return out

    def sample(self, prob, greedy, seed, counter, idx_out, logp_out=None, gather_from=None, gathered_out=None):
        capi.check(self.L.mtfjsp_sample_categorical(
            self.h, prob.data_ptr(), prob.shape[1], int(greedy), seed, counter, idx_out.data_ptr(),
            logp_out.data_ptr() if logp_out is not None else 0, gather_from.data_ptr() if gather_from is not None else 0,
            gathered_out.data_ptr() if gathered_out is not None else 0), self.h, enc=True)

    def set_bn_mode(self, per_instance):
        capi.check(self.L.mtfjsp_encoder_set_bn_mode(self.h, 1 if per_instance else 0), self.h, enc=True)

    def set_product_mode(self, f32_instruction_mask=0):
        capi.check(self.L.mtfjsp_encoder_set_product_mode(self.h, int(f32_instruction_mask)), self.h, enc=True)

    def set_stats_reduce(self, fn, global_batch=0):
        if fn is None:
            capi.check(self.L.mtfjsp_encoder_set_stats_reduce(self.h, None, None, 0), self.h, enc=True)
            self._reduce_cb = None
            return

        def tramp(user, ptr, n):
            try:
                fn(int(ptr), int(n))
                return 0
            except Exception:
                import traceback
                traceback.print_exc()
                return 1

        self._reduce_cb = C.CFUNCTYPE(C.c_int, C.c_void_p, C.c_void_p, C.c_int32)(tramp)
        capi.check(self.L.mtfjsp_encoder_set_stats_reduce(self.h, C.cast(self._reduce_cb, C.c_void_p), None, int(global_batch)), self.h, enc=True)

    def set_deferred_poll(self, deferred):
        capi.check(self.L.mtfjsp_encoder_set_deferred_poll(self.h, 1 if deferred else 0), self.h, enc=True)

    def check(self):
        r = C.c_int32(0)
        capi.check(self.L.mtfjsp_encoder_check(self.h, C.byref(r)), self.h, enc=True)
        return bool(r.value)

    def resident_failures(self):
        n = C.c_int64(0)
        capi.check(self.L.mtfjsp_encoder_resident_failures(self.h, C.byref(n)), self.h, enc=True)
        return int(n.value)

    def peek_nodes(self):
        import numpy as np
        out = np.empty((self.B * self.M, 128), dtype=np.float32)
        capi.check(self.L.mtfjsp_encoder_peek_nodes_host(self.h, out.ctypes.data, out.size), self.h, enc=True)
        return out

    def range_fallbacks(self):
        n, m = C.c_int64(0), C.c_int32(0)
        capi.check(self.L.mtfjsp_encoder_range_fallbacks(self.h, C.byref(n), C.byref(m)), self.h, enc=True)
        return int(n.value), int(m.value)

    def arm_selection(self, which, greedy, seed, counter, idx_out, logp_out=None, gather_from=None, gathered_out=None):
        capi.check(self.L.mtfjsp_encoder_arm_selection(
            self.h, which, int(greedy), seed, counter, idx_out.data_ptr(), logp_out.data_ptr() if logp_out is not None else 0,
            gather_from.data_ptr() if gather_from is not None else 0, gathered_out.data_ptr() if gathered_out is not None else 0),
            self.h, enc=True)

    def arm_mfea1(self, ctx):
        capi.check(self.L.mtfjsp_encoder_arm_mfea1(self.h, C.byref(ctx)), self.h, enc=True)

    def arm_machine_heads(self, prob, h_pooled, machine_v):
        capi.check(self.L.mtfjsp_encoder_arm_machine_heads(self.h, prob.data_ptr(), h_pooled.data_ptr(), machine_v.data_ptr()), self.h, enc=True)

    def fused_launches(self):
        n = C.c_int64(0)
        capi.check(self.L.mtfjsp_encoder_fused_launches(self.h, C.byref(n)), self.h, enc=True)
        return int(n.value)

    def arm_env_step(self, params):
        capi.check(self.L.mtfjsp_encoder_arm_env_step(self.h, params, len(params)), self.h, enc=True)

    def arm_values_only(self):
        capi.check(self.L.mtfjsp_encoder_arm_values_only(self.h), self.h, enc=True)

    def env_step_fused(self):
        return bool(self.L.mtfjsp_encoder_env_step_fused(self.h))

    def timing_begin(self):
        capi.check(self.L.mtfjsp_encoder_timing_begin(self.h), self.h, enc=True)

    def timing_end(self):
        out = {}
        for fam in FAMILIES:
            ms = C.c_double(); n = C.c_int64()
            capi.check(self.L.mtfjsp_encoder_timing_query(self.h, fam.encode(), C.byref(ms), C.byref(n)), self.h, enc=True)
            if n.value:
                out[fam] = {"ms_total": ms.value, "launches": n.value}
        ms = C.c_double(); n = C.c_int64()
        capi.check(self.L.mtfjsp_encoder_timing_end(self.h, C.byref(ms), C.byref(n)), self.h, enc=True)
        return out


class ActorPair:

    def __init__(self, n_job, n_machine, batch, device=0, obs_dtype="f32", weights=None, greedy=False, seed=0):
        self.enc = Encoder(n_job, n_machine, batch, device=device, obs_dtype=obs_dtype)
        w = weights if weights is not None else random_init_weights(seed)
        self.enc.load_weights(w[0], w[1], w[2] if len(w) > 2 else None)
        self.has_critic = len(w) > 2
        self.greedy, self.seed = greedy, seed
        self._mf_ctx, self._mf_env, self._mf_own = None, None, None
        self.last_mfea1 = self.last_mmask = None
        self.n_env_fused = 0
        self.fuse_env = bool(os.environ.get("MTFJSP_FUSED_ENV"))
        self.fused = not os.environ.get("MTFJSP_NO_FUSED_SELECT")
        self.fuse_mheads = not os.environ.get("MTFJSP_NO_FUSED_MHEADS")
        self.values_only_terminal = not os.environ.get("MTFJSP_NO_VALUES_ONLY")
        self.fuse_env3 = bool(os.environ.get("MTFJSP_FUSED_ENV3"))
        dev = self.enc.device
        self.job_logp = torch.zeros(batch, dtype=torch.float32, device=dev)
        self.mch_logp = torch.zeros(batch, dtype=torch.float32, device=dev)
        self.have_hm = False

    def begin_episode(self):
        self.have_hm = False

    def act(self, env, counter, task_idx, mach_idx, job_idx, jv_out=None, mv_out=None, job_logp=None, mach_logp=None,
            after_mfea1=None, force=None, env_step=None, mfea1_out=None, mmask_out=None):
        e = self.enc
        jl = job_logp if job_logp is not None else self.job_logp
        ml = mach_logp if mach_logp is not None else self.mch_logp
        hm = e.h_pooled_m if self.have_hm else None
        fuse_mfea1 = self.fused and force is None
        armed_m = armed_e = False
        if self.fused:
            e.arm_selection(0, self.greedy, self.seed, 2 * counter, job_idx, jl, env.candidate, task_idx)
            if fuse_mfea1:
                if self._mf_env is not env:
                    self._mf_ctx, self._mf_env = env.mfea1_context(), env
                    self._mf_own = (self._mf_ctx.m_fea1_out, self._mf_ctx.mmask_out)
                redirect = mfea1_out is not None and mmask_out is not None
                self._mf_ctx.m_fea1_out = mfea1_out.data_ptr() if redirect else self._mf_own[0]
                self._mf_ctx.mmask_out = mmask_out.data_ptr() if redirect else self._mf_own[1]
                e.arm_mfea1(self._mf_ctx)
                if self.fuse_mheads and not (self.fuse_env and env_step is not None):
                    e.arm_selection(1, self.greedy, self.seed, 2 * counter + 1, mach_idx, ml)
                    e.arm_machine_heads(e.mch_prob, e.h_pooled_m, mv_out if mv_out is not None else e.mach_v)
                    armed_m = True
                    if self.fuse_env3 and env_step is not None:
                        params = env.step_params(task_idx, mach_idx, *env_step)
                        if params is not None:
                            e.arm_env_step(params)
                            armed_e = True
            prob, h_o, _ = e.job_actor_forward(env.tasks_fea, env.ell_col, env.ell_val, env.candidate, env.job_mask, hm, v_out=jv_out)
        else:
            prob, h_o, _ = e.job_actor_forward(env.tasks_fea, env.ell_col, env.ell_val, env.candidate, env.job_mask, hm, v_out=jv_out)
            e.sample(prob, self.greedy, self.seed, 2 * counter, job_idx, jl, env.candidate, task_idx)
        if force is not None:
            task_idx.copy_(force[0])
            if len(force) > 2:
                job_idx.copy_(force[2])
        mf1, mmk = env.m_fea1, env.mmask
        if not fuse_mfea1:
            env.observe_mfea1(task_idx)
            if after_mfea1 is not None:
                after_mfea1(env)
        elif mfea1_out is not None and mmask_out is not None:
            mf1, mmk = mfea1_out, mmask_out
        elif after_mfea1 is not None:
            after_mfea1(env)
        self.last_mfea1, self.last_mmask = mf1, mmk
        stepped = False
        if self.fused:
            if not armed_m:
                e.arm_selection(1, self.greedy, self.seed, 2 * counter + 1, mach_idx, ml)
            if self.fuse_env and env_step is not None and force is None:
                params = env.step_params(task_idx, mach_idx, *env_step)
                if params is not None:
                    e.arm_env_step(params)
            e.machine_actor_forward(mf1, env.m_fea2, h_o, mmk, v_out=mv_out)
            stepped = (armed_e or (self.fuse_env and env_step is not None and force is None)) and e.env_step_fused()
        else:
            mprob, _, _ = e.machine_actor_forward(mf1, env.m_fea2, h_o, mmk, v_out=mv_out)
            e.sample(mprob, self.greedy, self.seed, 2 * counter + 1, mach_idx, ml)
        if force is not None:
            mach_idx.copy_(force[1])
        self.have_hm = True
        self.n_env_fused += int(stepped)
        return stepped

    def terminal_values(self, env, prev_job_mask, jv_out, mv_out):
        e = self.enc
        hm = e.h_pooled_m if self.have_hm else None
        if self.values_only_terminal:
            e.arm_values_only()
        _, h_o, _ = e.job_actor_forward(env.tasks_fea, env.ell_col, env.ell_val, env.candidate, prev_job_mask, hm, v_out=jv_out)
        mf1 = self.last_mfea1 if self.last_mfea1 is not None else env.m_fea1
        mmk = self.last_mmask if self.last_mmask is not None else env.mmask
        e.machine_actor_forward(mf1, env.m_fea2, h_o, mmk, v_out=mv_out)

    def timing_begin(self):
        self.enc.timing_begin()

    def timing_end(self):
        return self.enc.timing_end()

    def roofline(self, name, kd, B):
# ... 100 lines not shown
```

### include/mtfjsp.h

```cpp
#ifndef MTFJSP_H
#define MTFJSP_H

#include <stddef.h>
#include <stdint.h>

#ifdef __cplusplus
extern "C" {
#endif

typedef struct mtfjsp_env *mtfjsp_handle_t;
typedef struct mtfjsp_encoder *mtfjsp_encoder_t;

typedef enum {
    MTFJSP_OK = 0,
    MTFJSP_ERR_ARG = -1,
    MTFJSP_ERR_STATE = -2,
    MTFJSP_ERR_HIP = -3,
    MTFJSP_ERR_ACTION = -4,
    MTFJSP_ERR_RETRY = -5
} mtfjsp_status;

enum { MTFJSP_OBS_F64 = 0, MTFJSP_OBS_F32 = 1 };

enum {
// ... 16 lines not shown
    double gamma;
    double w_mk, w_ec, w_tt;
    double scaling_divisor;
} mtfjsp_config_t;

typedef struct {
    void *tasks_fea;
    int32_t *ell_col;
    float *ell_val;
    void *m_fea2;
    double *info;
    double *raw;
    int32_t *candidate;
    uint8_t *job_mask;
    int32_t *status;
} mtfjsp_obs_t;

int mtfjsp_create(const mtfjsp_config_t *cfg, mtfjsp_handle_t *out);
int mtfjsp_destroy(mtfjsp_handle_t h);
const char *mtfjsp_last_error(mtfjsp_handle_t h);
int mtfjsp_set_stream(mtfjsp_handle_t h, void *hip_stream);
int mtfjsp_synchronize(mtfjsp_handle_t h);

int mtfjsp_alloc_obs(mtfjsp_handle_t h, mtfjsp_obs_t *out);
int mtfjsp_bind_obs(mtfjsp_handle_t h, const mtfjsp_obs_t *obs);
int mtfjsp_snapshot_obs(mtfjsp_handle_t h, const mtfjsp_obs_t *dst);
int mtfjsp_snapshot_obs2(mtfjsp_handle_t h, const mtfjsp_obs_t *dst, const mtfjsp_obs_t *dst2, float *reward_out);

int mtfjsp_load_instances(mtfjsp_handle_t h, const double *t, const double *p, const double *tt,
                          const int32_t *shop_of_machine);
int mtfjsp_load_instances_host(mtfjsp_handle_t h, const double *t_host, const double *p_host,
                               const double *tt_host, const int32_t *shop_host);
int mtfjsp_generate_instances(mtfjsp_handle_t h, uint64_t seed, uint64_t first_instance, const double *scope9);
int mtfjsp_read_instances_host(mtfjsp_handle_t h, double *t, double *p, double *tt, int32_t *shop);

int mtfjsp_scaler_init(mtfjsp_handle_t h);
int mtfjsp_scaler_reset_returns(mtfjsp_handle_t h);
int mtfjsp_scaler_reset_returns_masked_host(mtfjsp_handle_t h, const uint8_t *mask_host);

int mtfjsp_reset(mtfjsp_handle_t h, const double *w3);
int mtfjsp_draw_reward_weights(mtfjsp_handle_t h, uint64_t seed, uint64_t episode, double *w3_out);
int mtfjsp_reset_episode(mtfjsp_handle_t h, uint64_t seed, uint64_t episode, double *w3_out, int32_t reset_returns);
int mtfjsp_reset_host(mtfjsp_handle_t h, const double *w3_host);

int mtfjsp_step(mtfjsp_handle_t h, const int32_t *task_idx, const int32_t *mach_idx);
int mtfjsp_step_record(mtfjsp_handle_t h, const int32_t *task_idx, const int32_t *mach_idx, float *r4_out, float *done_out);
int32_t mtfjsp_step_params_bytes(void);
int mtfjsp_step_params(mtfjsp_handle_t h, const int32_t *task_idx, const int32_t *mach_idx, float *r4_out, float *done_out,
                       void *params_out, int32_t params_bytes);
const char *mtfjsp_step_kernel_name(mtfjsp_handle_t h);
const char *mtfjsp_step_kernel_name_for(int32_t n_job, int32_t n_machine, int32_t batch, int32_t obs_f32, int64_t lds_max,
                                        int32_t *group_out, int64_t *lds_bytes_out, int32_t *overridden_out);
int mtfjsp_step_host(mtfjsp_handle_t h, const int32_t *task_idx_host, const int32_t *mach_idx_host);

int mtfjsp_observe_mfea1(mtfjsp_handle_t h, const int32_t *task_idx, const uint8_t *mmask_in,
                         void *out, uint8_t *mmask_out);

int mtfjsp_random_actions(mtfjsp_handle_t h, uint64_t seed, uint64_t counter, int32_t *task_idx,
                          int32_t *mach_idx, int32_t *job_idx);

enum { MTFJSP_FORK_INSTANCE = 1, MTFJSP_FORK_STATE = 2, MTFJSP_FORK_OBS = 4 };
int mtfjsp_fork(mtfjsp_handle_t dst, mtfjsp_handle_t src, const int32_t *src_index, int32_t flags);

int mtfjsp_lookahead_expand(mtfjsp_handle_t scratch, mtfjsp_handle_t src, int32_t *task_c, int32_t *mach_c);
int mtfjsp_lookahead_select(mtfjsp_handle_t scratch, mtfjsp_handle_t src, int32_t column, int32_t *task_out, int32_t *mach_out,
                            int32_t *job_out, double *best_out);

int mtfjsp_pdr_plan(mtfjsp_handle_t h, const int32_t *o_rule, const int32_t *m_rule, const int32_t *mor_order, uint64_t seed,
                    int32_t *task_out, int32_t *mach_out);

int mtfjsp_export_dense_adj(mtfjsp_handle_t h, double *out);
int mtfjsp_export_dense_adj_host(mtfjsp_handle_t h, double *out_host);
int mtfjsp_valid_action_mask(mtfjsp_handle_t h, uint8_t *out);
enum {
    MTFJSP_STATE_MACHINE = 0,
    MTFJSP_STATE_START = 1,
    MTFJSP_STATE_FINISH = 2,
    MTFJSP_STATE_ROUTES = 3,
    MTFJSP_STATE_PREV_COSTS = 4,
    MTFJSP_STATE_SCALER = 5,
    MTFJSP_STATE_W3 = 6
};
int mtfjsp_read_state_host(mtfjsp_handle_t h, int which, void *out_host);
int mtfjsp_set_scaler_state_host(mtfjsp_handle_t h, int32_t first, int32_t count, const double *state17);
int mtfjsp_copy_to_host(mtfjsp_handle_t h, void *dst_host, const void *src_dev, size_t nbytes);

int mtfjsp_gae(mtfjsp_handle_t h, int32_t S, const float *r, int64_t r_ss, int64_t r_sb, const float *v, int64_t v_ss, int64_t v_sb,
               const float *v_next, int64_t n_ss, int64_t n_sb, const float *done, float gamma, float lambda, float *adv);
int mtfjsp_normalize_advantages(mtfjsp_handle_t h, int32_t K, int32_t K_total, int32_t world, int32_t rank, int32_t S, const float *gathered, float eps,
                                const float *const *values, const int64_t *value_stride_s, const int64_t *value_stride_b,
                                float *norm_out, float *targets_out, float *full_out);
int mtfjsp_pack_views(mtfjsp_handle_t h, int32_t K, int32_t S, const float *const *src, const int64_t *stride_s, const int64_t *stride_b, float *out);

int mtfjsp_timing_begin(mtfjsp_handle_t h);
int mtfjsp_timing_end(mtfjsp_handle_t h, double *step_ms_total, int64_t *step_launches);

int mtfjsp_footprint_copy(mtfjsp_handle_t h, size_t read_bytes, size_t write_bytes, int32_t access_bytes, int32_t grid, int32_t reps,
                          double *avg_us_out, double *min_us_out);

typedef struct {
    int32_t n_job, n_machine, batch;
    int32_t hidden;
    int32_t obs_dtype;
    int32_t device_id;
} mtfjsp_encoder_config_t;

int mtfjsp_encoder_create(const mtfjsp_encoder_config_t *cfg, mtfjsp_encoder_t *out);
int mtfjsp_encoder_destroy(mtfjsp_encoder_t e);
const char *mtfjsp_encoder_last_error(mtfjsp_encoder_t e);
int mtfjsp_encoder_set_stream(mtfjsp_encoder_t e, void *hip_stream);
int mtfjsp_encoder_load_weight_host(mtfjsp_encoder_t e, const char *name, const float *data_host, int64_t numel);
int mtfjsp_encoder_weights_ready(mtfjsp_encoder_t e);

int mtfjsp_job_actor_forward(mtfjsp_encoder_t e, const void *tasks_fea, const int32_t *ell_col,
                             const float *ell_val, const int32_t *candidate, const uint8_t *job_mask,
                             const float *h_m_prev, float *prob, float *h_pooled, float *job_v, float *h_nodes);
int mtfjsp_machine_actor_forward(mtfjsp_encoder_t e, const void *m_fea1, const void *m_fea2,
                                 const float *h_pooled_o, const uint8_t *mmask, float *prob, float *h_pooled,
                                 float *machine_v);
int mtfjsp_global_critic_forward(mtfjsp_encoder_t e, const void *tasks_fea, const int32_t *ell_col, const float *ell_val,
                                 const void *m_fea1, const void *m_fea2, float *value4);
int mtfjsp_sample_categorical(mtfjsp_encoder_t e, const float *prob, int32_t n, int32_t greedy, uint64_t seed,
                              uint64_t counter, int32_t *idx_out, float *logp_out, const int32_t *gather_from,
                              int32_t *gathered_out);
typedef struct {
    const double *t, *p, *tt, *mean3;
    const int32_t *shop;
    const void *link;
    void *m_fea1_out;
    uint8_t *mmask_out;
    int32_t T, M, obs_f32;
    const void *m_fea2;
} mtfjsp_mfea1_ctx_t;
int mtfjsp_get_mfea1_context(mtfjsp_handle_t h, void *m_fea1_out, uint8_t *mmask_out, mtfjsp_mfea1_ctx_t *ctx);
int mtfjsp_encoder_arm_machine_heads(mtfjsp_encoder_t e, float *prob, float *h_pooled, float *machine_v);
int mtfjsp_encoder_fused_launches(mtfjsp_encoder_t e, int64_t *three_in_one_out);
int mtfjsp_encoder_arm_values_only(mtfjsp_encoder_t e);
int mtfjsp_encoder_set_bn_mode(mtfjsp_encoder_t e, int32_t per_instance);
typedef int (*mtfjsp_stats_reduce_fn)(void *user, double *sums, int32_t count);
int mtfjsp_encoder_set_stats_reduce(mtfjsp_encoder_t e, mtfjsp_stats_reduce_fn fn, void *user, int64_t global_batch);
int mtfjsp_encoder_set_deferred_poll(mtfjsp_encoder_t e, int32_t deferred);
int mtfjsp_encoder_set_product_mode(mtfjsp_encoder_t e, int32_t f32_instruction_mask);
int mtfjsp_encoder_arm_selection(mtfjsp_encoder_t e, int32_t which, int32_t greedy, uint64_t seed, uint64_t counter,
                                 int32_t *idx_out, float *logp_out, const int32_t *gather_from, int32_t *gathered_out);
int mtfjsp_encoder_arm_mfea1(mtfjsp_encoder_t e, const mtfjsp_mfea1_ctx_t *ctx);
int mtfjsp_encoder_arm_env_step(mtfjsp_encoder_t e, const void *params, int32_t params_bytes);
int mtfjsp_encoder_env_step_fused(mtfjsp_encoder_t e);
int mtfjsp_hostgen_infeasible(uint32_t *key, int32_t *pos, int64_t samples, int32_t T, int32_t M, int64_t first, int64_t count, double *t);
int mtfjsp_hostgen_transport(uint32_t *key, int32_t *pos, int64_t samples, int32_t M, const int64_t *shop_of_machine,
                             double in_lo, double in_hi, double out_hi, int64_t first, int64_t count, double *tt);
int mtfjsp_encoder_check(mtfjsp_encoder_t e, int32_t *gin_resident_out);
int mtfjsp_encoder_range_fallbacks(mtfjsp_encoder_t e, int64_t *count_out, int32_t *product_mode_out);
int mtfjsp_encoder_peek_nodes_host(mtfjsp_encoder_t e, float *out_host, int64_t count);
int mtfjsp_encoder_resident_failures(mtfjsp_encoder_t e, int64_t *count_out);
int mtfjsp_encoder_timing_begin(mtfjsp_encoder_t e);
int mtfjsp_encoder_timing_end(mtfjsp_encoder_t e, double *ms_total, int64_t *launches);
int mtfjsp_encoder_timing_query(mtfjsp_encoder_t e, const char *family, double *ms_total, int64_t *launches);

#ifdef __cplusplus
}
#endif
#endif
```

Measured before the change: 20.59 million.

## Transpose last GIN layer MFMA output to lane-per-column and restructure final pooling phase

For the last GIN layer, the resident kernel now swaps the MFMA operands so each lane holds one output column. This lets BatchNorm statistics fold with a single cross-half permute, and the scale and shift stay in registers instead of going through LDS and a barrier. The final phase is rewritten to do segmented mean pooling with a mask table, and to stage candidate features in an LDS image before writing them out with coalesced float4 stores. It also adds a debug dump mode for pre-activation values, a host accessor for cand_feat, and a build variant that disables the path. The cost is more LDS layout complexity and a constraint that the spilled-tile build must turn the path off.

Result: slower. 20.28 million (-1.5%).

```diff
diff --git a/__graft_entry__.py b/__graft_entry__.py
--- a/__graft_entry__.py
+++ b/__graft_entry__.py
@@ -15,6 +15,7 @@
     capi = import_module("e2e-mappo-for-mt-fjsp_amd.capi")
     capi.lib()
     print("variant:", _build.build_variant("funcs", ["-DMTFJSP_BODY_FUNCS=3"]))
+    print("variant:", _build.build_variant("lastt0", ["-DGR_LAST_T=0"]))
     from oracle import env_oracle
     print("oracle:", env_oracle.build(force=True))
     print("built", lib)
diff --git a/e2e-mappo-for-mt-fjsp_amd/capi.py b/e2e-mappo-for-mt-fjsp_amd/capi.py
--- a/e2e-mappo-for-mt-fjsp_amd/capi.py
+++ b/e2e-mappo-for-mt-fjsp_amd/capi.py
@@ -111,6 +111,7 @@
     "mtfjsp_encoder_resident_failures": (_I, [_VP, C.POINTER(C.c_int64)]),
     "mtfjsp_encoder_range_fallbacks": (_I, [_VP, C.POINTER(C.c_int64), C.POINTER(C.c_int32)]),
     "mtfjsp_encoder_peek_nodes_host": (_I, [_VP, _VP, C.c_int64]),
+    "mtfjsp_encoder_cand_feat_host": (_I, [_VP, _VP, C.c_int64, C.c_int32]),
     "mtfjsp_encoder_timing_begin": (_I, [_VP]),
     "mtfjsp_encoder_timing_end": (_I, [_VP, C.POINTER(C.c_double), C.POINTER(C.c_int64)]),
     "mtfjsp_encoder_timing_query": (_I, [_VP, C.c_char_p, C.POINTER(C.c_double), C.POINTER(C.c_int64)]),
diff --git a/e2e-mappo-for-mt-fjsp_amd/csrc/mtfjsp_encoder.hip b/e2e-mappo-for-mt-fjsp_amd/csrc/mtfjsp_encoder.hip
--- a/e2e-mappo-for-mt-fjsp_amd/csrc/mtfjsp_encoder.hip
+++ b/e2e-mappo-for-mt-fjsp_amd/csrc/mtfjsp_encoder.hip
@@ -2555,6 +2555,7 @@
     volatile unsigned *res_fail_host = nullptr;
     unsigned *range_flag = nullptr;
     long long range_fallbacks = 0;
+    bool res_dump_z5 = false;
     bool res_eligible = false;
     long long res_failures = 0, res_launches = 0;
     long long res_fail_at = getenv("MTFJSP_GIN_RES_FAIL_AT") ? atoll(getenv("MTFJSP_GIN_RES_FAIL_AT")) : 0;
@@ -2783,6 +2784,7 @@
                 if (!rc && hipMemset(e->res_stats, 0, (size_t)2 * GR_STATS_SET * 8) == hipSuccess &&
                     hipMemset(e->res_bar, 0, (size_t)17 * 16 * 8) == hipSuccess) {
                     e->res_ipc = ipc; e->res_grid = grid; e->res_eligible = true;
+                    e->res_dump_z5 = getenv("MTFJSP_GIN_DUMP_Z5") != nullptr;
                     e->res_ok = res_census(e);
                 }
             }
@@ -3300,6 +3302,7 @@
     a.bar = e->res_bar; a.epoch = e->res_epoch++; a.fail = e->res_fail; a.range_flag = e->range_flag;
     a.candidate = candidate; a.pooled = h_pooled; a.cand_feat = cand_feat; a.h_nodes = h_nodes; a.zspill = e->res_zspill;
     a.inv_rows = 1.0 / ((double)B * (double)T);
+    a.dump_z5 = e->res_dump_z5 ? 1 : 0;
     if (pre == "job_actor." && e->warm_heads) {
         const char *keys[9] = {"job_actor.o_policy.linears.0.weight", "job_actor.job_critic.linears.0.weight", "job_actor.o_policy.linears.1.weight",
                                "job_actor.job_critic.linears.1.weight", "machine_actor.gat_layer.W", "machine_actor.m_policy.linears.0.weight",
@@ -4061,6 +4064,15 @@
     HIPCHK(e, hipMemcpy(out_host, e->node, (size_t)count * sizeof(float), hipMemcpyDeviceToHost));
     return MTFJSP_OK;
 }
+extern "C" int mtfjsp_encoder_cand_feat_host(mtfjsp_encoder_t e, float *host, int64_t count, int32_t to_device)
+{
+    if (!e || !host || count < 0 || count > (int64_t)e->cfg.batch * e->cfg.n_job * HD) return MTFJSP_ERR_ARG;
+    HIPCHK(e, hipSetDevice(e->cfg.device_id));
+    HIPCHK(e, hipStreamSynchronize(e->stream));
+    if (to_device) HIPCHK(e, hipMemcpy(e->cand_feat, host, (size_t)count * sizeof(float), hipMemcpyHostToDevice));
+    else HIPCHK(e, hipMemcpy(host, e->cand_feat, (size_t)count * sizeof(float), hipMemcpyDeviceToHost));
+    return MTFJSP_OK;
+}
 extern "C" int mtfjsp_encoder_range_fallbacks(mtfjsp_encoder_t e, int64_t *count_out, int32_t *product_mode_out)
 {
     if (!e || !count_out) return MTFJSP_ERR_ARG;
diff --git a/e2e-mappo-for-mt-fjsp_amd/csrc/mtfjsp_gin_resident.h b/e2e-mappo-for-mt-fjsp_amd/csrc/mtfjsp_gin_resident.h
--- a/e2e-mappo-for-mt-fjsp_amd/csrc/mtfjsp_gin_resident.h
+++ b/e2e-mappo-for-mt-fjsp_amd/csrc/mtfjsp_gin_resident.h
@@ -41,6 +41,9 @@
 #endif
 #ifndef GR_STAT_ASM
 #define GR_STAT_ASM 0
+#endif
+#ifndef GR_LAST_T
+#define GR_LAST_T 1
 #endif
 #ifndef GR_PK
 #define GR_PK 1
@@ -76,6 +79,7 @@
     const void *warm[GR_MAXWARM];
     unsigned warm_lines[GR_MAXWARM];
     int nwarm;
+    int dump_z5;
 };
 #define GR_STATS_PART (6 * 8 * HD * 2)
 #define GR_STATS_SET GR_STATS_PART
@@ -97,7 +101,19 @@
 #define GR_OFF_ZERO (GR_OFF_CAND + GR_ROWS * 4)
 #define GR_OFF_FLAG (GR_OFF_ZERO + 2 * HD * 4)
 #define GR_OFF_CNT (GR_OFF_FLAG + 64)
+#if GR_LAST_T
+#define GR_OFF_ROFF ((GR_OFF_CNT + 5 * (GR_NT / GR_GRP) * 4 + 12 + 15) & ~15)
+#define GR_OFF_SLOTOK (GR_OFF_ROFF + GR_ROWS * 4)
+#define GR_LDS_BYTES (GR_OFF_SLOTOK + GR_MAXCAND * 4)
+#define GR_FIN_NPART (GR_ROWS / GR_MINT + 2)
+#define GR_FIN_OFF_WTAB (GR_FIN_NPART * 2 * HD * 4)
+#define GR_FIN_OFF_IMG (GR_FIN_OFF_WTAB + 33 * 32 * 4)
+#define GR_IMGCAP ((GR_OFF_ELLC - GR_FIN_OFF_IMG) / (HD * 4) - 1)
+static_assert(GR_VRES, "GR_LAST_T: the spilled-tile build (GR_VRES 0) takes its BatchNorm sums in the lane = row form only; build it with -DGR_LAST_T=0");
+static_assert(GR_FIN_OFF_IMG % 16 == 0 && GR_IMGCAP >= 96, "final phase: candidate image");
+#else
 #define GR_LDS_BYTES (GR_OFF_CNT + 5 * (GR_NT / GR_GRP) * 4 + 12)
+#endif
 static size_t gin_res_lds_bytes() { return (size_t)GR_LDS_BYTES; }
 static_assert(GR_LDS_BYTES <= 160 * 1024, "resident GIN kernel: LDS budget");
 
@@ -136,6 +152,12 @@
     asm("v_fma_mixlo_f16 %0, %1, -1.0, %2 op_sel_hi:[1,0,0]" : "=v"(r) : "v"(pp), "v"(v[0]));
     asm("v_fma_mixhi_f16 %0, %1, -1.0, %2 op_sel:[1,0,0] op_sel_hi:[1,0,0]" : "+v"(r) : "v"(pp), "v"(v[1]));
     return __builtin_bit_cast(gr_h2, r);
+}
+__device__ __forceinline__ float gr_hadd(f32x2 v)
+{
+    float r;
+    asm("v_add_f32 %0, %1, %2" : "=v"(r) : "v"(v[0]), "v"(v[1]));
+    return r;
 }
 template <typename F, int... I>
 __device__ __forceinline__ void gr_static_for_impl(F &&f, std::integer_sequence<int, I...>) { (f(std::integral_constant<int, I>{}), ...); }
@@ -212,6 +234,10 @@
     float *s_zero = reinterpret_cast<float *>(smem + GR_OFF_ZERO);
     unsigned *s_flag = reinterpret_cast<unsigned *>(smem + GR_OFF_FLAG);
     unsigned *s_cnt = reinterpret_cast<unsigned *>(smem + GR_OFF_CNT);
+#if GR_LAST_T
+    unsigned *s_rowoff = reinterpret_cast<unsigned *>(smem + GR_OFF_ROFF);
+    int *s_slotok = reinterpret_cast<int *>(smem + GR_OFF_SLOTOK);
+#endif
     const int tid = threadIdx.x, wave = __builtin_amdgcn_readfirstlane(tid >> 6), lane = tid & 63;
     const int n = lane & 31, h = lane >> 5;
     const unsigned nblk = gridDim.x + A.expect_extra;
@@ -291,6 +317,14 @@
         }
         if (tid == 0) s_flag[1] = 0u;
         if (tid < 5 * (GR_NT / GR_GRP)) s_cnt[tid] = 0u;
+#if GR_LAST_T
+#pragma unroll
+        for (int k = 0; k < (GR_MAXCAND + 255) / 256; k++) {
+            const int i = tid + 256 * k, c = cand_pre[k];
+            const bool ok = A.candidate && i < ninst * A.J && c >= 0 && c < T;
+            if (i < GR_MAXCAND) s_slotok[i] = ok ? (i / A.J) * T + c : -1;
+        }
+#endif
         for (int i = tid; i < 2 * GR_TILE / 16; i += 256) reinterpret_cast<float4 *>(s_planes)[i] = make_float4(0.f, 0.f, 0.f, 0.f);
         if (A.candidate) {
             LDS_BARRIER();
@@ -437,8 +471,9 @@
     const unsigned char *xa0 = s_planes + n * GR_ROWB + 16 * h;
 #define GR_FENCE() __builtin_amdgcn_sched_barrier(0)
 #define GR_PIN_V() do { } while (0)
-    auto consume_tile = [&](auto Tc) __attribute__((always_inline)) {
+    auto consume_tile = [&](auto Tc, auto Lc) __attribute__((always_inline)) {
         constexpr int RT = decltype(Tc)::value;
+        constexpr bool LT = GR_LAST_T && decltype(Lc)::value == 5;
         constexpr int PT = RT + GR_LOOK;
         constexpr bool NEXT = (PT < GR_NT) && !(GR_ABL & 1);
         constexpr bool STATS = RT > 0 && (GR_VRES || RT - 1 < GR_NRES) && !(GR_ABL & 4);
@@ -467,10 +502,14 @@
             const f32x16 &pv = GR_TILEVAL(RT > 0 ? RT - 1 : 0);
             auto M = [&](int ks, int wp, int xp) __attribute__((always_inline)) {
                 if (GR_ABL & 2) return;
-                if constexpr (VT) mfma_v(a, wf[wp][ks], (ks & 1) ? x1[xp] : x0[xp], ks == 0 && wp == 0 && xp == 1);
-                else if (ks == 0 && wp == 0 && xp == 1)
-                    a = __builtin_amdgcn_mfma_f32_32x32x16_f16(wf[wp][ks], x0[xp], f32x16{0.f, 0.f, 0.f, 0.f, 0.f, 0.f, 0.f, 0.f, 0.f, 0.f, 0.f, 0.f, 0.f, 0.f, 0.f, 0.f}, 0, 0, 0);
-                else a = __builtin_amdgcn_mfma_f32_32x32x16_f16(wf[wp][ks], (ks & 1) ? x1[xp] : x0[xp], a, 0, 0, 0);
+                const gr_h8 &xo = (ks & 1) ? x1[xp] : x0[xp];
+                const bool first = ks == 0 && wp == 0 && xp == 1;
+                if constexpr (VT) { if constexpr (LT) mfma_v(a, xo, wf[wp][ks], first); else mfma_v(a, wf[wp][ks], xo, first); }
+                else {
+                    const f32x16 c = first ? f32x16{0.f, 0.f, 0.f, 0.f, 0.f, 0.f, 0.f, 0.f, 0.f, 0.f, 0.f, 0.f, 0.f, 0.f, 0.f, 0.f} : a;
+                    if constexpr (LT) a = __builtin_amdgcn_mfma_f32_32x32x16_f16(xo, wf[wp][ks], c, 0, 0, 0);
+                    else a = __builtin_amdgcn_mfma_f32_32x32x16_f16(wf[wp][ks], xo, c, 0, 0, 0);
+                }
             };
             M(2 * g, 0, 1);
             xf[1][0] = *reinterpret_cast<const gr_h8 *>(xa + 32 * (2 * g + 1));
@@ -500,7 +539,8 @@
             M(2 * g + 1, 0, 0);
             if constexpr (NEXT) { if (!(GR_ABL & 8)) *reinterpret_cast<uint2 *>(dst + GR_PLANE) = make_uint2(__builtin_bit_cast(unsigned, q01), __builtin_bit_cast(unsigned, q23));
                                   else asm volatile("" :: "v"(p01), "v"(p23), "v"(q01), "v"(q23)); }
-            if constexpr (STATS) { stat2(2 * g, pv[4 * g], pv[4 * g + 1]); stat2(2 * g + 1, pv[4 * g + 2], pv[4 * g + 3]); }
+            if constexpr (STATS && LT) { stat2(0, pv[4 * g], pv[4 * g + 1]); stat2(0, pv[4 * g + 2], pv[4 * g + 3]); }
+            else if constexpr (STATS) { stat2(2 * g, pv[4 * g], pv[4 * g + 1]); stat2(2 * g + 1, pv[4 * g + 2], pv[4 * g + 3]); }
             GR_FENCE();
         });
         if constexpr (RT >= GR_NRES && !GR_VRES) {
@@ -532,23 +572,51 @@
         if constexpr (RT > 0 && (GR_VRES || RT - 1 < GR_NRES)) stats_tile(std::integral_constant<int, RT - 1>{});
         __builtin_amdgcn_sched_barrier(0);
     };
+    float bn5_s = 0.f, bn5_h = 0.f;
+    auto fresh_lane = [&]() __attribute__((always_inline)) {
+        int l;
+        asm volatile("v_mbcnt_lo_u32_b32 %0, -1, 0\n\tv_mbcnt_hi_u32_b32 %0, -1, %0" : "=v"(l));
+        return l;
+    };
     auto layer_boundary = [&](auto Kc) __attribute__((always_inline)) {
         constexpr int k = decltype(Kc)::value;
+        constexpr bool LT = GR_LAST_T && k == 5;
         GR_STAMP_AT(4 + 4 * k);
         if constexpr (GR_VRES && GR_NT > GR_NRES) {
             asm volatile("s_nop 15\n\ts_nop 15" ::: "memory");
-            stats_all(zs[(GR_NT - 1 - GR_NRES) & 1]);
-        }
+            if constexpr (LT) {
+                if (!(GR_ABL & 4)) {
+                    const f32x16 &a = zs[(GR_NT - 1 - GR_NRES) & 1];
+#pragma unroll
+                    for (int i = 0; i < 8; i++) stat2(0, a[2 * i], a[2 * i + 1]);
+                }
+            } else stats_all(zs[(GR_NT - 1 - GR_NRES) & 1]);
+        }
+        float colsum;
+        int kind, scol;
 #if GR_FOLD_DPP
         (void)fold_stats;
-        const float colsum = fold_stats_dpp();
-        const int kind = n >> 4, scol = 32 * wave + 8 * ((n & 15) >> 2) + 4 * h + (n & 3);
-        constexpr int PAIR = 16;
+        constexpr int PAIR = LT ? 32 : 16;
 #else
-        const float colsum = fold_stats();
-        const int kind = tid & 1, scol = tid >> 1;
-        constexpr int PAIR = 1;
-#endif
+        constexpr int PAIR = LT ? 32 : 1;
+#endif
+        int xaddr = 0;
+        if constexpr (LT) {
+            const int lf = fresh_lane();
+            xaddr = (lf ^ 32) << 2;
+            kind = lf >> 5; scol = 32 * wave + (lf & 31);
+            const float cs = gr_hadd(ts[0]), cq = gr_hadd(tq[0]);
+            ts[0] = f32x2{0.f, 0.f}; tq[0] = f32x2{0.f, 0.f};
+            colsum = (kind ? cq : cs) + __builtin_bit_cast(float, __builtin_amdgcn_ds_bpermute(xaddr, __builtin_bit_cast(int, kind ? cs : cq)));
+        } else {
+#if GR_FOLD_DPP
+            colsum = fold_stats_dpp();
+            kind = n >> 4; scol = 32 * wave + 8 * ((n & 15) >> 2) + 4 * h + (n & 3);
+#else
+            colsum = fold_stats();
+            kind = tid & 1; scol = tid >> 1;
+#endif
+        }
         const int sidx = 2 * scol + kind;
         if (k == 1) GR_STAMP_AT(2);
         const unsigned grp = blockIdx.x & 7u;
@@ -564,6 +632,20 @@
         if (k == 1) GR_STAMP_AT(3);
         const float ga = A.gamma[k][scol], be = A.beta[k][scol];
         if constexpr (k < 5) load_weights(k + 1);
+#if GR_LAST_T
+        if constexpr (k == 0) {
+#pragma unroll
+            for (int kk = 0; kk < (GR_ROWS + 255) / 256; kk++) {
+                const int r = tid + 256 * kk;
+                if (r < GR_ROWS) { const int sl = s_rowcand[r]; s_rowoff[r] = (unsigned)((sl >= 0 && sl < GR_IMGCAP ? sl : GR_IMGCAP) * (HD * 4)); }
+            }
+#pragma unroll
+            for (int kk = 0; kk < (GR_MAXCAND + 255) / 256; kk++) {
+                const int i = tid + 256 * kk;
+                if (i < GR_MAXCAND) { const int r = s_slotok[i]; s_slotok[i] = (r >= 0 && s_rowcand[r] == i) ? 1 : 0; }
+            }
+        }
+#endif
         GR_STAMP_AT(5 + 4 * k);
         const unsigned long long *w0 = A.stats + (size_t)k * 8 * 256 + sidx;
         unsigned long long vw[8], want[8], ssum = 0;
@@ -588,8 +670,22 @@
             }
             GR_STAMP_AT(6 + 4 * k);
             const double tot = gr_fix_decode(ssum, nblk, A.ffrac[k]);
-            const double oth = __shfl_xor(tot, PAIR);
-            if (!kind) {
+            double oth;
+            if constexpr (LT) {
+                const long long tb = __builtin_bit_cast(long long, tot);
+                const unsigned lo = (unsigned)__builtin_amdgcn_ds_bpermute(xaddr, (int)(unsigned)tb), hi = (unsigned)__builtin_amdgcn_ds_bpermute(xaddr, (int)(unsigned)(tb >> 32));
+                oth = __builtin_bit_cast(double, ((unsigned long long)hi << 32) | lo);
+            } else oth = __shfl_xor(tot, PAIR);
+            if constexpr (LT) {
+                const double csum = kind ? oth : tot, csq = kind ? tot : oth;
+                const double mean = csum * A.inv_rows;
+                double var = csq * A.inv_rows - mean * mean;
+                if (var < 0) var = 0;
+                const float rstd = 1.0f / sqrtf((float)(var + BN_EPS));
+                const float s = rstd * ga;
+                bn5_s = s * A.wsinv[k];
+                bn5_h = be - (float)mean * s;
+            } else if (!kind) {
                 const double mean = tot * A.inv_rows;
                 double var = oth * A.inv_rows - mean * mean;
                 if (var < 0) var = 0;
@@ -599,7 +695,7 @@
                 s_bn[HD + scol] = be - (float)mean * s;
             }
         }
-        LDS_BARRIER();
+        if constexpr (!LT) LDS_BARRIER();
         GR_STAMP_AT(7 + 4 * k);
     };
 
@@ -668,7 +764,7 @@
                     asm volatile("" ::: "memory");
                     __builtin_amdgcn_sched_barrier(0);
                 }
-                consume_tile(Tc);
+                consume_tile(Tc, std::integral_constant<int, layer>{});
                 GR_PIN_V();
                 if constexpr (RT % GR_GRP == GR_GRP - 1) {
                     if constexpr (GR_LOOK > GR_GRP) {
@@ -829,6 +925,124 @@
     });
 
     GR_STAMP_AT(30);
+#if GR_LAST_T
+    {
+        const int lf = fresh_lane(), n = lf & 31, h = lf >> 5, tid = 64 * wave + lf;
+        float *s_part = reinterpret_cast<float *>(smem);
+        float *s_wtab = reinterpret_cast<float *>(smem + GR_FIN_OFF_WTAB);
+        unsigned char *s_img = smem + GR_FIN_OFF_IMG;
+        static_assert(GR_FIN_OFF_IMG + (GR_IMGCAP + 1) * HD * 4 <= GR_OFF_ELLC, "final phase: inside the plane buffers and the ring area");
+        for (int i = tid; i < 33 * 32; i += 256) { const int k = i & 15; s_wtab[i] = 8 * (k >> 2) + 4 * ((i >> 4) & 1) + (k & 3) < (i >> 5) ? 1.0f : 0.0f; }
+        unsigned warm_word = 0;
+        if (A.nwarm > 0) {
+            unsigned l = (blockIdx.x >> 3) * 256u + (unsigned)tid;
+            const unsigned char *wp = reinterpret_cast<const unsigned char *>(A.warm[0]);
+            bool found = false;
+            for (int w = 0; w < A.nwarm; w++) {
+                const unsigned nl = A.warm_lines[w];
+                if (!found && l < nl) { wp = reinterpret_cast<const unsigned char *>(A.warm[w]) + (size_t)l * 128; found = true; }
+                if (!found) l -= nl;
+            }
+            warm_word = *reinterpret_cast<const unsigned *>(wp);
+        }
+        const bool cand_on = A.candidate && !(GR_ABL & 32);
+        const bool cand_img = cand_on && A.ipc * A.J <= GR_IMGCAP;
+        const bool cand_reg = cand_on && !cand_img;
+        const int col = 32 * wave + n;
+        const float sc5 = A.dump_z5 ? 1.0f : bn5_s, sh5 = A.dump_z5 ? 0.0f : bn5_h, fl5 = A.dump_z5 ? -__builtin_inff() : 0.0f;
+        const f32x2 SC = {sc5, sc5}, SH = {sh5, sh5}, FL = {fl5, fl5};
+        int left = T, cur = 0;
+        float run = 0.f;
+        LDS_BARRIER();
+        GR_STAMP_AT(28);
+        gr_static_for<GR_NT>([&](auto Tc) __attribute__((always_inline)) {
+            constexpr int rt = decltype(Tc)::value;
+            const f32x16 &a = GR_TILEVAL(rt);
+            const int b1 = left < 32 ? left : 32, b2 = left + T < 32 ? left + T : 32;
+            const float4 *wt1 = reinterpret_cast<const float4 *>(s_wtab + (2 * b1 + h) * 16), *wt2 = reinterpret_cast<const float4 *>(s_wtab + (2 * b2 + h) * 16);
+            float4 W1[4], W2[4];
+            uint4 ro[4];
+#pragma unroll
+            for (int g = 0; g < 4; g++) { W1[g] = wt1[g]; W2[g] = wt2[g]; }
+#pragma unroll
+            for (int g = 0; g < 4; g++) ro[g] = *reinterpret_cast<const uint4 *>(s_rowoff + rt * 32 + 8 * g + 4 * h);
+            f32x2 v[8];
+#pragma unroll
+            for (int i = 0; i < 8; i++) v[i] = __builtin_elementwise_max(gr_fma2(f32x2{a[2 * i], a[2 * i + 1]}, SC, SH), FL);
+            if (!(GR_ABL & 16)) {
+                f32x2 t2 = {0.f, 0.f}, p2 = t2, q2 = t2;
+#pragma unroll
+                for (int g = 0; g < 4; g++) {
+                    t2 = gr_add2(v[2 * g], t2); p2 = gr_fma2(v[2 * g], f32x2{W1[g].x, W1[g].y}, p2); q2 = gr_fma2(v[2 * g], f32x2{W2[g].x, W2[g].y}, q2);
+                    t2 = gr_add2(v[2 * g + 1], t2); p2 = gr_fma2(v[2 * g + 1], f32x2{W1[g].z, W1[g].w}, p2); q2 = gr_fma2(v[2 * g + 1], f32x2{W2[g].z, W2[g].w}, q2);
+                }
+                const float tot = gr_hadd(t2), s1 = gr_hadd(p2), s2 = gr_hadd(q2);
+                const bool f1 = left <= 32, f2 = left + T <= 32;
+                const float r1 = run + s1;
+                float *pp = s_part + (2 * cur + h) * HD + col;
+                pp[0] = r1;
+                pp[2 * HD] = s2 - s1;
+                run = f2 ? tot - s2 : f1 ? tot - s1 : r1;
+                cur += (f1 ? 1 : 0) + (f2 ? 1 : 0);
+                left += (f1 ? T : 0) + (f2 ? T : 0) - 32;
+            }
+            if (cand_img) {
+#pragma unroll
+                for (int g = 0; g < 4; g++) {
+                    *reinterpret_cast<float *>(s_img + ro[g].x + 4 * col) = v[2 * g][0]; *reinterpret_cast<float *>(s_img + ro[g].y + 4 * col) = v[2 * g][1];
+                    *reinterpret_cast<float *>(s_img + ro[g].z + 4 * col) = v[2 * g + 1][0]; *reinterpret_cast<float *>(s_img + ro[g].w + 4 * col) = v[2 * g + 1][1];
+                }
+            }
+            if (cand_reg) {
+                float *d = A.cand_feat + (size_t)inst0 * A.J * HD + col;
+#pragma unroll
+                for (int k = 0; k < 16; k++) {
+                    const int sl = s_rowcand[rt * 32 + 8 * (k >> 2) + 4 * h + (k & 3)];
+                    if (sl >= 0) d[(size_t)sl * HD] = v[k >> 1][k & 1];
+                }
+            }
+            if (A.h_nodes) {
+                float *d = A.h_nodes + (grow0 + rt * 32 + 4 * h) * HD + col;
+#pragma unroll
+                for (int k = 0; k < 16; k++) {
+                    const int r = 8 * (k >> 2) + (k & 3);
+                    if (rt * 32 + 4 * h + r < nrows) d[(size_t)r * HD] = v[k >> 1][k & 1];
+                }
+            }
+            __builtin_amdgcn_sched_barrier(0);
+        });
+        asm volatile("" :: "v"(warm_word));
+        GR_STAMP_AT(29);
+        LDS_BARRIER();
+        const float invT = 1.0f / (float)T;
+        for (int item = tid; item < ninst * HD; item += 256) {
+            const int inst = item >> 7, c = item & (HD - 1);
+            A.pooled[(size_t)inst0 * HD + item] = (s_part[(2 * inst) * HD + c] + s_part[(2 * inst + 1) * HD + c]) * invT;
+        }
+        if (cand_img) {
+            const int nsl = ninst * A.J;
+#pragma unroll 4
+            for (int s0 = 0; s0 < nsl; s0 += 8) {
+                const int sl = s0 + (tid >> 5);
+                if (sl < nsl && s_slotok[sl])
+                    *reinterpret_cast<float4 *>(A.cand_feat + ((size_t)inst0 * A.J + sl) * HD + 4 * (tid & 31)) = *reinterpret_cast<const float4 *>(s_img + sl * (HD * 4) + 16 * (tid & 31));
+            }
+        }
+        if (A.candidate && s_flag[1]) {
+            __threadfence();
+            __syncthreads();
+            for (int i = wave; i < ninst * A.J; i += 4) {
+                const int cnd = A.candidate[(size_t)inst0 * A.J + i];
+                if (cnd < 0 || cnd >= T) continue;
+                const int win = s_rowcand[(i / A.J) * T + cnd];
+                if (win != i) {
+                    const float2 x = *reinterpret_cast<const float2 *>(A.cand_feat + ((size_t)inst0 * A.J + win) * HD + 2 * lane);
+                    *reinterpret_cast<float2 *>(A.cand_feat + ((size_t)inst0 * A.J + i) * HD + 2 * lane) = x;
+                }
+            }
+        }
+    }
+#else
     {
         float *s_part = reinterpret_cast<float *>(s_planes);
         static_assert(2 * GR_NT * 2 * HD * 4 <= 2 * GR_TILE + 4096, "partial pool sums: plane buffers + 4 KB");
@@ -852,7 +1066,10 @@
         for (int g = 0; g < 4; g++) {
             S[g] = *reinterpret_cast<const float4 *>(s_bn + 32 * wave + 8 * g + 4 * h);
             Hs[g] = *reinterpret_cast<const float4 *>(s_bn + HD + 32 * wave + 8 * g + 4 * h);
-        }
+            if (A.dump_z5) { S[g] = make_float4(1.f, 1.f, 1.f, 1.f); Hs[g] = make_float4(0.f, 0.f, 0.f, 0.f); }
+        }
+        const float fl5 = A.dump_z5 ? -__builtin_inff() : 0.0f;
+        const f32x2 FL = {fl5, fl5};
         if constexpr (GR_NT - GR_NRES >= 1) zload(std::integral_constant<int, 0>{});
         if constexpr (GR_NT - GR_NRES >= 2) zload(std::integral_constant<int, 1>{});
         const int c = lane & 31;
@@ -900,8 +1117,8 @@
             float4 v[4];
 #pragma unroll
             for (int g = 0; g < 4; g++) {
-                const f32x2 lo = __builtin_elementwise_max(gr_fma2(f32x2{a[4 * g], a[4 * g + 1]}, f32x2{S[g].x, S[g].y}, f32x2{Hs[g].x, Hs[g].y}), f32x2{0.f, 0.f});
-                const f32x2 hi = __builtin_elementwise_max(gr_fma2(f32x2{a[4 * g + 2], a[4 * g + 3]}, f32x2{S[g].z, S[g].w}, f32x2{Hs[g].z, Hs[g].w}), f32x2{0.f, 0.f});
+                const f32x2 lo = __builtin_elementwise_max(gr_fma2(f32x2{a[4 * g], a[4 * g + 1]}, f32x2{S[g].x, S[g].y}, f32x2{Hs[g].x, Hs[g].y}), FL);
+                const f32x2 hi = __builtin_elementwise_max(gr_fma2(f32x2{a[4 * g + 2], a[4 * g + 3]}, f32x2{S[g].z, S[g].w}, f32x2{Hs[g].z, Hs[g].w}), FL);
                 v[g] = make_float4(lo[0], lo[1], hi[0], hi[1]);
             }
             float *wb = tb + (rt & 1) * (32 * 36);
@@ -954,6 +1171,7 @@
             }
         }
     }
+#endif
     GR_STAMP_AT(31);
 }
 #endif
diff --git a/e2e-mappo-for-mt-fjsp_amd/encoder.py b/e2e-mappo-for-mt-fjsp_amd/encoder.py
--- a/e2e-mappo-for-mt-fjsp_amd/encoder.py
+++ b/e2e-mappo-for-mt-fjsp_amd/encoder.py
@@ -179,6 +179,16 @@
         import numpy as np
         out = np.empty((self.B * self.M, 128), dtype=np.float32)
         capi.check(self.L.mtfjsp_encoder_peek_nodes_host(self.h, out.ctypes.data, out.size), self.h, enc=True)
+        return out
+
+    def cand_feat(self, fill=None):
+        import numpy as np
+        if fill is not None:
+            out = np.ascontiguousarray(fill, dtype=np.float32).reshape(self.B * self.J, 128)
+            capi.check(self.L.mtfjsp_encoder_cand_feat_host(self.h, out.ctypes.data, out.size, 1), self.h, enc=True)
+            return out
+        out = np.empty((self.B * self.J, 128), dtype=np.float32)
+        capi.check(self.L.mtfjsp_encoder_cand_feat_host(self.h, out.ctypes.data, out.size, 0), self.h, enc=True)
         return out
 
     def range_fallbacks(self):
diff --git a/include/mtfjsp.h b/include/mtfjsp.h
--- a/include/mtfjsp.h
+++ b/include/mtfjsp.h
@@ -192,6 +192,7 @@
 int mtfjsp_encoder_check(mtfjsp_encoder_t e, int32_t *gin_resident_out);
 int mtfjsp_encoder_range_fallbacks(mtfjsp_encoder_t e, int64_t *count_out, int32_t *product_mode_out);
 int mtfjsp_encoder_peek_nodes_host(mtfjsp_encoder_t e, float *out_host, int64_t count);
+int mtfjsp_encoder_cand_feat_host(mtfjsp_encoder_t e, float *host, int64_t count, int32_t to_device);
 int mtfjsp_encoder_resident_failures(mtfjsp_encoder_t e, int64_t *count_out);
 int mtfjsp_encoder_timing_begin(mtfjsp_encoder_t e);
 int mtfjsp_encoder_timing_end(mtfjsp_encoder_t e, double *ms_total, int64_t *launches);
```
